# zhouxian/FluidLab

Hardware: AMD Instinct MI355X
Metric: MPM substeps/sec (fwd+bwd), 128^3 grid / 200k particles (higher is better)
Workload: dtype f32; 1 GPU; water block 128^3 grid, 200k particles (BASELINE configs[1] inputs), fwd+bwd, evolving (rolling window); nc_start=34727, nc_end=99039, parallelism=1 env, 1 GPU

## Files before the change

### __graft_entry__.py

```python
import os
import subprocess
import sys

ROOT = os.path.dirname(os.path.abspath(__file__))
CSRC = os.path.join(ROOT, 'fluidlab_amd', 'csrc')
HIP_LIB = os.path.join(CSRC, 'libfluidengine_hip.so')
HIPCC_FLAGS = ['--offload-arch=gfx950', '-O3', '-std=c++17', '-shared', '-fPIC', '-munsafe-fp-atomics', '-fno-slp-vectorize']


def _hipcc():
    for c in ('/opt/rocm/bin/hipcc', 'hipcc'):
        if c == 'hipcc' or os.path.exists(c):
            return c


def _source_hash(sources):
    import hashlib
    h = hashlib.sha256(' '.join(HIPCC_FLAGS).encode())
    for s in sources:
        h.update(os.path.basename(s).encode())
        with open(s, 'rb') as f:
            h.update(f.read())
    return h.hexdigest()


def build(force=False):
    srcs = [os.path.join(CSRC, f) for f in ('fe_engine.hip', 'fe_math.h', 'fe_grid_launch.h', 'fe_smoke.h', 'fe_smoke_reads.h', 'fe_mesh.h', 'fe_param_grad.h', 'fe_summary.h', 'fe_task_loss.h', 'fe_density.h', 'fe_render.h')] + \
           [os.path.join(ROOT, 'include', f) for f in ('fluidengine.h', 'fluidengine_ext.h')]
    stamp, want = HIP_LIB + '.srchash', _source_hash(srcs)
    have = open(stamp).read().strip() if os.path.exists(stamp) else ''
    if force or os.environ.get('FE_FORCE_BUILD') == '1' or not os.path.exists(HIP_LIB) or have != want:
        subprocess.check_call([_hipcc()] + HIPCC_FLAGS + ['-o', HIP_LIB, os.path.join(CSRC, 'fe_engine.hip')])
        with open(stamp, 'w') as f:
            f.write(want + '\n')
        print('build: compiled', os.path.relpath(HIP_LIB, ROOT), 'from sources', want[:16])
    else:
        print('build: up to date', os.path.relpath(HIP_LIB, ROOT), 'sources', want[:16])
    subprocess.check_call(['make', '-s', '-C', os.path.join(ROOT, 'oracle')])
    if ROOT not in sys.path:
        sys.path.insert(0, ROOT)
    import fluidlab_amd
    from fluidlab_amd import _capi
    lib = _capi.load_hip()
    missing = lib.missing_symbols()
    assert not missing, f'libfluidengine_hip.so is missing ABI symbols: {missing}'
    assert lib.has_ext, f'libfluidengine_hip.so is missing extension symbols: {lib.missing_ext_symbols()}'


def smoke():
    if ROOT not in sys.path:
        sys.path.insert(0, ROOT)
    sys.path.insert(0, os.path.join(ROOT, 'tests'))
    import numpy as np
    import scenarios as S
    from fluidlab_amd import _capi
    hip = _capi.load_hip()
    oracle = _capi.EngineLib(os.path.join(ROOT, 'oracle', '_build', 'libfe_oracle_f64.so'))
    sc = S.latte_mini()
    a = S.run_latte(hip, sc, device=0)
    b = S.run_latte(oracle, sc)
    assert (a['final']['used'] == b['final']['used']).all()
    assert S.rel_l2(a['final']['x'], b['final']['x']) <= 1e-5, S.rel_l2(a['final']['x'], b['final']['x'])
    assert S.rel_l2(a['step_loss'], b['step_loss']) <= 1e-4
    assert S.cosine(a['action_grad'], b['action_grad']) >= 0.999999
    assert S.rel_l2(a['action_grad'], b['action_grad']) <= 1e-4
    print('smoke ok: backend', hip.backend, 'loss', float(np.sum(a['step_loss'])),
          'action-grad rel L2 vs oracle', S.rel_l2(a['action_grad'], b['action_grad']))


if __name__ == '__main__':
    build(force='--force' in sys.argv)
    if len(sys.argv) > 1 and sys.argv[1] == 'smoke':
        smoke()
```

### fluidlab_amd/csrc/fe_engine.hip

```cpp
#include <hip/hip_runtime.h>

#include <algorithm>
#include <cstdio>
#include <cstdlib>
#include <cstring>
#include <string>
#include <vector>

#include "../../include/fluidengine.h"
#include "../../include/fluidengine_ext.h"
#include "fe_math.h"
#include "fe_grid_launch.h"

static_assert(sizeof(fe_real) == 4, "the HIP engine is fp32 (macros.py:207-211)");

#define FR_WORDS 25
#define GR_WORDS 24

template <typename T>
struct Plane {
    char* base; unsigned off;
    __host__ __device__ __forceinline__ T& operator[](int s) const { return *(T*)(base + (size_t)(off + (unsigned)s * (unsigned)sizeof(T))); }
    __host__ __device__ __forceinline__ T* ptr() const { return (T*)(base + (size_t)off); }
};
// ... 278 lines not shown
struct TileO { int ox, oy, oz; };
#define BLK_PACK(bi, bj, bk) (((bi) << 20) | ((bj) << 10) | (bk))
#define BLK_I(pk) ((pk) >> 20)
#define BLK_J(pk) (((pk) >> 10) & 1023)
#define BLK_K(pk) ((pk) & 1023)
__device__ __forceinline__ TileO tile_origin(int pk) {
    TileO t; t.ox = BLK_I(pk) * 4 - 1; t.oy = BLK_J(pk) * 4 - 1; t.oz = BLK_K(pk) * 4 - 1; return t;
}
__device__ __forceinline__ int tile_base(const TileO& t, const Stencil& st) {
    int lx = st.base[0] - t.ox, ly = st.base[1] - t.oy, lz = st.base[2] - t.oz;
    bool in = (unsigned)lx <= TILE_T - 3 && (unsigned)ly <= TILE_T - 3 && (unsigned)lz <= TILE_T - 3;
    return in ? (lx * TILE_T + ly) * TILE_T + lz : -1;
}
__device__ __forceinline__ bool tile_node(const TileO& t, int l, int n, int& i, int& j, int& k) {
    i = t.ox + (l >> 6); j = t.oy + ((l >> 3) & 7); k = t.oz + (l & 7);
    return (unsigned)i < (unsigned)n && (unsigned)j < (unsigned)n && (unsigned)k < (unsigned)n;
}

struct PairCtx {
    int4 it;
    int  ti;
    int  slab;
    int  nth, t0;
    int  i;
    bool live;
    bool quad;
};
#define QUAD_BIT (1 << 29)
#define QUAD_MAX 64
#ifndef QH
#define QH 2
#endif
struct UnitRec { int4 a, b, c, d; };
struct Unit { int4 a, b, q; };
__device__ __forceinline__ PairCtx pair_ctx(const Unit& u) {
    const int tid = threadIdx.x, half = __builtin_amdgcn_readfirstlane(tid >> 7);
    const bool same = (u.a.w >> 30) & 1;
    const int ia = u.a.w & 0x1fffffff, ib = u.b.w;
    const int ih = half ? ib : ia;
    PairCtx c;
    c.live = same || ih >= 0;
    c.it = (half && ib >= 0) ? u.b : u.a;
    c.it.w = 0;
    if (ih < 0) c.it.z = 0;
    c.ti = (half && !same) ? 1 : 0;
    c.slab = same ? ia : (ih >= 0 ? ih : ia);
    c.nth = same ? WG : HALF;
    c.t0 = same ? tid : (tid & (HALF - 1));
    c.i = tid & (HALF - 1);
    c.quad = false;
    return c;
}
__device__ __forceinline__ PairCtx unit_ctx(const Unit& u) {
    const int tid = threadIdx.x;
    const bool quad = (u.a.w & QUAD_BIT) != 0;
    const int wave = __builtin_amdgcn_readfirstlane(tid >> 6), half = wave >> 1;
    const bool same = (u.a.w >> 30) & 1;
    const int ia = u.a.w & 0x1fffffff;
    const int ax = u.a.x, ay = u.a.y, az = u.a.z, bx = u.b.x, by = u.b.y, bz = u.b.z, bw = u.b.w, qx = u.q.x, qy = u.q.y, qz = u.q.z, qw = u.q.w;
    const bool second = half && bw >= 0;
    const int mx = quad ? qx : (second ? bx : ax);
    const int my = quad ? qy : (second ? by : ay);
    const int mz = quad ? qz : (second ? bz : az);
    const int ih = quad ? (wave == 0 ? ia : qw) : (half ? bw : ia);
    PairCtx c;
    c.quad = quad;
    c.live = (same && !quad) || ih >= 0;
    c.it = make_int4(mx, my, ih >= 0 ? mz : 0, 0);
    c.ti = quad ? wave : ((half && !same) ? 1 : 0);
    c.slab = quad ? (ih >= 0 ? ih : 0) : (same ? ia : (ih >= 0 ? ih : ia));
    c.nth = quad ? 64 : (same ? WG : HALF);
    c.t0 = quad ? (tid & 63) : (same ? tid : (tid & (HALF - 1)));
    c.i = quad ? (tid & 63) : (tid & (HALF - 1));
    return c;
}
__device__ __forceinline__ void unit_sync(bool quad) {
    if (quad) asm volatile("" ::: "memory");
    else __syncthreads();
}
__device__ __forceinline__ void unit_enter(bool quad, bool& prev_quad) {
    if (prev_quad && !quad) __syncthreads();
    prev_quad = quad;
}
template <bool GATHER = false>
__device__ __forceinline__ Unit unit_load(const TableP& T, int w) {
    const int4* p = (const int4*)((GATHER ? T.units_p : T.units) + (w < T.units_cap ? w : T.units_cap - 1));
    int4 a = p[0], b = p[1], q = p[__builtin_amdgcn_readfirstlane(threadIdx.x >> 6)];
    if (w >= T.units_cap) a.z = -2;
#define UNIT_SCALAR(q) make_int4(__builtin_amdgcn_readfirstlane(q.x), __builtin_amdgcn_readfirstlane(q.y), __builtin_amdgcn_readfirstlane(q.z), __builtin_amdgcn_readfirstlane(q.w))
    Unit u;
    u.a = UNIT_SCALAR(a); u.b = UNIT_SCALAR(b); u.q = UNIT_SCALAR(q);
#undef UNIT_SCALAR
    return u;
}

#define FE_MAX_BATCH 8
#ifndef FE_KALIGN_BYTES
#define FE_KALIGN_BYTES 16384
#endif
#define FE_KALIGN __attribute__((aligned(FE_KALIGN_BYTES)))
template <typename A> struct Batch { A a[FE_MAX_BATCH]; };


__device__ void effector_move(const EffP& e, int f) {
    float xin[3] = {e.pos[f * 3] + e.v[f * 3], e.pos[f * 3 + 1] + e.v[f * 3 + 1], e.pos[f * 3 + 2] + e.v[f * 3 + 2]};
    float xn[3], J[3][3];
    boundary_x(e.bnd, xin, xn, J);
    e.pos[(f + 1) * 3] = xn[0]; e.pos[(f + 1) * 3 + 1] = xn[1]; e.pos[(f + 1) * 3 + 2] = xn[2];
    float w3[3] = {e.w[f * 3], e.w[f * 3 + 1], e.w[f * 3 + 2]};
    float q[4] = {e.quat[f * 4], e.quat[f * 4 + 1], e.quat[f * 4 + 2], e.quat[f * 4 + 3]};
    float qw[4], qo[4];
    quat_from_w(w3, qw);
    quat_mul(qw, q, qo);
    e.quat[(f + 1) * 4] = qo[0]; e.quat[(f + 1) * 4 + 1] = qo[1]; e.quat[(f + 1) * 4 + 2] = qo[2]; e.quat[(f + 1) * 4 + 3] = qo[3];
}

#define GS_BLK 112
struct GridStore { float4* data; int* flag; int cap;
    unsigned char* touched; unsigned char* dirty; unsigned char* live; unsigned char* cur; unsigned char stamp; };
__device__ __forceinline__ int stencil_regions(int lb) {
    const int lut = 0x26c93;
    const int ax = (lut >> (3 * (lb >> 6))) & 7, ay = (lut >> (3 * ((lb >> 3) & 7))) & 7, az = (lut >> (3 * (lb & 7))) & 7;
    const int myz = ((ay & 1) ? az : 0) | ((ay & 2) ? az << 3 : 0) | ((ay & 4) ? az << 6 : 0);
    return ((ax & 1) ? myz : 0) | ((ax & 2) ? myz << 9 : 0) | ((ax & 4) ? myz << 18 : 0);
}
__device__ __forceinline__ int neighbour_entry(const int* __restrict__ blk_slot, int nb, int pk) {
    int lane = threadIdx.x & 63;
    asm volatile("" : "+v"(lane));
    int e = -1;
    if (lane < 27) {
        const int i2 = BLK_I(pk) + lane / 9 - 1, j2 = BLK_J(pk) + (lane / 3) % 3 - 1, k2 = BLK_K(pk) + lane % 3 - 1;
        if ((unsigned)i2 < (unsigned)nb && (unsigned)j2 < (unsigned)nb && (unsigned)k2 < (unsigned)nb) e = blk_slot[(i2 * nb + j2) * nb + k2];
    }
    return e;
}
template <int CTRL, int ROW_MASK>
__device__ __forceinline__ int dpp_or(int x) { return x | __builtin_amdgcn_update_dpp(0, x, CTRL, ROW_MASK, 0xf, true); }
template <bool FG = false>
__device__ __forceinline__ int touch_regions(int mask, int entry, const GridStore& GS) {
    mask = dpp_or<0x111, 0xf>(mask); mask = dpp_or<0x112, 0xf>(mask); mask = dpp_or<0x114, 0xf>(mask); mask = dpp_or<0x118, 0xf>(mask);
    mask = dpp_or<0x142, 0xa>(mask); mask = dpp_or<0x143, 0xc>(mask);
    mask = __builtin_amdgcn_readlane(mask, 63);
    if (!FG && entry >= 0 && ((mask >> (threadIdx.x & 63)) & 1)) GS.touched[entry] = GS.stamp;
    return mask;
}
__device__ __forceinline__ void mark_dirty(const GridStore& GS, const int* __restrict__ blk_slot, int b) {
    const int e = blk_slot[b];
    if (e >= 0) GS.dirty[e] = GS.stamp;
}

#define FG_SH 32
#define FG_LINE 32
enum { FGC_STARTED = 0 , FGC_DONE = 8 , FGC_FIN = FGC_DONE + FG_SH , FGC_TOP = FGC_FIN + FG_SH, FGC_LATE, FGC_SKIP, FGC_ERR, FGC_N };
struct FgDev {
    float* late;
    int* late_flag; int* late_list;
    unsigned char* skipm;
    int* ctr;
};
struct FgArgs {
    const FgDev* F; const float4* slab; float* acc; float4* out; int* blk_list; int* blk_count; int* blk_flag; int f;
};
#define FG_CNT(a) ((int)((a) & 0x1fffffull))
#define FG_TCH(a) ((int)(((a) >> 21) & 0x1fffffull))
#define FG_DRT(a) ((int)((a) >> 42))
__shared__ int s_fg[10];
template <bool BWD> __device__ __forceinline__ void fg_owner_phase(const SimP& S, const TableP& T, const GridStore& GS, const FgArgs& A);
__device__ __forceinline__ void fg_rare(const FgDev* F) { (void)__hip_atomic_fetch_or(F->ctr + FGC_TOP * FG_LINE, 1 << 16, __ATOMIC_RELAXED, __HIP_MEMORY_SCOPE_AGENT); }
__device__ __forceinline__ void fg_mark_late(const FgDev* F, int e) {
    int* fl = F->late_flag + e;
    const int v = __hip_atomic_load(fl, __ATOMIC_RELAXED, __HIP_MEMORY_SCOPE_AGENT);
    if (v != 1 && atomicCAS(fl, v, 1) == v) {
        const int i = atomicAdd(F->ctr + FGC_LATE * FG_LINE, 1);
        __hip_atomic_store(F->late_list + i, e, __ATOMIC_RELAXED, __HIP_MEMORY_SCOPE_AGENT);
        fg_rare(F);
    }
}
__device__ __forceinline__ void fg_begin(const FgDev* F) {
    if (threadIdx.x == 0) (void)__hip_atomic_fetch_add(F->ctr + (FGC_STARTED + (blockIdx.x & 7)) * FG_LINE, 1, __ATOMIC_RELAXED, __HIP_MEMORY_SCOPE_AGENT);
    if (threadIdx.x < 10) s_fg[threadIdx.x] = 0;
    __syncthreads();
}
__device__ __forceinline__ int wave_or(int mask) {
    mask = dpp_or<0x111, 0xf>(mask); mask = dpp_or<0x112, 0xf>(mask); mask = dpp_or<0x114, 0xf>(mask); mask = dpp_or<0x118, 0xf>(mask);
// ... 409 lines not shown
#pragma unroll
    for (int a = 0; a < 3; a++)
#pragma unroll
        for (int b = 0; b < 3; b++) nC.a[a][b] = c4 * __builtin_fmaf(-st.fx[b], nv[a], M.a[a][b]);
}
template <bool TILE, bool ALIAS, bool ROLLED = false>
__device__ __forceinline__ void g2p_gather(const SimP& S, int lb, const Stencil& st, const float4* __restrict__ g_out, int tofs, float nv[3], m3& nC) {
    if (!TILE) { g2p_gather_global<true, ALIAS ? FE_SLOW_UNR : 1>(S, st, g_out, nv, nC); return; }
    const float* gt = ALIAS ? (const float*)s_acc : s_gtile;
    nv[0] = nv[1] = nv[2] = 0.f;
    const float c4 = 4.f * S.inv_dx;
    m3 M = m3_zero();
#pragma unroll ROLLED ? 1 : 9
    for (int ij = 0; ij < 9; ij++) {
        const int i = ij / 3, j = ij - 3 * i;
        const float wij = STW(st, i, 0) * STW(st, j, 1);
        float T[3] = {0.f, 0.f, 0.f}, Tz[3] = {0.f, 0.f, 0.f};
#pragma unroll
        for (int kk = 0; kk < 3; kk++) {
            const float weight = wij * st.w[kk][2];
            float g0, g1, g2;
            if (TILE) {
                const int l = tofs + lb + (i * TILE_T + j) * TILE_T + kk;
                g0 = gt[l]; g1 = gt[TILE_N + l]; g2 = gt[2 * TILE_N + l];
            } else {
                float4 gv = g_out[cell_addr(st.base[0] + i, st.base[1] + j, st.base[2] + kk, S.nb)];
                g0 = gv.x; g1 = gv.y; g2 = gv.z;
            }
            const float gw[3] = {weight * g0, weight * g1, weight * g2};
#pragma unroll
            for (int a = 0; a < 3; a++) { T[a] += gw[a]; if (kk > 0) Tz[a] += (float)kk * gw[a]; }
        }
#pragma unroll
        for (int a = 0; a < 3; a++) {
            nv[a] += T[a];
            M.a[a][0] += (float)i * T[a]; M.a[a][1] += (float)j * T[a]; M.a[a][2] += Tz[a];
        }
    }
#pragma unroll
    for (int a = 0; a < 3; a++)
#pragma unroll
        for (int b = 0; b < 3; b++) nC.a[a][b] = c4 * (M.a[a][b] - st.fx[b] * nv[a]);
}
template <int NIT, typename LD, typename ST>
__device__ __forceinline__ void tile_nodes_n(int t0, int nth, LD&& ld, ST&& st) {
    float4 v[NIT];
#pragma unroll
    for (int it = 0; it < NIT; it++) v[it] = ld(t0 + it * nth);
#pragma unroll
    for (int it = 0; it < NIT; it++) st(t0 + it * nth, v[it]);
}
template <bool QUADS = true, int MAXIT = 8, typename LD, typename ST>
__device__ __forceinline__ void tile_nodes(int t0, int nth, LD&& ld, ST&& st) {
    if (nth == WG) tile_nodes_n<2>(t0, nth, ld, st);
    else if (!QUADS || nth == HALF) {
        if constexpr (MAXIT >= 4) tile_nodes_n<4>(t0, nth, ld, st);
        else { tile_nodes_n<2>(t0, nth, ld, st); tile_nodes_n<2>(t0 + 2 * nth, nth, ld, st); }
    } else {
        if constexpr (MAXIT >= 8) tile_nodes_n<8>(t0, nth, ld, st);
        else if constexpr (MAXIT >= 4) { tile_nodes_n<4>(t0, nth, ld, st); tile_nodes_n<4>(t0 + 4 * nth, nth, ld, st); }
        else { for (int r = 0; r < 4; r++) tile_nodes_n<2>(t0 + 2 * r * nth, nth, ld, st); }
    }
}
__device__ __forceinline__ float4 tile_node_load(const TileO& to, const SimP& S, const float4* __restrict__ src, int l) {
    int i, j, k;
    const bool ok = tile_node(to, l, S.n, i, j, k);
    const float4 v = src[ok ? cell_addr(i, j, k, S.nb) : 0];
    return make_float4(ok ? v.x : 0.f, ok ? v.y : 0.f, ok ? v.z : 0.f, ok ? v.w : 0.f);
}
template <bool ALIAS = false>
__device__ __forceinline__ void load_tile3(const TileO& to, const SimP& S, const float4* __restrict__ src, const PairCtx& pc, int tofs_alias = 0) {
    if (!pc.live) return;
    float* gt = ALIAS ? (float*)s_acc : s_gtile;
    const int tofs = ALIAS ? tofs_alias : pc.ti * 3 * TILE_N;
    tile_nodes<ALIAS>(pc.t0, pc.nth, [&](int l) { return tile_node_load(to, S, src, l); },
                      [&](int l, const float4 v) { gt[tofs + l] = v.x; gt[tofs + TILE_N + l] = v.y; gt[tofs + 2 * TILE_N + l] = v.z; });
}

struct FuseP { float* fr_prev; const float4* g_out; int* slow; int* blk_count_prev; };
template <bool WRITE, bool GENERAL, bool FUSED = false, bool FG = false>
__device__ __forceinline__ void p2g_body(SimP S, float* fr_cur, float* fr_next, TableP T,
                                            const int* __restrict__ pool_idx, GridW G, AgentP agent, InjectP inj, int act, int f,
                                            GridStore GS, int fiso, FuseP FU = FuseP{nullptr, nullptr, nullptr, nullptr}) {
    if (!WRITE && GS.cap > 0 && GS.flag[f]) return;
    const int tid = threadIdx.x;
    if (WRITE && blockIdx.x == 0 && tid == 0 && act) {
        for (int i = 0; i < agent.n; i++) effector_move(agent.e[i], f);
    }
    if (FG) {
        if (blockIdx.x == 0 && tid == 0 && GS.cap > 0) __hip_atomic_store(GS.flag + f, 1, __ATOMIC_RELAXED, __HIP_MEMORY_SCOPE_AGENT);
        fg_begin(G.fg);
    }
    if (FUSED && blockIdx.x == 0 && tid == 0) *FU.blk_count_prev = 0;
    FrameV cur = frame_view(fr_cur, S.Np, 0, (!GENERAL && (fiso & 1)) ? 1 : 0);
    FrameV curw = frame_view(fr_cur, S.Np, 0);
    FrameV prev = frame_view(FUSED ? FU.fr_prev : fr_cur, S.Np);
    FrameV nxt = frame_view(fr_next, S.Np, S.wt & 1, (!GENERAL && (fiso & 2)) ? 1 : 0);
    const int slab_wt = FG ? 1 : (S.wt & 1);
    TL(S, 0);
    Unit un = unit_load(T, blockIdx.x);
    const int n_slots = T.meta[5];
    bool prev_quad = false;
    for (int wg = blockIdx.x; FG || wg < n_slots; wg += gridDim.x) {
        if (FG || wg != (int)blockIdx.x) un = unit_load(T, wg);
        if (FG && wg >= n_slots) break;
        if (un.a.z == -2) continue;
        if (un.a.z >= 0) {
            const PairCtx pc = unit_ctx(un);
            unit_enter(pc.quad, prev_quad);
            const int4 it = pc.it;
            const TileO to = tile_origin(it.x);
            const int aofs = pc.ti * 4 * TILE_N;
            int fg_t = 0, fg_d = 0;
            TL(S, 1);
            const int nbr_entry = neighbour_entry(T.blk_slot, S.nb, it.x);
            auto zero_tile = [&]() {
                if (pc.quad) { if (pc.live) for (int l = pc.t0; l < TILE_N; l += 64) ((int4*)((int*)s_acc + aofs))[l] = make_int4(0, 0, 0, 0); }
                else if (pc.live) for (int l = pc.t0; l < 4 * TILE_N; l += pc.nth) s_acc[aofs + l] = 0.0;
            };
            if (!FUSED) { zero_tile(); unit_sync(pc.quad); }
            FixScale fs_p = {1.f, 1.f}, fs_m = {1.f, 1.f};
            bool wshell = false;
            {
                const int wbase = pc.quad ? 0 : (pc.i & 64);
                const int cnt = __builtin_amdgcn_readfirstlane(min(64, max(0, it.z - wbase)));
                const LaneSplit ls = lane_split(cnt, (S.lsplit & 1) != 0 && !(WRITE && !FUSED && act && agent.collector));
                const int i = wbase + ls.p, s = it.y + i;
                const bool has = ls.ok && i < it.z;
                const int s_ld = has ? s : it.y;
                const int uflag = cur.used[s_ld];
                P2GRaw raw;
                if (FUSED) {
                    const int gofs_w = pc.quad ? aofs : 2 * aofs;
                    const int uprev = prev.used[s_ld];
                    const float4 a0 = prev.A0[s_ld];
                    load_F(cur, s_ld, raw.p.F);
                    raw.info = load_info(S, T.info, s_ld);
                    load_tile3<true>(to, S, FU.g_out, pc, gofs_w);
                    unit_sync(pc.quad);
                    const float xp[3] = {a0.x, a0.y, a0.z};
                    Stencil stp;
                    stencil_make(xp, S.inv_dx, stp);
                    if (has && uprev != 0 && stencil_inside(stp, S.n)) {
                        const int lbp = tile_base(to, stp);
                        if (lbp >= 0) g2p_gather<true, true>(S, lbp, stp, FU.g_out, gofs_w, raw.p.v, raw.p.C);
                        else { if (ls.primary) atomicAdd(FU.slow, 1); g2p_gather<false, true, true>(S, 0, stp, FU.g_out, 0, raw.p.v, raw.p.C); }
#pragma unroll
                        for (int a = 0; a < 3; a++) raw.p.x[a] = xp[a] + S.dt * raw.p.v[a];
                        if (ls.primary) store_xvC(curw, s, raw.p.x, raw.p.v, raw.p.C);
                    } else load_xvC(cur, s_ld, raw.p);
                    unit_sync(pc.quad);
                    zero_tile();
                    unit_sync(pc.quad);
                } else p2g_load(S, cur, s_ld, T.info, raw);
                bool used = has && uflag != 0;
                bool taken = false;
                if (WRITE && !FUSED && used && act && agent.collector) { taken = collector_takes(S, cur, nxt, s, T.info, agent); used = !taken; }
                P2GPrep q;
                q.inside = false;
                int lb = -1;
                if (used) {
                    p2g_compute<WRITE, GENERAL>(S, nxt, s, raw, G, q, ls.primary);
                    if (q.inside) lb = tile_base(to, q.st);
                } else {
                    q.m = 0.f; q.affine = m3_zero(); q.mv[0] = q.mv[1] = q.mv[2] = 0.f;
                    float zero[3] = {0.f, 0.f, 0.f};
                    stencil_make(zero, S.inv_dx, q.st);
                }
                TL(S, 2);
#ifdef FE_DUMMY_VALU
                {
                    float dmy = q.m;
#pragma unroll
                    for (int i_ = 0; i_ < FE_DUMMY_VALU; i_++) asm volatile("v_fma_f32 %0, %0, %0, %0" : "+v"(dmy));
                    asm volatile("" :: "v"(dmy));
                }
#endif
                const bool in_tile = lb >= 0;
                if (used && q.inside && !in_tile && ls.primary) { atomicAdd(G.slow, 1); p2g_scatter_global<FG>(S, q, G, GS, T.blk_slot, it.x, fg_d); }
                if (__any(in_tile)) {
                    fg_t = touch_regions<FG>(in_tile ? stencil_regions(lb) : 0, nbr_entry, GS);
                    if (pc.quad) {
                        wshell = __any(in_tile && stencil_on_shell(lb));
                        float bp = 0.f;
#pragma unroll
                        for (int a = 0; a < 3; a++) bp = fmaxf(bp, fabsf(q.mv[a]) + 2.f * S.dx * (fabsf(q.affine.a[a][0]) + fabsf(q.affine.a[a][1]) + fabsf(q.affine.a[a][2])));
                        fs_p = fix_scale(wave_max(in_tile ? bp : 0.f));
                        fs_m = fix_scale(wave_max(in_tile ? q.m : 0.f));
                        if (__any(in_tile && !(bp <= 3.4e38f))) fs_p.inv = __int_as_float(0x7fc00000);
                        const float sp = in_tile ? fs_p.s : 1.f;
                        q.m *= in_tile ? fs_m.s : 1.f;
#pragma unroll
                        for (int a = 0; a < 3; a++) { q.mv[a] *= sp; q.affine.a[a][0] *= sp; q.affine.a[a][1] *= sp; q.affine.a[a][2] *= sp; }
                        p2g_scatter_tile_split<true>(S, q, in_tile, in_tile ? lb : 0, aofs, ls);
                    } else p2g_scatter_tile_split<false>(S, q, in_tile, in_tile ? lb : 0, aofs, ls);
                }
                if (has && !used && !taken && WRITE && ls.primary) unused_particle_fwd(S, cur, nxt, s, T.pid_of_slot[s], pool_idx, agent, inj, f);
            }
            TL(S, 4);
            unit_sync(pc.quad);
            TL(S, 5);
            if (pc.quad) {
                if (pc.live) quad_handover<4, FG>(S, (const int*)s_acc + aofs, fs_p.inv, fs_m.inv, G.slab, pc.slab, G.g_in, GS, to, nbr_entry, wshell, slab_wt, fg_d);
            } else if (pc.live) for (int l = pc.t0; l < TILE_N; l += pc.nth)
                tile_handover<4, false, FG>(S, G.slab, pc.slab, G.g_in, GS, to, nbr_entry, l,
                                 make_float4((float)s_acc[aofs + l], (float)s_acc[aofs + TILE_N + l], (float)s_acc[aofs + 2 * TILE_N + l], (float)s_acc[aofs + 3 * TILE_N + l]), slab_wt, fg_d);
            if (FG) fg_unit_end(T, pc, nbr_entry, fg_t, fg_d);
            else unit_sync(pc.quad);
            TL(S, 6);
        } else {
            const int s = un.a.y + tid;
            if (s < S.N) {
                P2GRaw raw;
                bool have = false;
                if (FUSED && prev.used[s]) {
                    const float4 a0 = prev.A0[s];
                    const float xp[3] = {a0.x, a0.y, a0.z};
                    Stencil stp;
                    stencil_make(xp, S.inv_dx, stp);
                    if (stencil_inside(stp, S.n)) {
                        g2p_gather<false, true, true>(S, 0, stp, FU.g_out, 0, raw.p.v, raw.p.C);
#pragma unroll
                        for (int a = 0; a < 3; a++) raw.p.x[a] = xp[a] + S.dt * raw.p.v[a];
                        store_xvC(curw, s, raw.p.x, raw.p.v, raw.p.C);
                        have = true;
                    }
                }
                if (cur.used[s]) {
                    if (WRITE && !FUSED && act && agent.collector && collector_takes(S, cur, nxt, s, T.info, agent)) continue;
                    P2GPrep q;
                    if (FUSED && have) { load_F(cur, s, raw.p.F); raw.info = load_info(S, T.info, s); p2g_compute<WRITE, GENERAL>(S, nxt, s, raw, G, q); }
                    else p2g_prepare<WRITE, GENERAL>(S, cur, nxt, s, T.info, G, q);
                    int none = 0;
                    if (q.inside) p2g_scatter_global<FG>(S, q, G, GS, T.blk_slot, -1, none);
                } else if (WRITE) unused_particle_fwd(S, cur, nxt, s, T.pid_of_slot[s], pool_idx, agent, inj, f);
            }
        }
    }
}
struct P2GArgs { SimP S; float* fr_cur; float* fr_next; TableP T; const int* pool_idx; GridW G; AgentP agent; InjectP inj; int act; int f; GridStore GS; int fiso; FuseP FU; };
template <bool WRITE, bool GENERAL>
__global__ FE_KALIGN __launch_bounds__(WG, GENERAL ? 3 : 4) void k_p2g(SimP S, float* fr_cur, float* fr_next, TableP T, const int* pool_idx, GridW G, AgentP agent, InjectP inj, int act, int f, GridStore GS, int fiso) { p2g_body<WRITE, GENERAL>(S, fr_cur, fr_next, T, pool_idx, G, agent, inj, act, f, GS, fiso); }
template <bool GENERAL>
__global__ FE_KALIGN __launch_bounds__(WG, GENERAL ? 3 : 4) void k_g2p_p2g(SimP S, float* fr_cur, float* fr_next, TableP T, const int* pool_idx, GridW G, AgentP agent, InjectP inj, int act, int f, GridStore GS, int fiso, FuseP FU) { p2g_body<true, GENERAL, true>(S, fr_cur, fr_next, T, pool_idx, G, agent, inj, act, f, GS, fiso, FU); }
template <typename ARGS>
__device__ __forceinline__ const ARGS* fg_args_again() {
    const ARGS* p = (const ARGS*)__builtin_amdgcn_kernarg_segment_ptr();
    asm volatile("" : "+s"(p));
    return p;
}
template <bool GENERAL>
__global__ FE_KALIGN __launch_bounds__(WG, GENERAL ? 3 : 4) void k_p2g_fg(P2GArgs A) {
    p2g_body<true, GENERAL, false, true>(A.S, A.fr_cur, A.fr_next, A.T, A.pool_idx, A.G, A.agent, A.inj, A.act, A.f, A.GS, A.fiso);
    const P2GArgs* B = fg_args_again<P2GArgs>();
    TL(B->S, 3);
    fg_owner_phase<false>(B->S, B->T, B->GS, FgArgs{B->G.fg, B->G.slab, B->G.g_in, B->G.g_out, B->G.blk_list, B->G.blk_count, B->G.blk_flag, B->f});
}
template <bool GENERAL>
__global__ FE_KALIGN __launch_bounds__(WG, GENERAL ? 3 : 4) void k_g2p_p2g_fg(P2GArgs A) {
    p2g_body<true, GENERAL, true, true>(A.S, A.fr_cur, A.fr_next, A.T, A.pool_idx, A.G, A.agent, A.inj, A.act, A.f, A.GS, A.fiso, A.FU);
    const P2GArgs* B = fg_args_again<P2GArgs>();
    TL(B->S, 3);
    fg_owner_phase<false>(B->S, B->T, B->GS, FgArgs{B->G.fg, B->G.slab, B->G.g_in, B->G.g_out, B->G.blk_list, B->G.blk_count, B->G.blk_flag, B->f});
}
template <bool GENERAL>
__global__ FE_KALIGN __launch_bounds__(WG, GENERAL ? 3 : 4) void k_g2p_p2g_b(Batch<P2GArgs> B) { const P2GArgs& A = B.a[blockIdx.y]; p2g_body<true, GENERAL, true>(A.S, A.fr_cur, A.fr_next, A.T, A.pool_idx, A.G, A.agent, A.inj, A.act, A.f, A.GS, A.fiso, A.FU); }
template <bool WRITE, bool GENERAL>
__global__ FE_KALIGN __launch_bounds__(WG, GENERAL ? 3 : 4) void k_p2g_b(Batch<P2GArgs> B) { const P2GArgs& A = B.a[blockIdx.y]; p2g_body<WRITE, GENERAL>(A.S, A.fr_cur, A.fr_next, A.T, A.pool_idx, A.G, A.agent, A.inj, A.act, A.f, A.GS, A.fiso); }


template <bool NODE>
__device__ __forceinline__ bool agent_collide_particle(const SimP& S, const AgentP& agent, int f, const float x[3], float nv[3]) {
    const float sdt = NODE ? 0.f : S.dt;
    bool any = false;
    for (int ei = 0; ei < agent.n; ei++) {
        const EffP& e = agent.e[ei];
        if (!e.has_mesh) continue;
        const float pos[3] = {x[0] + sdt * nv[0], x[1] + sdt * nv[1], x[2] + sdt * nv[2]};
        if (!(pos[1] > agent.collide_min_y)) continue;
        float out[3];
        any |= t_dynamic_collide<float>(e.mesh, e.pos + f * 3, e.quat + f * 4, e.pos + (f + 1) * 3, e.quat + (f + 1) * 4, pos, nv, S.dt, out);
        nv[0] = out[0]; nv[1] = out[1]; nv[2] = out[2];
    }
    return any;
}
#define FE_MAX_STATICS 4
struct NodeWork { int c, ni, nj, nk; float4 gi; float go[3]; float pad; };
struct StaticsP { int n; const SdfP* s; };

template <bool STATICS, bool DYN = false>
__device__ __forceinline__ void node_velocity(const SimP& S, const StaticsP& ST, const float4 gi, int i, int j, int k, float vo[3], float kmul[3],
                                              float (*trace)[3] = nullptr, const AgentP* agent = nullptr, int f = 0, float* vdyn = nullptr,
                                              bool* dyn_hit = nullptr) {
    float inv = 1.f / gi.w;
    vo[0] = fmaf(S.dt, S.g[0], inv * gi.x);
    vo[1] = fmaf(S.dt, S.g[1], inv * gi.y);
    vo[2] = fmaf(S.dt, S.g[2], inv * gi.z);
    float xn[3] = {(float)i * S.dx, (float)j * S.dx, (float)k * S.dx};
    if (STATICS) {
#pragma unroll
        for (int si = 0; si < FE_MAX_STATICS; si++) {
            if (si < ST.n) {
                if (trace) { trace[si][0] = vo[0]; trace[si][1] = vo[1]; trace[si][2] = vo[2]; }
                static_collide(ST.s[si], xn, vo, nullptr);
            }
        }
    }
    if (DYN) {
        if (vdyn) { vdyn[0] = vo[0]; vdyn[1] = vo[1]; vdyn[2] = vo[2]; }
        const bool hit = agent_collide_particle<true>(S, *agent, f, xn, vo);
        if (dyn_hit) *dyn_hit = hit;
    }
    boundary_v(S.bnd, xn, vo, kmul);
}
__device__ __forceinline__ void node_statics_grad(const SimP& S, const StaticsP& ST, int i, int j, int k, const float (*trace)[3], float g[3]) {
    float xn[3] = {(float)i * S.dx, (float)j * S.dx, (float)k * S.dx};
#pragma unroll
    for (int si = FE_MAX_STATICS - 1; si >= 0; si--) {
        if (si < ST.n) {
            float vin[3] = {trace[si][0], trace[si][1], trace[si][2]};
            static_collide(ST.s[si], xn, vin, g);
        }
    }
}

__device__ __forceinline__ int2 nbr_record(const TableP& T, int e, int lane) {
    return lane < 27 ? T.nbr[e * 27 + lane] : make_int2(0, 0);
}
template <int NPL>
__device__ __forceinline__ float4 gather_slabs(const float4* __restrict__ slab, const int2 mine, int lane) {
    const int o[3] = {lane >> 4, (lane >> 2) & 3, lane & 3};
    int a0[8], n[8];
    float4 v0[8], v1[8];
#pragma unroll
    for (int c = 0; c < 8; c++) {
        int nbr = 0, si = 0;
        bool valid = true;
#pragma unroll
        for (int d = 0; d < 3; d++) {
            const bool other = (c >> d) & 1;
            valid = valid && (!other || o[d] <= 1);
            nbr = nbr * 3 + (other ? 0 : 1);
            si = si * SLAB_T + o[d] + (other ? 4 : 0);
        }
        const int f = __shfl(mine.x, nbr, 64), k = __shfl(mine.y, nbr, 64);
        n[c] = valid ? k : 0;
        a0[c] = valid ? (NPL == 4 ? f * SLAB_N + si : f * (SLAB_N * 16) + si * 12) : 0;
    }
    const __amdgpu_buffer_rsrc_t rs = wt_rsrc((void*)slab);
    auto ld = [&](int at) -> float4 {
        if (NPL == 4) return slab[at];
        const u32x3 u = __builtin_amdgcn_raw_buffer_load_b96(rs, at, 0, 0);
        return make_float4(__uint_as_float(u.x), __uint_as_float(u.y), __uint_as_float(u.z), 0.f);
    };
    constexpr int STRIDE = NPL == 4 ? SLAB_N : SLAB_N * 16;
#pragma unroll
    for (int c = 0; c < 8; c++) {
        const bool h0 = n[c] > 0, h1 = n[c] > 2;
        const float4 a = ld(h0 ? a0[c] : 0);
        const float4 b = ld(h1 ? a0[c] + 2 * STRIDE : 0);
        v0[c] = make_float4(h0 ? a.x : 0.f, h0 ? a.y : 0.f, h0 ? a.z : 0.f, h0 ? a.w : 0.f);
        v1[c] = make_float4(h1 ? b.x : 0.f, h1 ? b.y : 0.f, h1 ? b.z : 0.f, h1 ? b.w : 0.f);
    }
    float4 acc = make_float4(0.f, 0.f, 0.f, 0.f);
#pragma unroll
    for (int c = 0; c < 8; c++) {
        acc.x += v0[c].x; acc.y += v0[c].y; acc.z += v0[c].z; acc.w += v0[c].w;
        acc.x += v1[c].x; acc.y += v1[c].y; acc.z += v1[c].z; acc.w += v1[c].w;
        for (int k = 4; k < n[c]; k += 2) {
            const float4 v = ld(a0[c] + k * STRIDE);
            acc.x += v.x; acc.y += v.y; acc.z += v.z; acc.w += v.w;
        }
    }
    return acc;
}

__device__ __forceinline__ int static_entry(int wave) {
    const int G = gridDim.x;
    if ((G & 127) != 0) return blockIdx.x * 4 + wave;
    const int j = blockIdx.x >> 3;
    return ((j >> 4) * 8 + (blockIdx.x & 7)) * 64 + (j & 15) * 4 + wave;
}
template <bool KEEP, bool STATICS, bool DYN>
__device__ __forceinline__ void grid_body(SimP S, TableP T, const float4* __restrict__ slab, float* g_in, float4* g_out,
                                              const int* __restrict__ blk_list, const int* __restrict__ blk_count, int* blk_flag,
                                              GridStore GS, int f, int* frame_slow, StaticsP ST, AgentP agent) {
    if (KEEP && GS.cap > 0 && GS.flag[f]) return;
    const int lane = threadIdx.x & 63, wave = __builtin_amdgcn_readfirstlane(threadIdx.x >> 6);
    TL(S, 0);
    const int es = static_entry(wave);
    const bool es_ok = es < S.nb * S.nb * S.nb;
    const int blk_s = es_ok ? T.active[es] : 0;
    const unsigned char tch_s = es_ok ? GS.touched[es] : (unsigned char)0, drt_s = es_ok ? GS.dirty[es] : (unsigned char)0;
    const int2 nbr_s = es_ok ? nbr_record(T, es, lane) : make_int2(0, 0);
    const int n_static = T.meta[2], n_dyn = *blk_count;
    if (!KEEP && blockIdx.x == 0 && threadIdx.x == 0) {
        if (GS.cap > 0) GS.flag[f] = (n_static <= GS.cap && *frame_slow == 0) ? 1 : 0;
        *frame_slow = 0;
    }
    auto one_block = [&](int e, int b, bool is_static, bool touched, bool dirty, const int2 nbr) {
        const int c = (b << 6) | lane;
        const int bi = b / (S.nb * S.nb), bj = (b / S.nb) % S.nb, bk = b % S.nb;
        TL(S, 1);
        float4 gi = make_float4(0.f, 0.f, 0.f, 0.f);
        if (dirty) gi = make_float4(g_in[c], g_in[S.ncell + c], g_in[2 * S.ncell + c], g_in[3 * S.ncell + c]);
        if (touched) { const float4 t = gather_slabs<4>(slab, nbr, lane); gi.x += t.x; gi.y += t.y; gi.z += t.z; gi.w += t.w; }
        float4 out = make_float4(0.f, 0.f, 0.f, 0.f);
        if (gi.w > FE_EPS) TL(S, 2);
        if (gi.w > FE_EPS) {
            float vo[3], kmul[3];
            node_velocity<STATICS, DYN>(S, ST, gi, bi * 4 + (lane >> 4), bj * 4 + ((lane >> 2) & 3), bk * 4 + (lane & 3), vo, kmul, nullptr, &agent, f);
            out = make_float4(vo[0], vo[1], vo[2], 0.f);
        }
        g_out[c] = out;
        if (!KEEP) {
            if (is_static && e < GS.cap) {
                float4* dst = GS.data + ((size_t)f * GS.cap + e) * GS_BLK;
                dst[lane] = gi;
                const u32x3 u = {__float_as_uint(out.x), __float_as_uint(out.y), __float_as_uint(out.z)};
                __builtin_amdgcn_raw_buffer_store_b96(u, wt_rsrc(dst), 1024 + lane * 12, 0, 0);
            }
            if (dirty) { g_in[c] = 0.f; g_in[S.ncell + c] = 0.f; g_in[2 * S.ncell + c] = 0.f; g_in[3 * S.ncell + c] = 0.f; }
            if (lane == 0 && !is_static) blk_flag[b] = 0;
        } else {
            g_in[c] = gi.x; g_in[S.ncell + c] = gi.y; g_in[2 * S.ncell + c] = gi.z; g_in[3 * S.ncell + c] = gi.w;
        }
        TL(S, 3);
    };
    if (n_static <= 4 * (int)gridDim.x) {
        if (es < n_static) {
            const bool tm = tch_s == GS.stamp, dm = drt_s == GS.stamp;
            if (lane == 0) {
                if (KEEP) GS.cur[es] = (tm || dm) ? 1 : 0;
                else if (es < GS.cap) GS.live[(size_t)f * GS.cap + es] = (tm || dm) ? 1 : 0;
            }
            if (tm || dm) one_block(es, blk_s, true, tm, dm, nbr_s);
        }
    } else {
        const int W = 4 * (int)gridDim.x;
        for (int e0 = es; e0 < n_static; e0 += 8 * W) {
            unsigned tm = 0, dm = 0;
            int blk8[8]; int2 nbr8[8];
#pragma unroll
            for (int k = 0; k < 8; k++) {
                const int e = e0 + k * W;
                const bool ok = e < n_static;
                const int ec = ok ? e : e0;
                const unsigned char t = GS.touched[ec], d = GS.dirty[ec];
                blk8[k] = T.active[ec]; nbr8[k] = nbr_record(T, ec, lane);
                tm |= ((ok && t == GS.stamp) ? 1u : 0u) << k; dm |= ((ok && d == GS.stamp) ? 1u : 0u) << k;
            }
            tm = __builtin_amdgcn_readfirstlane(tm); dm = __builtin_amdgcn_readfirstlane(dm);
            if (lane < 8 && e0 + lane * W < n_static) {
                const int e = e0 + lane * W;
                if (KEEP) GS.cur[e] = ((tm | dm) >> lane) & 1;
                else if (e < GS.cap) GS.live[(size_t)f * GS.cap + e] = ((tm | dm) >> lane) & 1;
            }
            unsigned todo = tm | dm;
            while (todo) {
                const int k = __builtin_ctz(todo);
                todo &= todo - 1;
                int blk = blk8[0]; int2 nbr = nbr8[0];
#pragma unroll
                for (int j = 1; j < 8; j++) if (k == j) { blk = blk8[j]; nbr = nbr8[j]; }
                one_block(e0 + k * W, __builtin_amdgcn_readfirstlane(blk), true, (tm >> k) & 1, (dm >> k) & 1, nbr);
            }
        }
    }
    for (int d = blockIdx.x * 4 + wave; d < n_dyn; d += gridDim.x * 4) one_block(-1, blk_list[d], false, false, true, make_int2(0, 0));
}
struct GridArgs { SimP S; TableP T; const float4* slab; float* g_in; float4* g_out; const int* blk_list; const int* blk_count; int* blk_flag; GridStore GS; int f; int* frame_slow; StaticsP ST; AgentP agent; };
template <bool KEEP, bool STATICS, bool DYN>
__global__ FE_KALIGN __launch_bounds__(256, (STATICS || DYN) ? 2 : 4) void k_grid(SimP S, TableP T, const float4* slab, float* g_in, float4* g_out, const int* blk_list, const int* blk_count, int* blk_flag, GridStore GS, int f, int* frame_slow, StaticsP ST, AgentP agent) { grid_body<KEEP, STATICS, DYN>(S, T, slab, g_in, g_out, blk_list, blk_count, blk_flag, GS, f, frame_slow, ST, agent); }
template <bool KEEP, bool STATICS, bool DYN>
__global__ FE_KALIGN __launch_bounds__(256, (STATICS || DYN) ? 2 : 4) void k_grid_b(Batch<GridArgs> B) { const GridArgs& A = B.a[blockIdx.y]; grid_body<KEEP, STATICS, DYN>(A.S, A.T, A.slab, A.g_in, A.g_out, A.blk_list, A.blk_count, A.blk_flag, A.GS, A.f, A.frame_slow, A.ST, A.agent); }

__device__ __forceinline__ float4 fg_load16(const void* base, unsigned byte_off) {
    const u32x4 u = __builtin_amdgcn_raw_buffer_load_b128(wt_rsrc((void*)base), (int)byte_off, 0, 16);
    return make_float4(__uint_as_float(u.x), __uint_as_float(u.y), __uint_as_float(u.z), __uint_as_float(u.w));
}
__device__ __forceinline__ float4 fg_node_out(const SimP& S, const float4 gi, int b, int lane, float kmul[3]) {
    float4 out = make_float4(0.f, 0.f, 0.f, 0.f);
    kmul[0] = kmul[1] = kmul[2] = 0.f;
    if (gi.w > FE_EPS) {
        const int bi = b / (S.nb * S.nb), bj = (b / S.nb) % S.nb, bk = b % S.nb;
        float vo[3];
        node_velocity<false, false>(S, StaticsP{0, nullptr}, gi, bi * 4 + (lane >> 4), bj * 4 + ((lane >> 2) & 3), bk * 4 + (lane & 3), vo, kmul);
        out = make_float4(vo[0], vo[1], vo[2], 0.f);
    }
    return out;
}
__device__ __forceinline__ void fg_fwd_store(const GridStore& GS, const FgArgs& A, int e, int c, int lane, const float4 gi, const float4 out) {
    wt_store16(A.out, (unsigned)c * 16u, out);
    if (e >= 0 && e < GS.cap) {
        float4* dst = GS.data + ((size_t)A.f * GS.cap + e) * GS_BLK;
        wt_store16(dst, (unsigned)lane * 16u, gi);
        const u32x3 u = {__float_as_uint(out.x), __float_as_uint(out.y), __float_as_uint(out.z)};
        __builtin_amdgcn_raw_buffer_store_b96(u, wt_rsrc(dst), 1024 + lane * 12, 0, 16);
    }
}
__device__ __forceinline__ void fg_fwd_block(const SimP& S, const GridStore& GS, const FgArgs& A, int e, int b, const int2 nbr, bool touched, bool dirty) {
    const int lane = threadIdx.x & 63;
    const int c = (b << 6) | lane;
    float4 gi = make_float4(0.f, 0.f, 0.f, 0.f);
    if (dirty) gi = make_float4(atomicExch(A.acc + c, 0.f), atomicExch(A.acc + S.ncell + c, 0.f), atomicExch(A.acc + 2 * S.ncell + c, 0.f), atomicExch(A.acc + 3 * S.ncell + c, 0.f));
    if (touched) { const float4 t = gather_slabs<4>(A.slab, nbr, lane); gi.x += t.x; gi.y += t.y; gi.z += t.z; gi.w += t.w; }
    float kmul[3];
    const float4 out = fg_node_out(S, gi, b, lane, kmul);
    fg_fwd_store(GS, A, e, c, lane, gi, out);
}
__device__ __forceinline__ float4 fg_grad_out(const float4 gi, const float4 go, const float kmul[3]) {
    float4 out = make_float4(0.f, 0.f, 0.f, 0.f);
    if (gi.w > FE_EPS) {
        const float inv = 1.f / gi.w;
        const float g0 = go.x * kmul[0], g1 = go.y * kmul[1], g2 = go.z * kmul[2];
        out.x = g0 * inv; out.y = g1 * inv; out.z = g2 * inv;
        out.w = -(gi.x * g0 + gi.y * g1 + gi.z * g2) * inv * inv;
    }
    return out;
}
__device__ __forceinline__ void fg_bwd_block(const SimP& S, const GridStore& GS, const FgArgs& A, int e, int b, const int2 nbr, bool dirty) {
    const int lane = threadIdx.x & 63;
    const int c = (b << 6) | lane;
    const float4 gi = GS.data[((size_t)A.f * GS.cap + e) * GS_BLK + lane];
    float4 go = make_float4(0.f, 0.f, 0.f, 0.f);
    if (dirty) go = make_float4(atomicExch(A.acc + c, 0.f), atomicExch(A.acc + S.ncell + c, 0.f), atomicExch(A.acc + 2 * S.ncell + c, 0.f), 0.f);
    { const float4 t = gather_slabs<3>(A.slab, nbr, lane); go.x += t.x; go.y += t.y; go.z += t.z; }
    float kmul[3];
    (void)fg_node_out(S, gi, b, lane, kmul);
    wt_store16(A.out, (unsigned)c * 16u, fg_grad_out(gi, go, kmul));
}
__device__ __forceinline__ unsigned long long fg_word(const unsigned long long* p) {
    const unsigned long long a = __hip_atomic_load(p, __ATOMIC_RELAXED, __HIP_MEMORY_SCOPE_AGENT);
    return (unsigned long long)(unsigned)__builtin_amdgcn_readfirstlane((int)(unsigned)a) | ((unsigned long long)(unsigned)__builtin_amdgcn_readfirstlane((int)(unsigned)(a >> 32)) << 32);
}
__device__ __forceinline__ int fg_int(const int* p) { return __hip_atomic_load(p, __ATOMIC_RELAXED, __HIP_MEMORY_SCOPE_AGENT); }
__device__ __forceinline__ int fg_int_u(const int* p) { return __builtin_amdgcn_readfirstlane(fg_int(p)); }
#define FG_SPIN_MAX (1 << 22)
__device__ __forceinline__ void fg_give_up(const FgDev* F) { if ((threadIdx.x & 63) == 0) atomicAdd(F->ctr + FGC_ERR * FG_LINE, 1); }
template <bool BWD>
__device__ __forceinline__ void fg_entry(const SimP& S, const TableP& T, const GridStore& GS, const FgArgs& A, int e, unsigned long long a) {
    const int lane = threadIdx.x & 63;
    const bool touched = FG_TCH(a) != 0, dirty = FG_DRT(a) != 0;
    if (lane == 0) __hip_atomic_store(T.arrive + e, 0ull, __ATOMIC_RELAXED, __HIP_MEMORY_SCOPE_AGENT);
    const int b = T.active[e];
    const int2 nbr = nbr_record(T, e, lane);
    if (!BWD) {
        if (lane == 0 && e < GS.cap) __hip_atomic_store(GS.live + (size_t)A.f * GS.cap + e, (unsigned char)((touched || dirty) ? 1 : 0), __ATOMIC_RELAXED, __HIP_MEMORY_SCOPE_AGENT);
        if (touched || dirty) fg_fwd_block(S, GS, A, e, b, nbr, touched, dirty);
    } else {
        if (GS.live[(size_t)A.f * GS.cap + e] != 0) fg_bwd_block(S, GS, A, e, b, nbr, dirty);
    }
}
template <bool BWD>
__device__ __forceinline__ void fg_final(const SimP& S, const TableP& T, const GridStore& GS, const FgArgs& A) {
    const int lane = threadIdx.x & 63;
    const FgDev* F = A.F;
    int* const ctr = F->ctr;
    const int n_static = T.meta[2];
    const int* __restrict__ expected = (const int*)(T.arrive + S.nb * S.nb * S.nb);
    const int n_dyn = BWD ? 0 : fg_int_u(A.blk_count), n_skip = fg_int_u(ctr + FGC_SKIP * FG_LINE), n_late = fg_int_u(ctr + FGC_LATE * FG_LINE);
    if (!BWD && n_dyn > 0) {
        for (int d = 0; d < n_dyn; d++) {
            const int b = fg_int_u(A.blk_list + d), c = (b << 6) | lane;
            const float4 gi = make_float4(atomicExch(F->late + c, 0.f), atomicExch(F->late + S.ncell + c, 0.f), atomicExch(F->late + 2 * S.ncell + c, 0.f), atomicExch(F->late + 3 * S.ncell + c, 0.f));
            float kmul[3];
            fg_fwd_store(GS, A, -1, c, lane, gi, fg_node_out(S, gi, b, lane, kmul));
            if (lane == 0) __hip_atomic_store(A.blk_flag + b, 0, __ATOMIC_RELAXED, __HIP_MEMORY_SCOPE_AGENT);
        }
        if (lane == 0) {
            __hip_atomic_store(A.blk_count, 0, __ATOMIC_RELAXED, __HIP_MEMORY_SCOPE_AGENT);
            if (GS.cap > 0) __hip_atomic_store(GS.flag + A.f, 0, __ATOMIC_RELAXED, __HIP_MEMORY_SCOPE_AGENT);
        }
    }
    if (n_skip > 0) {
        for (int e0 = 0; e0 < n_static; e0 += 64) {
            const int e = e0 + lane;
            unsigned long long todo = __ballot(e < n_static && __hip_atomic_load(F->skipm + e, __ATOMIC_RELAXED, __HIP_MEMORY_SCOPE_AGENT) == GS.stamp);
            while (todo) {
                const int k = __builtin_ctzll(todo);
                todo &= todo - 1;
                const int ek = e0 + k;
                if (lane == 0) __hip_atomic_store(F->skipm + ek, (unsigned char)0, __ATOMIC_RELAXED, __HIP_MEMORY_SCOPE_AGENT);
                const unsigned long long a = fg_word(T.arrive + ek);
                if (FG_CNT(a) != expected[ek]) fg_give_up(F);
                fg_entry<BWD>(S, T, GS, A, ek, a);
            }
        }
        if (lane == 0) __hip_atomic_store(ctr + FGC_SKIP * FG_LINE, 0, __ATOMIC_RELAXED, __HIP_MEMORY_SCOPE_AGENT);
    }
    if (n_late > 0) {
        for (int it = 0; ; it++) {
            int v = lane < FG_SH ? fg_int(ctr + (FGC_FIN + lane) * FG_LINE) : 0;
#pragma unroll
            for (int o = 16; o >= 1; o >>= 1) v += __shfl_xor(v, o, 64);
            if ((unsigned)__builtin_amdgcn_readfirstlane(v) - S.fg_base == gridDim.x) break;
            if (it > FG_SPIN_MAX) { fg_give_up(F); break; }
            __builtin_amdgcn_s_sleep(8);
        }
        for (int i = 0; i < n_late; i++) {
            const int e = fg_int_u(F->late_list + i);
            const int b = T.active[e], c = (b << 6) | lane;
            if (lane == 0) __hip_atomic_store(F->late_flag + e, 0, __ATOMIC_RELAXED, __HIP_MEMORY_SCOPE_AGENT);
            float4 lt = make_float4(atomicExch(F->late + c, 0.f), atomicExch(F->late + S.ncell + c, 0.f), atomicExch(F->late + 2 * S.ncell + c, 0.f), 0.f);
            float kmul[3];
            if (!BWD) {
                lt.w = atomicExch(F->late + 3 * S.ncell + c, 0.f);
                const bool live = e < GS.cap && __hip_atomic_load(GS.live + (size_t)A.f * GS.cap + e, __ATOMIC_RELAXED, __HIP_MEMORY_SCOPE_AGENT) != 0;
                float4 gi = make_float4(0.f, 0.f, 0.f, 0.f);
                if (live) gi = fg_load16(GS.data + ((size_t)A.f * GS.cap + e) * GS_BLK, (unsigned)lane * 16u);
                gi.x += lt.x; gi.y += lt.y; gi.z += lt.z; gi.w += lt.w;
                fg_fwd_store(GS, A, e, c, lane, gi, fg_node_out(S, gi, b, lane, kmul));
                if (lane == 0 && e < GS.cap) __hip_atomic_store(GS.live + (size_t)A.f * GS.cap + e, (unsigned char)1, __ATOMIC_RELAXED, __HIP_MEMORY_SCOPE_AGENT);
            } else if (GS.live[(size_t)A.f * GS.cap + e] != 0) {
                const float4 gi = GS.data[((size_t)A.f * GS.cap + e) * GS_BLK + lane];
                (void)fg_node_out(S, gi, b, lane, kmul);
                const float4 d = fg_grad_out(gi, lt, kmul), o = fg_load16(A.out, (unsigned)c * 16u);
                wt_store16(A.out, (unsigned)c * 16u, make_float4(o.x + d.x, o.y + d.y, o.z + d.z, o.w + d.w));
            }
        }
        if (lane == 0) __hip_atomic_store(ctr + FGC_LATE * FG_LINE, 0, __ATOMIC_RELAXED, __HIP_MEMORY_SCOPE_AGENT);
    }
}
#define FG_NPF 2
template <bool BWD>
__device__ __forceinline__ void fg_owner_phase(const SimP& S, const TableP& T, const GridStore& GS, const FgArgs& A) {
    int lane = threadIdx.x & 63;
    asm volatile("" : "+v"(lane));
    const int wave = __builtin_amdgcn_readfirstlane(threadIdx.x >> 6);
    const FgDev* F = A.F;
    int* const ctr = F->ctr;
    const int G_ = gridDim.x, W = 4 * G_;
    const int es = static_entry(wave);
    const int n_static = T.meta[2];
    const int* __restrict__ expected = (const int*)(T.arrive + S.nb * S.nb * S.nb);
    const int e_l = es + lane * W;
    const bool have = e_l < n_static;
    const int exp_l = have ? expected[e_l] : 0, b_l = have ? T.active[e_l] : 0;
    const unsigned char live_l = (BWD && have) ? GS.live[(size_t)A.f * GS.cap + e_l] : (unsigned char)0;
    int2 pf[FG_NPF];
#pragma unroll
    for (int j = 0; j < FG_NPF; j++) pf[j] = (es + j * W < n_static) ? nbr_record(T, es + j * W, lane) : make_int2(0, 0);
    int st = lane < 8 ? fg_int(ctr + (FGC_STARTED + lane) * FG_LINE) : 0;
    st += __shfl_xor(st, 1, 64); st += __shfl_xor(st, 2, 64); st += __shfl_xor(st, 4, 64);
    const bool wait = (unsigned)__builtin_amdgcn_readfirstlane(st) - S.fg_base == (unsigned)G_ && !S.fg_nowait;
    unsigned long long a_l = have ? __hip_atomic_load(T.arrive + e_l, __ATOMIC_RELAXED, __HIP_MEMORY_SCOPE_AGENT) : 0ull;
    unsigned long long pending = __ballot(have);
    if (!wait) {
        const bool skip = have && FG_CNT(a_l) != exp_l;
        if (skip) __hip_atomic_store(F->skipm + e_l, GS.stamp, __ATOMIC_RELAXED, __HIP_MEMORY_SCOPE_AGENT);
        int nskip = __popcll(__ballot(skip));
        for (int e = es + 64 * W; e < n_static; e += W) { if (lane == 0) __hip_atomic_store(F->skipm + e, GS.stamp, __ATOMIC_RELAXED, __HIP_MEMORY_SCOPE_AGENT); nskip++; }
        if (nskip && lane == 0) { atomicAdd(ctr + FGC_SKIP * FG_LINE, nskip); fg_rare(F); }
        pending &= ~__ballot(skip);
    }
    asm volatile("s_waitcnt vmcnt(0)" ::: "memory");
    int r1 = -1;
    bool signs = false;
    if (lane == 0 && atomicAdd(&s_fg[8], 1) == 3) { signs = true; r1 = atomicAdd(ctr + (FGC_DONE + (int)(blockIdx.x % FG_SH)) * FG_LINE, 1); }
    signs = __builtin_amdgcn_readfirstlane(signs ? 1 : 0) != 0;
    for (int it = 0; pending; it++) {
        const bool mine_pending = (pending >> lane) & 1ull;
        const bool done = mine_pending && FG_CNT(a_l) == exp_l;
        const unsigned long long done_now = __ballot(done);
        if (!done_now) {
            if (it > FG_SPIN_MAX) { fg_give_up(F); break; }
            __builtin_amdgcn_s_sleep(2);
            if (mine_pending) a_l = __hip_atomic_load(T.arrive + e_l, __ATOMIC_RELAXED, __HIP_MEMORY_SCOPE_AGENT);
            continue;
        }
        TL(S, 5);
        const bool touched = FG_TCH(a_l) != 0, dirty = FG_DRT(a_l) != 0;
        bool heavy = false;
        if (done) {
            __hip_atomic_store(T.arrive + e_l, 0ull, __ATOMIC_RELAXED, __HIP_MEMORY_SCOPE_AGENT);
            if (!BWD) {
                heavy = touched || dirty;
                if (e_l < GS.cap) __hip_atomic_store(GS.live + (size_t)A.f * GS.cap + e_l, (unsigned char)(heavy ? 1 : 0), __ATOMIC_RELAXED, __HIP_MEMORY_SCOPE_AGENT);
            } else heavy = live_l != 0;
        }
        unsigned long long todo = __ballot(heavy);
        const unsigned long long dirty_set = __ballot(dirty), touched_set = __ballot(touched);
        pending &= ~done_now;
        if ((pending >> lane) & 1ull) a_l = __hip_atomic_load(T.arrive + e_l, __ATOMIC_RELAXED, __HIP_MEMORY_SCOPE_AGENT);
        auto record = [&](int kk) -> int2 {
            if (kk < FG_NPF) {
                int2 r = pf[0];
#pragma unroll
                for (int j = 1; j < FG_NPF; j++) if (kk == j) r = pf[j];
                return r;
            }
            return nbr_record(T, es + kk * W, lane);
        };
        int k = todo ? __builtin_ctzll(todo) : -1;
        int2 nbr = k >= 0 ? record(k) : make_int2(0, 0);
        while (k >= 0) {
            todo &= todo - 1;
            const int k_next = todo ? __builtin_ctzll(todo) : -1;
            const int2 nbr_next = k_next >= 0 ? record(k_next) : make_int2(0, 0);
            const int e = es + k * W, b = __builtin_amdgcn_readlane(b_l, k);
            if (!BWD) fg_fwd_block(S, GS, A, e, b, nbr, (touched_set >> k) & 1ull, (dirty_set >> k) & 1ull);
            else fg_bwd_block(S, GS, A, e, b, nbr, (dirty_set >> k) & 1ull);
            k = k_next; nbr = nbr_next;
        }
    }
    if (wait) for (int e = es + 64 * W; e < n_static; e += W) {
        const int exp_e = expected[e];
        unsigned long long a = fg_word(T.arrive + e);
        for (int it = 0; FG_CNT(a) != exp_e; it++) {
            if (it > FG_SPIN_MAX) { fg_give_up(F); break; }
            __builtin_amdgcn_s_sleep(2);
            a = fg_word(T.arrive + e);
        }
        fg_entry<BWD>(S, T, GS, A, e, a);
    }
    TL(S, 4);
// ... 29 lines not shown
}

__device__ __forceinline__ void load_tile4(const TileO& to, const SimP& S, const float4* __restrict__ src, const PairCtx& pc) {
    if (!pc.live) return;
    const int tofs = pc.ti * 4 * TILE_N;
    tile_nodes<false>(pc.t0, pc.nth, [&](int l) { return tile_node_load(to, S, src, l); },
                      [&](int l, const float4 v) { s_tile[tofs + l] = v.x; s_tile[tofs + TILE_N + l] = v.y; s_tile[tofs + 2 * TILE_N + l] = v.z; s_tile[tofs + 3 * TILE_N + l] = v.w; });
}

template <bool COLLIDE>
__device__ __forceinline__ bool slot_g2p(const SimP& S, const FrameV& cur, const FrameV& nxt, int s, bool use_tile,
                                         const TileO& to, const float4* __restrict__ g_out, int* slow, const AgentP& agent, int f,
                                         int u, const float4 a0, int tofs, float xn[3]) {
    if (!u) return false;
    float x[3] = {a0.x, a0.y, a0.z};
    Stencil st;
    stencil_make(x, S.inv_dx, st);
    if (!stencil_inside(st, S.n)) return false;
    const int lb = use_tile ? tile_base(to, st) : -1;
    if (lb >= 0) used_particle_g2p<true, COLLIDE>(S, cur, nxt, s, lb, st, x, g_out, agent, f, tofs, xn);
    else { if (use_tile) atomicAdd(slow, 1); used_particle_g2p<false, COLLIDE>(S, cur, nxt, s, 0, st, x, g_out, agent, f, 0, xn); }
    return true;
}

#define SORT_CLR_WGS 32
struct SortKeyP { int* key; int* rank; int* cnt; int* bcnt; int* nact; };
__shared__ int s_sk[8];
__device__ __forceinline__ int sort_key_of(const SimP& S, const float x[3]) {
    Stencil st;
    stencil_make(x, S.inv_dx, st);
    return stencil_inside(st, S.n) ? cell_addr(st.base[0], st.base[1], st.base[2], S.nb) : S.ncell;
}
template <bool WG_TAIL>
__device__ __forceinline__ void sort_key_rank(const SimP& S, const SortKeyP& K, bool has, int s, int kk) {
    int lane = threadIdx.x & 63;
    asm volatile("" : "+v"(lane));
    const unsigned long long below = (1ull << lane) - 1ull;
    int r_tail = -1;
    if (WG_TAIL) {
        const int wave = __builtin_amdgcn_readfirstlane(threadIdx.x >> 6);
        const unsigned long long mt = __ballot(has && kk == S.ncell);
        if (lane == 0) s_sk[wave] = __popcll(mt);
        __syncthreads();
        if (threadIdx.x == 0) {
            const int tot = s_sk[0] + s_sk[1] + s_sk[2] + s_sk[3];
            int base = 0;
            if (tot > 0) { base = atomicAdd(K.cnt + S.ncell, tot); atomicAdd(K.bcnt + (S.ncell >> 6), tot); }
            s_sk[4] = base;
        }
        __syncthreads();
        int before = 0;
        for (int w = 0; w < wave; w++) before += s_sk[w];
        if (has && kk == S.ncell) r_tail = s_sk[4] + before + __popcll(mt & below);
        __syncthreads();
        has = has && kk != S.ncell;
    }
    unsigned long long rem = __ballot(has);
    int leader = lane, idx = 0, size = 0;
    while (rem) {
        const int L = __builtin_ctzll(rem);
        const int k = __builtin_amdgcn_readlane(kk, L);
        const unsigned long long m = __ballot(has && kk == k);
        if ((m >> lane) & 1ull) { leader = L; idx = __popcll(m & below); size = __popcll(m); }
        rem &= ~m;
    }
    int base = 0;
    if (has && lane == leader) base = atomicAdd(K.cnt + kk, size);
    rem = __ballot(has);
    while (rem) {
        const int L = __builtin_ctzll(rem);
        const int b = __builtin_amdgcn_readlane(kk >> 6, L);
        const unsigned long long m = __ballot(has && (kk >> 6) == b);
        if (lane == L) atomicAdd(K.bcnt + b, __popcll(m));
        rem &= ~m;
    }
    const int r = __shfl(base, leader, 64) + idx;
    if (has) { K.key[s] = kk; K.rank[s] = r; }
    else if (WG_TAIL && r_tail >= 0) { K.key[s] = S.ncell; K.rank[s] = r_tail; }
}

template <bool COLLIDE, bool SORTKEY = false>
__device__ __forceinline__ void g2p_body(SimP S, float* fr_cur, float* fr_next, TableP T, const float4* __restrict__ g_out,
                                            int* blk_count, int* slow, AgentP agent, int f, SortKeyP K = SortKeyP{nullptr, nullptr, nullptr, nullptr, nullptr}) {
    const int tid = threadIdx.x;
    if (blockIdx.x == 0 && tid == 0) { *blk_count = 0; if (SORTKEY) *K.nact = 0; }
    const int n_wg = gridDim.x;
    FrameV cur = frame_view(fr_cur, S.Np);
    FrameV nxt = frame_view(fr_next, S.Np, S.wt & 2);
    TL(S, 0);
    Unit un = unit_load<true>(T, blockIdx.x);
    const int n_slots = T.meta[9];
    for (int wg = blockIdx.x; wg < n_slots; wg += n_wg) {
        if (wg != (int)blockIdx.x) un = unit_load<true>(T, wg);
        if (un.a.z == -2) continue;
        if (un.a.z >= 0) {
            const PairCtx pc = pair_ctx(un);
            const int4 it = pc.it;
            const TileO to = tile_origin(it.x);
            const int i = pc.i;
            const int s0 = it.y + (i < it.z ? i : 0);
            TL(S, 1);
            const int u = cur.used[s0];
            const float4 a0 = cur.A0[s0];
            load_tile3(to, S, g_out, pc);
            __syncthreads();
            TL(S, 2);
            float xn[3] = {0.f, 0.f, 0.f};
            bool moved = false;
            if (i < it.z) moved = slot_g2p<COLLIDE>(S, cur, nxt, s0, true, to, g_out, slow, agent, f, u, a0, pc.ti * 3 * TILE_N, xn);
            if (SORTKEY) {
                int kk = S.ncell;
                if (moved) kk = sort_key_of(S, xn);
                else if (i < it.z && !u && nxt.used[s0]) { const float4 n0 = nxt.A0[s0]; const float xi[3] = {n0.x, n0.y, n0.z}; kk = sort_key_of(S, xi); }
                sort_key_rank<false>(S, K, i < it.z, s0, kk);
            }
            TL(S, 3);
            __syncthreads();
            TL(S, 4);
        } else {
            const int s = un.a.y + tid;
            TileO none = {0, 0, 0};
            float xn[3] = {0.f, 0.f, 0.f};
            bool moved = false;
            int u = 0;
            if (s < S.N) { u = cur.used[s]; moved = slot_g2p<COLLIDE>(S, cur, nxt, s, false, none, g_out, slow, agent, f, u, cur.A0[s], 0, xn); }
            if (SORTKEY) {
                int kk = S.ncell;
                if (moved) kk = sort_key_of(S, xn);
                else if (s < S.N && !u && nxt.used[s]) { const float4 n0 = nxt.A0[s]; const float xi[3] = {n0.x, n0.y, n0.z}; kk = sort_key_of(S, xi); }
                sort_key_rank<true>(S, K, s < S.N, s, kk);
            }
        }
    }
}
struct G2PArgs { SimP S; float* fr_cur; float* fr_next; TableP T; const float4* g_out; int* blk_count; int* slow; AgentP agent; int f; };
template <bool COLLIDE>
__global__ FE_KALIGN __launch_bounds__(WG) void k_g2p(SimP S, float* fr_cur, float* fr_next, TableP T, const float4* g_out, int* blk_count, int* slow, AgentP agent, int f) { g2p_body<COLLIDE>(S, fr_cur, fr_next, T, g_out, blk_count, slow, agent, f); }
template <bool COLLIDE>
__global__ FE_KALIGN __launch_bounds__(WG) void k_g2p_sortkey(SimP S, float* fr_cur, float* fr_next, TableP T, const float4* g_out, int* blk_count, int* slow, AgentP agent, int f, SortKeyP K) { g2p_body<COLLIDE, true>(S, fr_cur, fr_next, T, g_out, blk_count, slow, agent, f, K); }
template <bool COLLIDE>
__global__ FE_KALIGN __launch_bounds__(WG) void k_g2p_b(Batch<G2PArgs> B) { const G2PArgs& A = B.a[blockIdx.y]; g2p_body<COLLIDE>(A.S, A.fr_cur, A.fr_next, A.T, A.g_out, A.blk_count, A.slow, A.agent, A.f); }



struct VoutSrc { const float4* g_out; const float4* store; const int* blk_slot; };
__device__ __forceinline__ float4 store_vout(const float4* __restrict__ st, int slot, int node) {
    const u32x3 u = __builtin_amdgcn_raw_buffer_load_b96(wt_rsrc((void*)st), slot * (GS_BLK * 16) + 1024 + node * 12, 0, 0);
    return make_float4(__uint_as_float(u.x), __uint_as_float(u.y), __uint_as_float(u.z), 0.f);
}
__device__ __forceinline__ float4 vout_at(const SimP& S, const VoutSrc& V, int i, int j, int k) {
    if (!V.store) return V.g_out[cell_addr(i, j, k, S.nb)];
    const int slot = V.blk_slot[(((i >> 2) * S.nb) + (j >> 2)) * S.nb + (k >> 2)];
    return slot >= 0 ? store_vout(V.store, slot, ((i & 3) << 4) | ((j & 3) << 2) | (k & 3)) : make_float4(0.f, 0.f, 0.f, 0.f);
}

template <bool GPRE = false>
__device__ __forceinline__ void used_particle_g2p_grad(const SimP& S, const FrameV& Gn, const FrameV& Gc, int s, const Stencil& st, const VoutSrc& V, float* gg_out,
                                                       const PState* gpre = nullptr) {
    PState g;
    if (GPRE) copy_xvC(g, *gpre);
    else load_xvC(Gn, s, g);
    float gv[3] = {g.v[0] + S.dt * g.x[0], g.v[1] + S.dt * g.x[1], g.v[2] + S.dt * g.x[2]};
    const float c4 = 4.f * S.inv_dx;
    float gfx[3] = {0.f, 0.f, 0.f};
    float qb[3], qz[3], nvw[3] = {0.f, 0.f, 0.f};
#pragma unroll
    for (int a = 0; a < 3; a++) {
        qb[a] = gv[a] - c4 * (g.C.a[a][0] * st.fx[0] + g.C.a[a][1] * st.fx[1] + g.C.a[a][2] * st.fx[2]);
        qz[a] = c4 * g.C.a[a][2];
    }
#pragma unroll 1
    for (int ij = 0; ij < 9; ij++) {
        const int i = ij / 3, j = ij - 3 * i;
        const float wi = STW(st, i, 0), wj = STW(st, j, 1);
        const float wiwj = wi * wj, dwiwj = stencil_dw(st, i, 0) * wj, widwj = wi * stencil_dw(st, j, 1);
        float qij[3];
#pragma unroll
        for (int a = 0; a < 3; a++) qij[a] = qb[a] + c4 * (g.C.a[a][0] * (float)i + g.C.a[a][1] * (float)j);
#pragma unroll
        for (int kk = 0; kk < 3; kk++) {
            const float wk = st.w[kk][2];
            const float weight = wiwj * wk;
            float q[3];
#pragma unroll
            for (int a = 0; a < 3; a++) q[a] = kk == 0 ? qij[a] : qij[a] + (float)kk * qz[a];
            const int c = cell_addr(st.base[0] + i, st.base[1] + j, st.base[2] + kk, S.nb);
            const float4 vo = vout_at(S, V, st.base[0] + i, st.base[1] + j, st.base[2] + kk);
            const float v0 = vo.x, v1 = vo.y, v2 = vo.z;
            float* dst = gg_out + c;
            unsafeAtomicAdd(dst, weight * q[0]);
            unsafeAtomicAdd(dst + S.ncell, weight * q[1]);
            unsafeAtomicAdd(dst + 2 * S.ncell, weight * q[2]);
            const float sdot = v0 * q[0] + v1 * q[1] + v2 * q[2];
            const float w3 = wiwj * wk;
            nvw[0] += w3 * v0; nvw[1] += w3 * v1; nvw[2] += w3 * v2;
            const float t = wk * sdot;
            gfx[0] += dwiwj * t;
            gfx[1] += widwj * t;
            gfx[2] += wiwj * (stencil_dw(st, kk, 2) * sdot);
        }
    }
#pragma unroll
    for (int b = 0; b < 3; b++) gfx[b] -= c4 * (nvw[0] * g.C.a[0][b] + nvw[1] * g.C.a[1][b] + nvw[2] * g.C.a[2][b]);
    pstore(Gc, Gc.A0, s, make_float4(g.x[0] + S.inv_dx * gfx[0], g.x[1] + S.inv_dx * gfx[1], g.x[2] + S.inv_dx * gfx[2], 0.f));
}

template <bool GPRE = false>
__device__ __forceinline__ void g2p_grad_slot_global(const SimP& S, const FrameV& cur, const FrameV& Gn, const FrameV& Gc, int s,
                                                     const VoutSrc& V, float* gg_out, const AgentP& agent, int f, const GridStore& GS, const PState* gpre = nullptr) {
    if (!cur.used[s]) return;
    float4 a0 = cur.A0[s];
    float x[3] = {a0.x, a0.y, a0.z};
    Stencil st;
    stencil_make(x, S.inv_dx, st);
    if (!stencil_inside(st, S.n)) {
        if (GPRE) Gc.A0[s] = make_float4(gpre->x[0], gpre->x[1], gpre->x[2], 0.f);
        else { float4 gx = Gn.A0[s]; Gc.A0[s] = make_float4(gx.x, gx.y, gx.z, 0.f); }
        return;
    }
    used_particle_g2p_grad<GPRE>(S, Gn, Gc, s, st, V, gg_out, gpre);
    for (int bx = st.base[0] >> 2; bx <= (st.base[0] + 2) >> 2; bx++)
        for (int by = st.base[1] >> 2; by <= (st.base[1] + 2) >> 2; by++)
// ... 202 lines not shown
        gfx[1] -= nvw[0] * qy[0] + nvw[1] * qy[1] + nvw[2] * qy[2];
        gfx[2] -= nvw[0] * qz[0] + nvw[1] * qz[1] + nvw[2] * qz[2];
        if (live && primary) pstore(Gc, Gc.A0, s, make_float4(g.x[0] + S.inv_dx * gfx[0], g.x[1] + S.inv_dx * gfx[1], g.x[2] + S.inv_dx * gfx[2], 0.f));
    }
    NODE_FENCE();
    float inv = 1.f;
    if (QUAD) {
        asm volatile("s_waitcnt lgkmcnt(0)" ::: "memory");
        int* acc = (int*)acc3 + tofs;
        for (int l = threadIdx.x & 63; l < 3 * TILE_N / 4; l += 64) ((int4*)acc)[l] = make_int4(0, 0, 0, 0);
        asm volatile("" ::: "memory");
        float b = 0.f;
#pragma unroll
        for (int a = 0; a < 3; a++) b = fmaxf(b, fabsf(qb[a]) + 2.f * (fabsf(qx[a]) + fabsf(qy[a]) + fabsf(qz[a])));
        const FixScale fs = fix_scale(wave_max(live ? b : 0.f));
        inv = __any(live && !(b <= 3.4e38f)) ? __int_as_float(0x7fc00000) : fs.inv;
#pragma unroll
        for (int a = 0; a < 3; a++) { qb[a] *= fs.s; qx[a] *= fs.s; qy[a] *= fs.s; qz[a] *= fs.s; }
    }
    Stencil sw = st;
    int l0s = l0;
    if (G == 1 && S.wsort) {
        int key = live ? lb : 0x3ff;
        if (wave_needs_sort(key)) {
            const int dest = wave_sort_dest(key);
            wave_send(dest, key);
#pragma unroll
            for (int a = 0; a < 3; a++) {
                wave_send(dest, qb[a]); wave_send(dest, qx[a]); wave_send(dest, qy[a]); wave_send(dest, qz[a]);
#pragma unroll
                for (int b = 0; b < 3; b++) wave_send(dest, sw.w[a][b]);
            }
            live = key != 0x3ff; lb = live ? key : 0; l0s = tofs + lb;
        }
    }
    const SegScan sc = seg_setup(live ? lb + (G > 1 ? gofs << 10 : 0) : (0x40000000 | (int)threadIdx.x));
    const bool issue = sc.tail && live;
    const float livef = live ? 1.f : 0.f;
#pragma unroll UNR_X
    for (int ii = 0; ii < NI; ii++) {
        const int i = G > 1 ? gi : ii;
        const float lwi = livef * ((G > 1 || MINW >= 4) ? STW(sw, i, 0) : sw.w[ii][0]);
#pragma unroll
        for (int jj = 0; jj < NJ; jj++) {
            const int j = G == 9 ? gj : jj;
            const float lw = lwi * (G == 9 ? STW(sw, j, 1) : sw.w[jj][1]);
            float qij[3];
#pragma unroll
            for (int a = 0; a < 3; a++) qij[a] = qb[a] + (float)i * qx[a] + (float)j * qy[a];
#pragma unroll
            for (int kk = 0; kk < 3; kk++) {
                const float weight = lw * sw.w[kk][2];
                float c0 = weight * (qij[0] + (float)kk * qz[0]), c1 = weight * (qij[1] + (float)kk * qz[1]), c2 = weight * (qij[2] + (float)kk * qz[2]);
                seg_scan3(sc, c0, c1, c2);
                if (issue) {
                    const int l = l0s + ((G > 1 ? 0 : ii) * TILE_T + (G == 9 ? 0 : jj)) * TILE_T + kk;
                    if (QUAD) {
                        int* acc = (int*)acc3;
                        atomicAdd(acc + l, fix_round(c0));
                        atomicAdd(acc + TILE_N + l, fix_round(c1));
                        atomicAdd(acc + 2 * TILE_N + l, fix_round(c2));
                    } else {
                        atomicAdd(&acc3[l], (double)c0);
                        atomicAdd(&acc3[TILE_N + l], (double)c1);
                        atomicAdd(&acc3[2 * TILE_N + l], (double)c2);
                    }
                }
            }
        }
    }
    return inv;
}
template <int MINW, bool QUAD, int AR = 0>
__device__ __forceinline__ float g2p_grad_particle2_split(const SimP& S, const FrameV& Gn, const FrameV& Gc, int s, int lb, const Stencil& st,
                                                          bool live, int tofs, const float* gt, const LaneSplit& ls, const PState* gpre = nullptr) {
    if (ls.G == 1) return g2p_grad_particle2<MINW, QUAD, 1, AR>(S, Gn, Gc, s, lb, st, live, tofs, gt, 0, true, gpre);
    if (ls.G == 3) return g2p_grad_particle2<MINW, QUAD, 3, AR>(S, Gn, Gc, s, lb, st, live, tofs, gt, ls.gofs, ls.primary, gpre);
    return g2p_grad_particle2<MINW, QUAD, 9, AR>(S, Gn, Gc, s, lb, st, live, tofs, gt, ls.gofs, ls.primary, gpre);
}
template <int MINW>
__device__ __forceinline__ void g2p_grad2_body(SimP S, float* fr_cur, float* Gn_, float* Gc_, TableP T,
                                                  const float4* __restrict__ g_out, float* gg_out, float4* slab, int* slow,
                                                  GridStore GS, int f, AgentP agent) {
    const int tid = threadIdx.x;
    const bool stored = GS.cap > 0 && GS.flag[f];
    VoutSrc V; V.g_out = g_out; V.store = stored ? GS.data + (size_t)f * GS.cap * GS_BLK : nullptr; V.blk_slot = T.blk_slot;
    FrameV cur = frame_view(fr_cur, S.Np);
    FrameV Gn = frame_view(Gn_, S.Np), Gc = frame_view(Gc_, S.Np, S.wt & 4);
    TL(S, 0);
    Unit un = unit_load(T, blockIdx.x);
    const int n_slots = T.meta[5];
    bool prev_quad = false;
    for (int wg = blockIdx.x; wg < n_slots; wg += gridDim.x) {
        if (wg != (int)blockIdx.x) un = unit_load(T, wg);
        if (un.a.z == -2) continue;
        if (un.a.z >= 0) {
            const PairCtx pc = unit_ctx(un);
            unit_enter(pc.quad, prev_quad);
            const int4 it = pc.it;
            const TileO to = tile_origin(it.x);
            const int tofs = pc.ti * 3 * TILE_N;
            const int wbase = pc.quad ? 0 : (pc.i & 64);
            const int cnt = __builtin_amdgcn_readfirstlane(min(64, max(0, it.z - wbase)));
            const LaneSplit ls = lane_split(cnt, (S.lsplit & 2) != 0);
            const int i = wbase + ls.p;
            const bool has = ls.ok && i < it.z;
            const int s = it.y + (has ? i : 0);
            const int nbr_entry = neighbour_entry(T.blk_slot, S.nb, it.x);
            const int u0 = cur.used[s];
            const float4 a00 = cur.A0[s];
            float* gt = pc.quad ? (float*)s_acc3 + tofs : s_tile3 + tofs;
            float inv = 1.f;
            bool wshell = false;
            if (FE_LEAN_QUADS && pc.quad && V.store) {
                const bool u_ = has && u0 != 0;
                const int l0_ = (int)(a00.x * S.inv_dx - 0.5f) - to.ox, l1_ = (int)(a00.y * S.inv_dx - 0.5f) - to.oy, l2_ = (int)(a00.z * S.inv_dx - 0.5f) - to.oz;
                const bool in_ = u_ && (unsigned)l0_ <= TILE_T - 3 && (unsigned)l1_ <= TILE_T - 3 && (unsigned)l2_ <= TILE_T - 3;
                wshell = __any(in_ && ((l0_ == 0) | (l0_ == 5) | (l1_ == 0) | (l1_ == 5) | (l2_ == 0) | (l2_ == 5)));
                if (pc.live) { if (wshell) g2p_grad_load_tile2(to, S, g_out, V.store, nbr_entry, pc, gt); else quad_load_vout_inner(V.store, nbr_entry, gt); }
            } else {
                g2p_grad_load_tile2(to, S, g_out, V.store, nbr_entry, pc, gt);
                if (!pc.quad && pc.live) for (int l = pc.t0; l < 3 * TILE_N; l += pc.nth) s_acc3[tofs + l] = 0.0;
            }
            unit_sync(pc.quad);
            TL(S, 2);
            {
                const bool used = has && u0 != 0;
                float x[3] = {0.f, 0.f, 0.f};
                if (used) { x[0] = a00.x; x[1] = a00.y; x[2] = a00.z; }
                Stencil st;
                stencil_make(x, S.inv_dx, st);
                const bool inside = used && stencil_inside(st, S.n);
                const int lb = inside ? tile_base(to, st) : -1;
                const bool live = lb >= 0;
                if (pc.quad && !(FE_LEAN_QUADS && V.store)) wshell = __any(live && stencil_on_shell(lb));
                if (__any(live)) {
                    if (pc.quad) inv = g2p_grad_particle2_split<MINW, true>(S, Gn, Gc, s, live ? lb : 0, st, live, tofs, gt, ls);
                    else g2p_grad_particle2_split<MINW, false>(S, Gn, Gc, s, live ? lb : 0, st, live, tofs, gt, ls);
                } else if (pc.quad && pc.live) {
                    asm volatile("s_waitcnt lgkmcnt(0)" ::: "memory");
                    for (int l = pc.t0; l < 3 * TILE_N; l += pc.nth) ((int*)s_acc3)[tofs + l] = 0;
                }
                g2p_grad_wave_slow(S, Gn, Gc, s, a00, inside && !live && ls.primary, used && !inside && ls.primary, V, gg_out, slow, GS, nullptr, it.x, nbr_entry);
            }
            TL(S, 5);
            unit_sync(pc.quad);
            TL(S, 6);
            if (pc.quad) {
                if (pc.live) quad_handover<3>(S, (const int*)s_acc3 + tofs, inv, inv, slab, pc.slab, gg_out, GS, to, nbr_entry, wshell, S.wt & 4);
            } else if (pc.live) for (int l = pc.t0; l < TILE_N; l += pc.nth)
                tile_handover<3>(S, slab, pc.slab, gg_out, GS, to, nbr_entry, l,
                                 make_float4((float)s_acc3[tofs + l], (float)s_acc3[tofs + TILE_N + l], (float)s_acc3[tofs + 2 * TILE_N + l], 0.f), S.wt & 4);
            unit_sync(pc.quad);
            TL(S, 7);
        } else {
            const int s = un.a.y + tid;
            if (s < S.N) g2p_grad_slot_global(S, cur, Gn, Gc, s, V, gg_out, agent, f, GS);
        }
    }
}
template <int MINW>
__global__ FE_KALIGN __launch_bounds__(WG, MINW) void k_g2p_grad2(SimP S, float* fr_cur, float* Gn_, float* Gc_, TableP T, const float4* g_out, float* gg_out, float4* slab, int* slow, GridStore GS, int f, AgentP agent) { g2p_grad2_body<MINW>(S, fr_cur, Gn_, Gc_, T, g_out, gg_out, slab, slow, GS, f, agent); }
template <int MINW>
__global__ FE_KALIGN __launch_bounds__(WG, MINW) void k_g2p_grad2_b(Batch<G2PGradArgs> B) { const G2PGradArgs& A = B.a[blockIdx.y]; g2p_grad2_body<MINW>(A.S, A.fr_cur, A.Gn_, A.Gc_, A.T, A.g_out, A.gg_out, A.slab, A.slow, A.GS, A.f, A.agent); }


__device__ __forceinline__ float row_sum(float v) {
    v += __shfl_xor(v, 8, 64); v += __shfl_xor(v, 4, 64); v += __shfl_xor(v, 2, 64); v += __shfl_xor(v, 1, 64);
    return v;
}
template <bool NODE>
__device__ __forceinline__ void collide_chain_grad_row(const SimP& S, const AgentP& agent, int f, const float x[3], const float nv0[3],
                                                       float g[3], float gx[3], int sub) {
    const int row0 = (threadIdx.x & 63) & ~15;
    const float sdt = NODE ? 0.f : S.dt;
    float nv[3] = {nv0[0], nv0[1], nv0[2]};
    float vin[FE_MAX_EFF][3];
#pragma unroll
    for (int ei = 0; ei < FE_MAX_EFF; ei++) {
        if (ei < agent.n && agent.e[ei].has_mesh) {
            const EffP& e = agent.e[ei];
            vin[ei][0] = nv[0]; vin[ei][1] = nv[1]; vin[ei][2] = nv[2];
            const float pos[3] = {x[0] + sdt * nv[0], x[1] + sdt * nv[1], x[2] + sdt * nv[2]};
            if (pos[1] > agent.collide_min_y) {
                float out[3];
                t_dynamic_collide<float>(e.mesh, e.pos + f * 3, e.quat + f * 4, e.pos + (f + 1) * 3, e.quat + (f + 1) * 4, pos, nv, S.dt, out);
                nv[0] = out[0]; nv[1] = out[1]; nv[2] = out[2];
            }
        }
    }
#pragma unroll
    for (int ei = FE_MAX_EFF - 1; ei >= 0; ei--) {
        if (!(ei < agent.n && agent.e[ei].has_mesh)) continue;
        const EffP& e = agent.e[ei];
        const float v[3] = {vin[ei][0], vin[ei][1], vin[ei][2]};
        if (!(x[1] + sdt * v[1] > agent.collide_min_y)) continue;
        const int dir = sub;
        Dual p0[3], q0[4], p1[3], q1[4], pos[3], mv[3], out[3];
#pragma unroll
        for (int d = 0; d < 3; d++) {
            p0[d] = Dual(e.pos[f * 3 + d], dir == 3 + d ? 1.f : 0.f);
            p1[d] = Dual(e.pos[(f + 1) * 3 + d]);
            mv[d] = Dual(v[d], dir == d ? 1.f : 0.f);
            pos[d] = Dual(x[d] + sdt * v[d]);
        }
#pragma unroll
        for (int d = 0; d < 4; d++) {
            q0[d] = Dual(e.quat[f * 4 + d], dir == 6 + d ? 1.f : 0.f);
            q1[d] = Dual(e.quat[(f + 1) * 4 + d]);
        }
        const bool hit = t_dynamic_collide<Dual>(e.mesh, p0, q0, p1, q1, pos, mv, S.dt, out);
        if (!hit) continue;
        const float r = dir < 10 ? g[0] * out[0].d + g[1] * out[1].d + g[2] * out[2].d : 0.f;
        float c[3], a[3], gq0[4];
#pragma unroll
        for (int d = 0; d < 3; d++) { c[d] = __shfl(r, row0 + d, 64); a[d] = __shfl(r, row0 + 3 + d, 64); }
#pragma unroll
        for (int d = 0; d < 4; d++) gq0[d] = __shfl(r, row0 + 6 + d, 64);
        const float idt = 1.f / S.dt;
        const float w[3] = {(g[0] - c[0]) * idt, (g[1] - c[1]) * idt, (g[2] - c[2]) * idt};
        float pm[3];
        {
            const float qn = 1.f / sqrtf(e.quat[f * 4] * e.quat[f * 4] + e.quat[f * 4 + 1] * e.quat[f * 4 + 1] + e.quat[f * 4 + 2] * e.quat[f * 4 + 2] + e.quat[f * 4 + 3] * e.quat[f * 4 + 3]);
            const float qi[4] = {e.quat[f * 4] * qn, -e.quat[f * 4 + 1] * qn, -e.quat[f * 4 + 2] * qn, -e.quat[f * 4 + 3] * qn};
            const float rel0[3] = {x[0] + sdt * v[0] - e.pos[f * 3], x[1] + sdt * v[1] - e.pos[f * 3 + 1], x[2] + sdt * v[2] - e.pos[f * 3 + 2]};
            t_quat_rotate(rel0, qi, pm);
        }
        float gq1[4];
#pragma unroll
        for (int k = 0; k < 4; k++) {
            Dual qd[4], pmd[3], rot[3];
            for (int d = 0; d < 4; d++) qd[d] = Dual(e.quat[(f + 1) * 4 + d], d == k ? 1.f : 0.f);
            for (int d = 0; d < 3; d++) pmd[d] = Dual(pm[d]);
            t_quat_rotate(pmd, qd, rot);
            gq1[k] = w[0] * rot[0].d + w[1] * rot[1].d + w[2] * rot[2].d;
        }
#pragma unroll
        for (int d = 0; d < 3; d++) {
            const float gpos = -a[d] - w[d];
            if (!NODE) gx[d] += gpos;
            g[d] = c[d] + sdt * gpos;
            if (sub == 0) { atomicAdd(&s_pose[ei * 14 + d], a[d]); atomicAdd(&s_pose[ei * 14 + 7 + d], w[d]); }
        }
        if (sub == 0) {
#pragma unroll
            for (int d = 0; d < 4; d++) { atomicAdd(&s_pose[ei * 14 + 3 + d], gq0[d]); atomicAdd(&s_pose[ei * 14 + 10 + d], gq1[d]); }
        }
    }
}

__device__ void collide_grad_row(const SimP& S, const AgentP& agent, int f, const FrameV& cur, const FrameV& Gn, const VoutSrc& V, int s, int sub) {
    const float4 a0 = cur.A0[s];
    const float x[3] = {a0.x, a0.y, a0.z};
    Stencil st;
    stencil_make(x, S.inv_dx, st);
    const float4 g0 = Gn.A0[s], g1 = Gn.A1[s];
    float g[3] = {g0.w + S.dt * g0.x, g1.x + S.dt * g0.y, g1.y + S.dt * g0.z};
    float gx[3] = {0.f, 0.f, 0.f};
    if (stencil_inside(st, S.n)) {
        float nv[3] = {0.f, 0.f, 0.f};
        for (int n = sub; n < 27; n += 16) {
            const int i = n / 9, j = (n / 3) % 3, k = n % 3;
            const float weight = STW(st, i, 0) * STW(st, j, 1) * STW(st, k, 2);
            const float4 gv = vout_at(S, V, st.base[0] + i, st.base[1] + j, st.base[2] + k);
            nv[0] += weight * gv.x; nv[1] += weight * gv.y; nv[2] += weight * gv.z;
        }
        nv[0] = row_sum(nv[0]); nv[1] = row_sum(nv[1]); nv[2] = row_sum(nv[2]);
        collide_chain_grad_row<false>(S, agent, f, x, nv, g, gx, sub);
    }
    if (sub == 0) {
        const float nx[3] = {g0.x + gx[0], g0.y + gx[1], g0.z + gx[2]};
        Gn.A0[s] = make_float4(nx[0], nx[1], nx[2], g[0] - S.dt * nx[0]);
        Gn.A1[s] = make_float4(g[1] - S.dt * nx[1], g[2] - S.dt * nx[2], g1.z, g1.w);
    }
}

__global__ __launch_bounds__(256) void k_collide_list(SimP S, float* fr_cur, int f, AgentP agent, int* list, int* count) {
    const int s = blockIdx.x * 256 + threadIdx.x;
    if (s < S.N && frame_view(fr_cur, S.Np).used[s] != 0 && agent.hit[(size_t)f * S.Np + s] != 0) list[atomicAdd(count, 1)] = s;
}
__global__ __launch_bounds__(256) void k_collide_grad(SimP S, float* fr_cur, float* Gn_, const float4* __restrict__ g_out, TableP T,
                                                      GridStore GS, int f, AgentP agent, const int* __restrict__ list, const int* __restrict__ count) {
    const int n = *count;
    if ((int)blockIdx.x * 16 >= n) return;
    const int tid = threadIdx.x;
    if (tid < FE_MAX_EFF * 14) s_pose[tid] = 0.f;
    __syncthreads();
    FrameV cur = frame_view(fr_cur, S.Np), Gn = frame_view(Gn_, S.Np);
    const bool stored = GS.cap > 0 && GS.flag[f];
    VoutSrc V; V.g_out = g_out; V.store = stored ? GS.data + (size_t)f * GS.cap * GS_BLK : nullptr; V.blk_slot = T.blk_slot;
    for (int base = blockIdx.x * 16; base < n; base += gridDim.x * 16) {
        const int idx = base + (tid >> 4);
        if (idx < n) collide_grad_row(S, agent, f, cur, Gn, V, list[idx], tid & 15);
    }
    pose_flush(agent, f);
}

template <bool STATICS, bool DYN>
__device__ __forceinline__ void grid_grad_body(SimP S, TableP T, const float4* __restrict__ slab, float* g_in, float* gg_out, float4* gg_in,
                                                   const int* __restrict__ blk_list, const int* __restrict__ blk_count, int* blk_flag,
                                                   GridStore GS, int f, StaticsP ST, AgentP agent, NodeWork* work, int* work_count) {
    const int lane = threadIdx.x & 63, wave = __builtin_amdgcn_readfirstlane(threadIdx.x >> 6);
    const int es = static_entry(wave);
    const bool es_ok = es < S.nb * S.nb * S.nb;
    const int blk_s = es_ok ? T.active[es] : 0;
    const unsigned char lv_st = (es_ok && es < GS.cap) ? GS.live[(size_t)f * GS.cap + es] : (unsigned char)0, lv_cur = es_ok ? GS.cur[es] : (unsigned char)0;
    const unsigned char drt_s = es_ok ? GS.dirty[es] : (unsigned char)0;
    const int2 nbr_s = es_ok ? nbr_record(T, es, lane) : make_int2(0, 0);
    const bool stored = GS.cap > 0 && GS.flag[f];
    const int n_static = T.meta[2], n_dyn = *blk_count;
    auto one_block = [&](int e, int b, bool is_static, bool dirty, const int2 nbr) {
        const int c = (b << 6) | lane;
        const int bi = b / (S.nb * S.nb), bj = (b / S.nb) % S.nb, bk = b % S.nb;
        const float4 gi = stored ? GS.data[((size_t)f * GS.cap + e) * GS_BLK + lane]
                                 : make_float4(g_in[c], g_in[S.ncell + c], g_in[2 * S.ncell + c], g_in[3 * S.ncell + c]);
        float4 go = make_float4(0.f, 0.f, 0.f, 0.f);
        if (dirty) go = make_float4(gg_out[c], gg_out[S.ncell + c], gg_out[2 * S.ncell + c], 0.f);
        if (is_static) { const float4 t = gather_slabs<3>(slab, nbr, lane); go.x += t.x; go.y += t.y; go.z += t.z; }
        float4 out = make_float4(0.f, 0.f, 0.f, 0.f);
        if (gi.w > FE_EPS) {
            float vo[3], kmul[3];
            float trace[FE_MAX_STATICS][3];
            const int ni = bi * 4 + (lane >> 4), nj = bj * 4 + ((lane >> 2) & 3), nk = bk * 4 + (lane & 3);
            bool dyn_hit = false;
            node_velocity<STATICS, DYN>(S, ST, gi, ni, nj, nk, vo, kmul, trace, &agent, f, nullptr, &dyn_hit);
            float inv = 1.f / gi.w;
            float gcol[3] = {go.x * kmul[0], go.y * kmul[1], go.z * kmul[2]};
            if (DYN && dyn_hit && (gcol[0] != 0.f || gcol[1] != 0.f || gcol[2] != 0.f)) {
                NodeWork w; w.c = c; w.ni = ni; w.nj = nj; w.nk = nk; w.gi = gi; w.go[0] = go.x; w.go[1] = go.y; w.go[2] = go.z; w.pad = 0.f;
                work[atomicAdd(work_count, 1)] = w;
                gcol[0] = gcol[1] = gcol[2] = 0.f;
            }
            if (STATICS) node_statics_grad(S, ST, ni, nj, nk, trace, gcol);
            float g0 = gcol[0], g1 = gcol[1], g2 = gcol[2];
            out.x = g0 * inv; out.y = g1 * inv; out.z = g2 * inv;
            out.w = -(gi.x * g0 + gi.y * g1 + gi.z * g2) * inv * inv;
        }
        gg_in[c] = out;
        if (!stored) { g_in[c] = 0.f; g_in[S.ncell + c] = 0.f; g_in[2 * S.ncell + c] = 0.f; g_in[3 * S.ncell + c] = 0.f; }
        if (dirty) { gg_out[c] = 0.f; gg_out[S.ncell + c] = 0.f; gg_out[2 * S.ncell + c] = 0.f; }
        if (lane == 0 && !is_static) blk_flag[b] = 0;
    };
    const unsigned char* __restrict__ live = stored ? GS.live + (size_t)f * GS.cap : GS.cur;
    if (n_static <= 4 * (int)gridDim.x) {
        if (es < n_static && (stored ? lv_st : lv_cur) != 0) one_block(es, blk_s, true, drt_s == GS.stamp, nbr_s);
    } else {
        const int W = 4 * (int)gridDim.x;
        for (int e0 = es; e0 < n_static; e0 += 8 * W) {
            unsigned lm = 0, dm = 0;
#pragma unroll
            for (int k = 0; k < 8; k++) {
                const int e = e0 + k * W;
                const bool ok = e < n_static;
                const unsigned char l = ok ? live[e] : (unsigned char)0, d = ok ? GS.dirty[e] : (unsigned char)0;
                lm |= (l != 0 ? 1u : 0u) << k; dm |= (d == GS.stamp ? 1u : 0u) << k;
            }
            lm = __builtin_amdgcn_readfirstlane(lm); dm = __builtin_amdgcn_readfirstlane(dm);
            unsigned todo = lm;
            int k = todo ? __builtin_ctz(todo) : -1;
            int blk = k >= 0 ? T.active[e0 + k * W] : 0;
            int2 nbr = k >= 0 ? nbr_record(T, e0 + k * W, lane) : make_int2(0, 0);
            while (k >= 0) {
                todo &= todo - 1;
                const int k_next = todo ? __builtin_ctz(todo) : -1;
                const int blk_next = k_next >= 0 ? T.active[e0 + k_next * W] : 0;
                const int2 nbr_next = k_next >= 0 ? nbr_record(T, e0 + k_next * W, lane) : make_int2(0, 0);
                one_block(e0 + k * W, blk, true, (dm >> k) & 1, nbr);
                k = k_next; blk = blk_next; nbr = nbr_next;
            }
        }
    }
    for (int d = blockIdx.x * 4 + wave; d < n_dyn; d += gridDim.x * 4) one_block(0, blk_list[d], false, true, make_int2(0, 0));
}
struct GridGradArgs { SimP S; TableP T; const float4* slab; float* g_in; float* gg_out; float4* gg_in; const int* blk_list; const int* blk_count; int* blk_flag; GridStore GS; int f; StaticsP ST; AgentP agent; NodeWork* work; int* work_count; };
template <bool STATICS, bool DYN>
__global__ FE_KALIGN __launch_bounds__(256, (STATICS || DYN) ? 2 : 4) void k_grid_grad(SimP S, TableP T, const float4* slab, float* g_in, float* gg_out, float4* gg_in, const int* blk_list, const int* blk_count, int* blk_flag, GridStore GS, int f, StaticsP ST, AgentP agent, NodeWork* work, int* work_count) { grid_grad_body<STATICS, DYN>(S, T, slab, g_in, gg_out, gg_in, blk_list, blk_count, blk_flag, GS, f, ST, agent, work, work_count); }
template <bool STATICS, bool DYN>
__global__ FE_KALIGN __launch_bounds__(256, (STATICS || DYN) ? 2 : 4) void k_grid_grad_b(Batch<GridGradArgs> B) { const GridGradArgs& A = B.a[blockIdx.y]; grid_grad_body<STATICS, DYN>(A.S, A.T, A.slab, A.g_in, A.gg_out, A.gg_in, A.blk_list, A.blk_count, A.blk_flag, A.GS, A.f, A.ST, A.agent, A.work, A.work_count); }


template <bool STATICS>
__global__ __launch_bounds__(256) void k_grid_collide_grad(SimP S, float4* gg_in, int f, StaticsP ST, AgentP agent, const NodeWork* __restrict__ work,
                                                           const int* __restrict__ work_count) {
    const int n = *work_count;
    if ((int)blockIdx.x * 16 >= n) return;
    const int tid = threadIdx.x;
    if (tid < FE_MAX_EFF * 14) s_pose[tid] = 0.f;
    __syncthreads();
    const int sub = tid & 15;
    for (int base = blockIdx.x * 16; base < n; base += gridDim.x * 16) {
    const int idx = base + (tid >> 4);
    if (idx < n) {
        const NodeWork w = work[idx];
        float vo[3], kmul[3], vdyn[3];
        float trace[FE_MAX_STATICS][3];
        node_velocity<STATICS, true>(S, ST, w.gi, w.ni, w.nj, w.nk, vo, kmul, trace, &agent, f, vdyn);
        float gcol[3] = {w.go[0] * kmul[0], w.go[1] * kmul[1], w.go[2] * kmul[2]};
        const float xn[3] = {(float)w.ni * S.dx, (float)w.nj * S.dx, (float)w.nk * S.dx};
        collide_chain_grad_row<true>(S, agent, f, xn, vdyn, gcol, nullptr, sub);
        if (STATICS) node_statics_grad(S, ST, w.ni, w.nj, w.nk, trace, gcol);
        const float inv = 1.f / w.gi.w;
        if (sub == 0)
            gg_in[w.c] = make_float4(gcol[0] * inv, gcol[1] * inv, gcol[2] * inv, -(w.gi.x * gcol[0] + w.gi.y * gcol[1] + w.gi.z * gcol[2]) * inv * inv);
    }
    }
    pose_flush(agent, f);
}

__device__ void effector_move_grad(const EffP& e, int f) {
    float xin[3] = {e.pos[f * 3] + e.v[f * 3], e.pos[f * 3 + 1] + e.v[f * 3 + 1], e.pos[f * 3 + 2] + e.v[f * 3 + 2]};
    float xn[3], J[3][3];
    boundary_x(e.bnd, xin, xn, J);
    for (int d = 0; d < 3; d++) {
        float g = J[0][d] * e.gpos[(f + 1) * 3] + J[1][d] * e.gpos[(f + 1) * 3 + 1] + J[2][d] * e.gpos[(f + 1) * 3 + 2];
        atomicAdd(&e.gpos[f * 3 + d], g);
        e.gv[f * 3 + d] += g;
    }
    const float gq[4] = {e.gquat[(f + 1) * 4], e.gquat[(f + 1) * 4 + 1], e.gquat[(f + 1) * 4 + 2], e.gquat[(f + 1) * 4 + 3]};
    if (gq[0] != 0.f || gq[1] != 0.f || gq[2] != 0.f || gq[3] != 0.f) {
#pragma unroll 1
        for (int dir = 0; dir < 7; dir++) {
            Dual w[3], q[4], out[4];
            for (int d = 0; d < 3; d++) w[d] = Dual(e.w[f * 3 + d], dir == d ? 1.f : 0.f);
            for (int d = 0; d < 4; d++) q[d] = Dual(e.quat[f * 4 + d], dir == 3 + d ? 1.f : 0.f);
            t_move_quat<Dual>(w, q, out);
            const float c = gq[0] * out[0].d + gq[1] * out[1].d + gq[2] * out[2].d + gq[3] * out[3].d;
            if (dir < 3) e.gw[f * 3 + dir] += c; else atomicAdd(&e.gquat[f * 4 + dir - 3], c);
        }
    }
}

struct GradDst {
    FrameV G; const int* __restrict__ to_slot; const int* __restrict__ pid_of_slot;
    __device__ __forceinline__ int slot(int s) const { return to_slot ? to_slot[pid_of_slot[s]] : s; }
};
template <bool TILE, bool GENERAL, bool PRE = false, bool NOSTASH = false, int G = 1, int AR = 0, bool KEEP = false>
__device__ __forceinline__ void used_particle_p2g_grad(const SimP& S, const FrameV& cur, const FrameV& Gn, const FrameV& Gc, int s,
                                                       const float4* __restrict__ info_, const TileO& to,
                                                       const float4* __restrict__ gg_in, int* slow, int tofs, const P2GRaw& pre, const GradDst& D, const float* tl = nullptr,
                                                       int gofs = 0, bool primary = true, PState* keep = nullptr) {
    PState p;
    PInfo info;
    if (PRE) { p = pre.p; info = pre.info; }
    else { load_xvC(cur, s, p); load_F(cur, s, p.F); info = load_info(S, info_, s); }
    Constitutive k;
    constitutive_eval_t<GENERAL>(p.C, p.F, S.dt, info.mu, info.lam, info.mass, info.cls, S.stress_scale, k);
    Stencil st;
    stencil_make(p.x, S.inv_dx, st);
    const bool inside = stencil_inside(st, S.n);
    const int lb = (TILE && inside) ? tile_base(to, st) : -1;
    if (TILE && inside && lb < 0) {
        if (!primary && !KEEP) return;
        if (primary) atomicAdd(slow, 1);
        used_particle_p2g_grad<false, GENERAL, false, NOSTASH, 1, AR, KEEP>(S, cur, Gn, Gc, s, info_, to, gg_in, slow, 0, pre, D, nullptr, 0, primary, keep);
        return;
    }
    float* stash = Stash<GENERAL, AR>::at();
    int col = threadIdx.x;
    if (!NOSTASH) {
#pragma unroll
        for (int a = 0; a < 3; a++)
// ... 86 lines not shown
    asm volatile("" : "+v"(s));
    const int sd = D.slot(s);
    {
        asm volatile("" : "+v"(col));
        if (NOSTASH) { PState q2; load_xvC(cur, s, q2); p.C = q2.C; load_F(cur, s, p.F); }
        else {
#pragma unroll
        for (int a = 0; a < 3; a++)
#pragma unroll
            for (int b = 0; b < 3; b++) {
                p.C.a[a][b] = stash[(a * 3 + b) * WG + col]; p.F.a[a][b] = stash[(9 + a * 3 + b) * WG + col];
                if (GENERAL) { k.U.a[a][b] = stash[(18 + a * 3 + b) * WG + col]; k.V.a[a][b] = stash[(27 + a * 3 + b) * WG + col]; }
            }
        }
        m3 IdtC = m3_scale(p.C, S.dt);
        IdtC.a[0][0] += 1.f; IdtC.a[1][1] += 1.f; IdtC.a[2][2] += 1.f;
        k.Ft = m3_mul(IdtC, p.F);
        if (!GENERAL) k.J = m3_det(k.Ft);
    }
    m3 Fg2; load_F(Gn, s, Fg2);
    const float4 gc0 = Gc.A0[s];
    float gx[3] = {gc0.x + gxs[0], gc0.y + gxs[1], gc0.z + gxs[2]};
    float gvv[3] = {info.mass * Gv[0], info.mass * Gv[1], info.mass * Gv[2]};
    m3 gC, gF;
    constitutive_grad_t<GENERAL>(p.C, p.F, S.dt, info.mu, info.lam, info.mass, info.cls, S.stress_scale, k, GA, Fg2, gC, gF);
    if (KEEP) {
#pragma unroll
        for (int a = 0; a < 3; a++) {
            keep->x[a] = gx[a]; keep->v[a] = gvv[a];
#pragma unroll
            for (int b = 0; b < 3; b++) keep->C.a[a][b] = gC.a[a][b];
        }
        if (primary) store_F(D.G, sd, gF);
        return;
    }
    if (G > 1 && !primary) return;
    store_xvC(D.G, sd, gx, gvv, gC);
    store_F(D.G, sd, gF);
}

template <bool TILE, bool GENERAL, bool PRE = false, bool NOSTASH = false, int G = 1, int AR = 0, bool KEEP = false>
__device__ __forceinline__ bool slot_p2g_grad(const SimP& S, const FrameV& cur, const FrameV& Gn, const FrameV& Gc, int s, const TableP& T,
                                              const int* __restrict__ pool_idx,
                                              const TileO& to, const float4* __restrict__ gg_in, int* slow, const AgentP& agent,
                                              const InjectP& inj, int f, int tofs, int used, const P2GRaw& pre, const GradDst& D, const float* tl = nullptr,
                                              int gofs = 0, bool primary = true, PState* keep = nullptr) {
    if (!PRE) used = cur.used[s];
    if (used) { used_particle_p2g_grad<TILE, GENERAL, PRE, NOSTASH, G, AR, KEEP>(S, cur, Gn, Gc, s, T.info, to, gg_in, slow, tofs, pre, D, tl, gofs, primary, keep); return true; }
    if ((G > 1 || KEEP) && !primary) return false;
    bool injected = false;
    if (!(KEEP && TILE) && inj.on) { const int j = pool_idx[T.pid_of_slot[s]] - inj.act_id; injected = j >= 0 && j < inj.flux; }
    FrameV Gn_f = Gn, Dg_f = D.G;
    if (!injected) Gn_f.iso = 0;
    Dg_f.iso = 0;
    PState g; load_xvC(Gn, s, g); load_F(Gn_f, s, g.F);
    if (Gn_f.iso == 2) { const float t = g.F.a[2][2] * (1.f / 3.f); g.F.a[0][0] = g.F.a[1][1] = g.F.a[2][2] = t; }
    const int sd = D.slot(s);
    store_xvC(D.G, sd, g.x, g.v, g.C); store_F(Dg_f, sd, g.F);
    if (!(KEEP && TILE) && inj.on) {
        int j = pool_idx[T.pid_of_slot[s]] - inj.act_id;
        if (j >= 0 && j < inj.flux) {
            const EffP& e = agent.e[agent.inj];
            float* gp = e.gpos + f * 3;
            atomicAdd(gp + 0, g.x[0]); atomicAdd(gp + 1, g.x[1]); atomicAdd(gp + 2, g.x[2]);
#pragma unroll 1
            for (int k = 0; k < 4; k++) {
                Dual q[4], ip[3], iv[3], rp[3], rv[3];
                for (int d = 0; d < 4; d++) q[d] = Dual(e.quat[f * 4 + d], d == k ? 1.f : 0.f);
                for (int d = 0; d < 3; d++) { ip[d] = Dual(e.inject_p[d]); iv[d] = Dual(e.inject_v[d]); }
                t_quat_rotate(ip, q, rp); t_quat_rotate(iv, q, rv);
                const float c = g.x[0] * rp[0].d + g.x[1] * rp[1].d + g.x[2] * rp[2].d + g.v[0] * rv[0].d + g.v[1] * rv[1].d + g.v[2] * rv[2].d;
                if (c != 0.f) atomicAdd(&e.gquat[f * 4 + k], c);
            }
        }
    }
    return false;
}

template <bool GENERAL, int MINW>
__device__ __forceinline__ void p2g_grad_body(SimP S, float* fr_cur, float* Gn_, float* Gc_, TableP T,
                                                 const int* __restrict__ pool_idx,
                                                 const float4* __restrict__ gg_in, int* blk_count, int* slow, AgentP agent,
                                                 InjectP inj, int act, int f, float* Gd_, const int* __restrict__ to_slot, int fiso) {
    const int tid = threadIdx.x;
    if (blockIdx.x == 0 && tid == 0) {
        *blk_count = 0;
        if (act) for (int i = agent.n - 1; i >= 0; i--) effector_move_grad(agent.e[i], f);
    }
    FrameV cur = frame_view(fr_cur, S.Np, 0, (!GENERAL && (fiso & 1)) ? 1 : 0);
    FrameV Gn = frame_view(Gn_, S.Np, 0, (!GENERAL && (fiso & 2)) ? 2 : 0), Gc = frame_view(Gc_, S.Np, S.wt & 8);
    const GradDst D = {frame_view(Gd_, S.Np, S.wt & 8, (!GENERAL && (fiso & 4)) ? 2 : 0), to_slot, T.pid_of_slot};
    TL(S, 0);
    constexpr bool QLIST = !GENERAL;
    Unit un = unit_load<!QLIST>(T, blockIdx.x);
    bool useq = QLIST;
    if (QLIST) {
        const Unit un_p = unit_load<true>(T, blockIdx.x);
        useq = T.meta[16] != 0;
        if (!useq) un = un_p;
    }
    const int n_slots = T.meta[useq ? 5 : 9];
    bool prev_quad = false;
    for (int wg = blockIdx.x; wg < n_slots; wg += gridDim.x) {
        if (wg != (int)blockIdx.x) { if (useq) un = unit_load<false>(T, wg); else un = unit_load<true>(T, wg); }
        if (un.a.z == -2) continue;
        if (QLIST && un.a.z >= 0 && (un.a.w & QUAD_BIT)) {
            const PairCtx pc = unit_ctx(un);
            unit_enter(true, prev_quad);
            const int4 it = pc.it;
            const TileO to = tile_origin(it.x);
            float* tl = pc.ti < 2 ? s_tile + pc.ti * 4 * TILE_N : s_stash_l + (pc.ti - 2) * 4 * TILE_N;
            if (pc.live) tile_nodes_n<8>(pc.t0, 64, [&](int l) { return tile_node_load(to, S, gg_in, l); },
                                         [&](int l, const float4 v) { tl[l] = v.x; tl[TILE_N + l] = v.y; tl[2 * TILE_N + l] = v.z; tl[3 * TILE_N + l] = v.w; });
            unit_sync(true);
            P2GRaw no_pre;
            {
                const LaneSplit ls = lane_split(__builtin_amdgcn_readfirstlane(min(64, it.z)), FE_SPLIT_PGG && (S.lsplit & 4) != 0);
                const int i = ls.p;
                if (ls.ok && i < it.z) {
                    if (ls.G == 1) slot_p2g_grad<true, GENERAL, false, true, 1>(S, cur, Gn, Gc, it.y + i, T, pool_idx, to, gg_in, slow, agent, inj, f, 0, 0, no_pre, D, tl);
                    else if (ls.G == 3) slot_p2g_grad<true, GENERAL, false, true, 3>(S, cur, Gn, Gc, it.y + i, T, pool_idx, to, gg_in, slow, agent, inj, f, 0, 0, no_pre, D, tl, ls.gofs, ls.primary);
                    else slot_p2g_grad<true, GENERAL, false, true, 9>(S, cur, Gn, Gc, it.y + i, T, pool_idx, to, gg_in, slow, agent, inj, f, 0, 0, no_pre, D, tl, ls.gofs, ls.primary);
                }
            }
            unit_sync(true);
            continue;
        }
        if (un.a.z >= 0) {
            const PairCtx pc = QLIST ? unit_ctx(un) : pair_ctx(un);
            if (QLIST) unit_enter(false, prev_quad);
            const int4 it = pc.it;
            const TileO to = tile_origin(it.x);
            TL(S, 1);
            load_tile4(to, S, gg_in, pc);
            __syncthreads();
            TL(S, 2);
            P2GRaw no_pre;
            {
                const int wbase = pc.i & 64;
                const LaneSplit ls = lane_split(__builtin_amdgcn_readfirstlane(min(64, max(0, it.z - wbase))), FE_SPLIT_PGG && !GENERAL && (S.lsplit & 4) != 0);
                const int i = wbase + ls.p, tofs = pc.ti * 4 * TILE_N;
                if (ls.ok && i < it.z) {
                    if (GENERAL || ls.G == 1) slot_p2g_grad<true, GENERAL, false, false, 1>(S, cur, Gn, Gc, it.y + i, T, pool_idx, to, gg_in, slow, agent, inj, f, tofs, 0, no_pre, D);
                    else if (ls.G == 3) slot_p2g_grad<true, GENERAL, false, false, 3>(S, cur, Gn, Gc, it.y + i, T, pool_idx, to, gg_in, slow, agent, inj, f, tofs, 0, no_pre, D, nullptr, ls.gofs, ls.primary);
                    else slot_p2g_grad<true, GENERAL, false, false, 9>(S, cur, Gn, Gc, it.y + i, T, pool_idx, to, gg_in, slow, agent, inj, f, tofs, 0, no_pre, D, nullptr, ls.gofs, ls.primary);
                }
            }
            TL(S, 3);
            __syncthreads();
            TL(S, 4);
        } else {
            if (QLIST) unit_enter(false, prev_quad);
            const int s = un.a.y + tid;
            TileO none = {0, 0, 0};
            P2GRaw none_pre;
            if (s < S.N) slot_p2g_grad<false, GENERAL, false>(S, cur, Gn, Gc, s, T, pool_idx, none, gg_in, slow, agent, inj, f, 0, 0, none_pre, D);
        }
    }
}
struct P2GGradArgs { SimP S; float* fr_cur; float* Gn_; float* Gc_; TableP T; const int* pool_idx; const float4* gg_in; int* blk_count; int* slow; AgentP agent; InjectP inj; int act; int f; float* Gd_; const int* to_slot; int fiso; };
template <bool GENERAL, int MINW>
__global__ FE_KALIGN __launch_bounds__(WG, MINW) void k_p2g_grad(SimP S, float* fr_cur, float* Gn_, float* Gc_, TableP T, const int* pool_idx, const float4* gg_in, int* blk_count, int* slow, AgentP agent, InjectP inj, int act, int f, float* Gd_, const int* to_slot, int fiso) { p2g_grad_body<GENERAL, MINW>(S, fr_cur, Gn_, Gc_, T, pool_idx, gg_in, blk_count, slow, agent, inj, act, f, Gd_, to_slot, fiso); }
template <bool GENERAL, int MINW>
__global__ FE_KALIGN __launch_bounds__(WG, MINW) void k_p2g_grad_b(Batch<P2GGradArgs> B) { const P2GGradArgs& A = B.a[blockIdx.y]; p2g_grad_body<GENERAL, MINW>(A.S, A.fr_cur, A.Gn_, A.Gc_, A.T, A.pool_idx, A.gg_in, A.blk_count, A.slow, A.agent, A.inj, A.act, A.f, A.Gd_, A.to_slot, A.fiso); }

struct BwdFuseP { float* fr_prev; float* Gp_; const float4* g_out; float* gg_out; float4* slab; };
template <int MINW, bool GENERAL = false>
__device__ __forceinline__ void p2g_grad_g2p_grad_body(SimP S, float* fr_cur, float* Gn_, float* Gc_, TableP T, const int* __restrict__ pool_idx,
                                                         const float4* __restrict__ gg_in, int* blk_count, int* slow, AgentP agent, InjectP inj, int act, int f,
                                                         int fiso, BwdFuseP B, GridStore GS) {
    const int tid = threadIdx.x;
    if (blockIdx.x == 0 && tid == 0) {
        *blk_count = 0;
        if (act) for (int i = agent.n - 1; i >= 0; i--) effector_move_grad(agent.e[i], f);
    }
    VoutSrc V; V.g_out = B.g_out; V.store = GS.data + (size_t)(f - 1) * GS.cap * GS_BLK; V.blk_slot = T.blk_slot;
    constexpr int AR = GENERAL ? 2 : 1;
    FrameV cur = frame_view(fr_cur, S.Np, 0, (!GENERAL && (fiso & 1)) ? 1 : 0), prev = frame_view(B.fr_prev, S.Np);
    FrameV Gn = frame_view(Gn_, S.Np, 0, (!GENERAL && (fiso & 2)) ? 2 : 0);
    FrameV Gc = frame_view(Gc_, S.Np, S.wt & 8, (!GENERAL && (fiso & 4)) ? 2 : 0);
    FrameV Gp = frame_view(B.Gp_, S.Np, S.wt & 4);
    const GradDst D = {Gc, nullptr, T.pid_of_slot};
    float* const t4 = lds_tile4<AR>();
    double* const acc3 = lds_acc3<AR>();
    const int n_slots = T.meta[GENERAL ? 9 : 5];
    bool prev_quad = false, any_tail = false;
    for (int wg = blockIdx.x; ; wg += gridDim.x) {
        const Unit un = unit_load<GENERAL>(T, wg);
        if (wg >= n_slots) break;
        if (un.a.z == -2) continue;
        if (un.a.z >= 0) {
            const PairCtx pc = GENERAL ? pair_ctx(un) : unit_ctx(un);
            unit_enter(pc.quad, prev_quad);
            const int4 it = pc.it;
            const TileO to = tile_origin(it.x);
            const int wbase = pc.quad ? 0 : (pc.i & 64);
            const int cnt = __builtin_amdgcn_readfirstlane(min(64, max(0, it.z - wbase)));
            const LaneSplit ls = lane_split(cnt, false);
            const int i = wbase + ls.p;
            const bool has = ls.ok && i < it.z;
            const int s = it.y + (has ? i : 0);
            const int nbr_entry = neighbour_entry(T.blk_slot, S.nb, it.x);
            float* tl = t4 + pc.ti * 4 * TILE_N;
            if (pc.live) tile_nodes<!GENERAL>(pc.t0, pc.nth, [&](int l) { return tile_node_load(to, S, gg_in, l); },
                                              [&](int l, const float4 v) { tl[l] = v.x; tl[TILE_N + l] = v.y; tl[2 * TILE_N + l] = v.z; tl[3 * TILE_N + l] = v.w; });
            unit_sync(pc.quad);
            PState g;
            bool kept = false;
            P2GRaw no_pre;
            if (has) {
                if (pc.quad) kept = slot_p2g_grad<true, GENERAL, false, true, 1, AR, true>(S, cur, Gn, Gc, s, T, pool_idx, to, gg_in, slow, agent, inj, f, 0, 0, no_pre, D, tl, 0, ls.primary, &g);
                else kept = slot_p2g_grad<true, GENERAL, false, false, 1, AR, true>(S, cur, Gn, Gc, s, T, pool_idx, to, gg_in, slow, agent, inj, f, pc.ti * 4 * TILE_N, 0, no_pre, D, nullptr, 0, ls.primary, &g);
            }
            if (!kept) {
#pragma unroll
                for (int a = 0; a < 3; a++) { g.x[a] = 0.f; g.v[a] = 0.f; }
                g.C = m3_zero();
            }
            asm volatile("" : "+v"(g.x[0]), "+v"(g.x[1]), "+v"(g.x[2]), "+v"(g.v[0]), "+v"(g.v[1]), "+v"(g.v[2]));
            asm volatile("" : "+v"(g.C.a[0][0]), "+v"(g.C.a[0][1]), "+v"(g.C.a[0][2]), "+v"(g.C.a[1][0]), "+v"(g.C.a[1][1]), "+v"(g.C.a[1][2]), "+v"(g.C.a[2][0]), "+v"(g.C.a[2][1]), "+v"(g.C.a[2][2]));
            unit_sync(pc.quad);
            const int tofs = pc.quad ? pc.ti * 4 * TILE_N - 6 * TILE_N : pc.ti * 3 * TILE_N;
            const int u0 = prev.used[s];
            const float4 a00 = prev.A0[s];
            float* gt = pc.quad ? (float*)acc3 + tofs : lds_tile3<AR>() + tofs;
            g2p_grad_load_tile2<!GENERAL, GENERAL ? 2 : 4>(to, S, B.g_out, V.store, nbr_entry, pc, gt);
            if (!pc.quad && pc.live) for (int l = pc.t0; l < 3 * TILE_N; l += pc.nth) acc3[tofs + l] = 0.0;
            unit_sync(pc.quad);
            float inv = 1.f;
            bool wshell = false;
            {
                const bool used = has && u0 != 0;
                float x[3] = {0.f, 0.f, 0.f};
                if (used) { x[0] = a00.x; x[1] = a00.y; x[2] = a00.z; }
                Stencil st;
                stencil_make(x, S.inv_dx, st);
                const bool inside = used && stencil_inside(st, S.n);
                const int lb = inside ? tile_base(to, st) : -1;
                const bool live = lb >= 0;
                if (has && kept && ls.primary && !inside) store_xvC(Gc, s, g.x, g.v, g.C);
                if (pc.quad) wshell = __any(live && stencil_on_shell(lb));
                if (__any(live)) {
                    if (pc.quad) inv = g2p_grad_particle2<4, true, 1, AR>(S, Gc, Gp, s, live ? lb : 0, st, live, tofs, gt, 0, true, &g);
                    else g2p_grad_particle2<4, false, 1, AR>(S, Gc, Gp, s, live ? lb : 0, st, live, tofs, gt, 0, true, &g);
                } else if (pc.quad && pc.live) {
                    asm volatile("s_waitcnt lgkmcnt(0)" ::: "memory");
                    for (int l = pc.t0; l < 3 * TILE_N; l += pc.nth) ((int*)acc3)[tofs + l] = 0;
                }
                g2p_grad_wave_slow<true>(S, Gc, Gp, s, a00, inside && !live && ls.primary, used && !inside && ls.primary, V, B.gg_out, slow, GS, &g, it.x, nbr_entry);
            }
            unit_sync(pc.quad);
            if (pc.quad) {
                if (pc.live) quad_handover<3>(S, (const int*)acc3 + tofs, inv, inv, B.slab, pc.slab, B.gg_out, GS, to, nbr_entry, wshell, S.wt & 4);
            } else if (pc.live) for (int l = pc.t0; l < TILE_N; l += pc.nth)
                tile_handover<3>(S, B.slab, pc.slab, B.gg_out, GS, to, nbr_entry, l,
                                 make_float4((float)acc3[tofs + l], (float)acc3[tofs + TILE_N + l], (float)acc3[tofs + 2 * TILE_N + l], 0.f), S.wt & 4);
            unit_sync(pc.quad);
        } else any_tail = true;
    }
    if (!any_tail) return;
    __syncthreads();
    for (int wg = blockIdx.x; wg < n_slots; wg += gridDim.x) {
        const Unit un = unit_load<GENERAL>(T, wg);
        if (un.a.z != -1) continue;
        {
            int t_ = tid;
            asm volatile("" : "+v"(t_));
            const int s = un.a.y + t_;
            TileO none = {0, 0, 0};
            P2GRaw none_pre;
            if (s < S.N) {
                PState g;
                const bool kept = slot_p2g_grad<false, GENERAL, false, false, 1, AR, true>(S, cur, Gn, Gc, s, T, pool_idx, none, gg_in, slow, agent, inj, f, 0, 0, none_pre, D, nullptr, 0, true, &g);
                if (kept) {
                    if (!prev.used[s]) store_xvC(Gc, s, g.x, g.v, g.C);
                    else g2p_grad_slot_global<true>(S, prev, Gc, Gp, s, V, B.gg_out, agent, f - 1, GS, &g);
                }
            }
        }
    }
}
struct PggArgs { SimP S; float* fr_cur; float* Gn_; float* Gc_; TableP T; const int* pool_idx; const float4* gg_in; int* blk_count; int* slow; AgentP agent; InjectP inj; int act; int f; int fiso; BwdFuseP B; GridStore GS; };
#ifndef FE_FB_WAVES_LESS
#define FE_FB_WAVES_LESS 0
#endif
template <int MINW, bool GENERAL = false>
__global__ FE_KALIGN __launch_bounds__(WG, MINW - FE_FB_WAVES_LESS) void k_pgg_g2pg(SimP S, float* fr_cur, float* Gn_, float* Gc_, TableP T, const int* pool_idx, const float4* gg_in, int* blk_count, int* slow, AgentP agent, InjectP inj, int act, int f, int fiso, BwdFuseP B, GridStore GS) { p2g_grad_g2p_grad_body<MINW, GENERAL>(S, fr_cur, Gn_, Gc_, T, pool_idx, gg_in, blk_count, slow, agent, inj, act, f, fiso, B, GS); }
template <int MINW>
__global__ FE_KALIGN __launch_bounds__(WG, MINW - FE_FB_WAVES_LESS) void k_pgg_g2pg_b(Batch<PggArgs> Bt) { const PggArgs& A = Bt.a[blockIdx.y]; p2g_grad_g2p_grad_body<MINW>(A.S, A.fr_cur, A.Gn_, A.Gc_, A.T, A.pool_idx, A.gg_in, A.blk_count, A.slow, A.agent, A.inj, A.act, A.f, A.fiso, A.B, A.GS); }


#ifndef SORT_YFAST
#define SORT_YFAST 0
#endif
#define SORT_HB 4096
__device__ __forceinline__ int row_iscan(int x) {
    x += __builtin_amdgcn_update_dpp(0, x, 0x111, 0xf, 0xf, false);
    x += __builtin_amdgcn_update_dpp(0, x, 0x112, 0xf, 0xf, false);
    x += __builtin_amdgcn_update_dpp(0, x, 0x114, 0xf, 0xf, false);
    x += __builtin_amdgcn_update_dpp(0, x, 0x118, 0xf, 0xf, false);
    return x;
}
__device__ __forceinline__ int wave_iscan(int x) {
    x = row_iscan(x);
    x += __builtin_amdgcn_update_dpp(0, x, 0x142, 0xa, 0xf, false);
    x += __builtin_amdgcn_update_dpp(0, x, 0x143, 0xc, 0xf, false);
    return x;
}
__global__ __launch_bounds__(256) void k_sort_count(SimP S, float* fr, int n_pwg, int* key, int* rank, int* cnt, int* bcnt,
                                                    const int* __restrict__ clr_active, const int* __restrict__ clr_meta, int* clr_slot, int* nact) {
    __shared__ int hist[SORT_HB + 1];
    __shared__ int kmin;
    const int tid = threadIdx.x;
    if (blockIdx.x == 0 && tid == 0) *nact = 0;
    if ((int)blockIdx.x >= n_pwg) {
        const int n = clr_meta[2];
        for (int i = (blockIdx.x - n_pwg) * 256 + tid; i < n; i += SORT_CLR_WGS * 256) clr_slot[clr_active[i]] = -1;
        return;
    }
    const int s = blockIdx.x * blockDim.x + tid;
    const bool valid = s < S.N;
    int kk = S.ncell;
    if (valid) {
        FrameV cur = frame_view(fr, S.Np);
        const float4 a0 = cur.A0[s];
        if (cur.used[s]) {
            float x[3] = {a0.x, a0.y, a0.z};
            Stencil st;
            stencil_make(x, S.inv_dx, st);
            if (stencil_inside(st, S.n)) {
                kk = cell_addr(st.base[0], st.base[1], st.base[2], S.nb);
#if SORT_YFAST
                kk = (kk & ~63) | ((st.base[0] & 3) << 4) | ((st.base[2] & 3) << 2) | (st.base[1] & 3);
#endif
            }
        }
    }
    const bool is_tail = kk == S.ncell;
    if (tid == 0) kmin = 0x7fffffff;
    for (int l = tid; l <= SORT_HB; l += 256) hist[l] = 0;
    __syncthreads();
    if (valid && !is_tail) atomicMin(&kmin, kk);
    __syncthreads();
    const int rel = is_tail ? SORT_HB : kk - kmin;
    const bool local = valid && rel <= SORT_HB && (is_tail || rel < SORT_HB);
    int r = 0;
    if (local) r = atomicAdd(&hist[rel], 1);
    else if (valid) r = atomicAdd(&cnt[kk], 1);
    {
        unsigned long long todo = __ballot(valid && !local);
        const int myb = kk >> 6;
        while (todo) {
            const int b = __builtin_amdgcn_readlane(myb, __builtin_ctzll(todo));
            const unsigned long long same = __ballot(valid && !local && myb == b);
            if ((tid & 63) == __builtin_ctzll(todo)) atomicAdd(&bcnt[b], __popcll(same));
            todo &= ~same;
        }
    }
    __syncthreads();
    if (kmin != 0x7fffffff) {
        const int k0 = kmin, base = k0 & ~63, lane = tid & 63;
        for (int j = tid >> 6; j <= SORT_HB / 64; j += 4) {
            const int l = base + j * 64 + lane - k0;
            const int n = wave_iscan((l >= 0 && l < SORT_HB) ? hist[l] : 0);
            if (lane == 63 && n > 0) atomicAdd(&bcnt[(base >> 6) + j], n);
        }
    }
    if (tid == 255 && hist[SORT_HB] > 0) atomicAdd(&bcnt[S.ncell >> 6], hist[SORT_HB]);
    __syncthreads();
    {
// ... 835 lines not shown
    double* tl_partial = nullptr; size_t tl_partial_cap = 0;
    int* tl_cnt = nullptr;
    FeDensitySpec dn_spec[FE_DENSITY_MAX_FIELDS] = {}; double* dn_target[FE_DENSITY_MAX_FIELDS] = {}; bool dn_has_target[FE_DENSITY_MAX_FIELDS] = {};
    unsigned long long* dn_words[FE_TASK_LOSS_MAX_DENSITY_TERMS + 1] = {}; double* dn_r[FE_TASK_LOSS_MAX_DENSITY_TERMS + 1] = {}; size_t dn_cap[FE_TASK_LOSS_MAX_DENSITY_TERMS + 1] = {};
    int tl_n_density = 0;
    int density_lds = -1;
    struct RenderState* render = nullptr;
    int render_lane_pixels = FE_RENDER_LANE_PIXELS;
    int task_pair_chunk = 0;
    bool has_mesh_effector = false; std::vector<float*> mesh_vox;
    bool has_rigid = false; int n_bodies = 0;
    RigidBody* bodies_dev = nullptr;
    int* body_start = nullptr; int* body_pids = nullptr;
    int *blk_flag = nullptr, *blk_list = nullptr, *blk_count = nullptr, *err_dev = nullptr;
    float* stage_r = nullptr; int* stage_i = nullptr;
    unsigned char* node_mark = nullptr; unsigned long long* counters = nullptr;
    std::vector<EffHost> effs;
    EffP* effs_dev = nullptr;
    int loss_steps = 0; float *tgt = nullptr, *chamfer = nullptr, *step_loss = nullptr;
    size_t bytes = 0;
    std::string err;
    hipEvent_t ev_t0 = nullptr, ev_t1 = nullptr, ev_batch = nullptr;
    hipStream_t own_stream = nullptr;
    bool prof_on = false;
    std::vector<hipEvent_t> prof_ev; std::vector<int> prof_kid; size_t prof_used = 0;
    double prof_ms[KID_COUNT] = {0}; long long prof_n[KID_COUNT] = {0};
#ifdef FE_TIMELINE
    unsigned long long* tl_dev = nullptr;
#endif

    float* frame(int f) { return frame_ptr[f]; }
    float*& spare_frame() { return frame_ptr[L + 1]; }
    float* grad(int f) { return grad_ptr[f & 1]; }
    size_t grad_words() const { return (size_t)GR_WORDS * Np + Np; }
    TableP tableP(int id) const { TableP t; t.pid_of_slot = tables[id].pid; t.info = tables[id].info; t.meta = tables[id].meta; t.active = tables[id].active; t.blk_slot = tables[id].blk_slot; t.units = tables[id].units; t.units_p = tables[id].units_p; t.units_cap = (int)units_cap; t.nbr = tables[id].nbr; t.arrive = tables[id].arrive; return t; }
    int* expected_of(int id) const { return (int*)(tables[id].arrive + (size_t)nb * nb * nb); }
    const int* pid_of(int f) const { return tables[tbl_of_frame[f]].pid; }
};

static std::string g_create_err;

static hipError_t hipMemcpyOnStream(FeEngine* h, void* dst, const void* src, size_t bytes, hipMemcpyKind kind);

#define FAIL(h, msg) do { (h)->err = (msg); return 1; } while (0)
#define FE_ENTRY(h) do { if ((h) != nullptr) (void)hipSetDevice((h)->device); } while (0)
#define HIPCK(h, call) do { hipError_t e_ = (call); if (e_ != hipSuccess) { (h)->err = std::string(#call) + ": " + hipGetErrorString(e_); return 1; } } while (0)
#define CHECK_FRAME(h, f) do { if ((f) < 0 || (f) > (h)->L) FAIL(h, "frame index out of range"); } while (0)
#define CHECK_EFF(h, e) do { if ((e) < 0 || (e) >= (int)(h)->effs.size()) FAIL(h, "effector index out of range"); } while (0)

static hipError_t hipMemcpyOnStream(FeEngine* h, void* dst, const void* src, size_t bytes, hipMemcpyKind kind) {
    hipError_t e = hipMemcpyAsync(dst, src, bytes, kind, h->stream);
    if (e != hipSuccess) return e;
    return hipStreamSynchronize(h->stream);
}

namespace {

template <typename T>
int dev_alloc(FeEngine* h, T** p, size_t count, bool zero = true) {
    size_t bytes = count * sizeof(T);
    if (bytes == 0) bytes = sizeof(T);
    HIPCK(h, hipMalloc((void**)p, bytes));
    if (zero) HIPCK(h, hipMemsetAsync(*p, 0, bytes, h->stream));
    h->bytes += bytes;
    return 0;
}

BoundaryP to_boundary(const FeBoundary& b) {
    BoundaryP r;
    r.type = b.type;
    for (int i = 0; i < 3; i++) { r.lower[i] = b.lower[i]; r.upper[i] = b.upper[i]; }
    r.cx = b.xz_center[0]; r.cz = b.xz_center[1]; r.radius = b.xz_radius; r.restitution = b.restitution; r.lock_dims = b.lock_dims;
    return r;
}

AgentP agent_params(FeEngine* h) {
    AgentP a; a.n = (int)h->effs.size(); a.inj = 0; a.e = h->effs_dev; a.collide_min_y = h->collide_min_y;
    a.collector = h->has_collector ? h->collector_dev : nullptr; a.collector_mat = h->collector_mat;
    a.hit = h->hit_dev;
    for (size_t i = 0; i < h->effs.size(); i++) if (h->effs[i].p.type == FE_EFF_INJECTOR) a.inj = (int)i;
    return a;
}

inline dim3 pgrid(FeEngine* h) { return dim3((h->N + 255) / 256); }
inline dim3 wgrid(FeEngine* h) { int g = (h->N + 63) / 64 + 8; if (g < 512) g = 512; return dim3(g < h->wgrid_cap ? g : h->wgrid_cap); }
inline dim3 wgrid_g2p(FeEngine* h) { int g = (h->N + 63) / 64 + 8; if (g < 512) g = 512; return dim3(g < h->wgrid_cap_g2p ? g : h->wgrid_cap_g2p); }
inline dim3 wgrid_pgg(FeEngine* h) { int g = (h->N + 63) / 64 + 8; if (g < 512) g = 512; return dim3(g < h->wgrid_cap_pgg ? g : h->wgrid_cap_pgg); }
inline dim3 ggrid(FeEngine* h) { return dim3(fe_grid_launch_fixed(h->nb * h->nb * h->nb, h->ggrid_cap)); }
inline dim3 ggrid_list(FeEngine* h, int t, int f, bool fwd) {
    const int blocks = h->nb * h->nb * h->nb;
    long long hint = -1; int kind = FE_GL_NONE;
    if (h->grid_list_launch) {
        if (h->grid_hint_force >= 0) { hint = h->grid_hint_force; kind = FE_GL_FORCED; }
        else if (h->len_host && t > 0 && (size_t)t < h->len_slots) {
            const unsigned mine = h->tbl_serial[t];
            const unsigned long long w = __atomic_load_n(h->len_host + t, __ATOMIC_RELAXED);
            if (mine != 0u && mine > h->hint_floor_serial && (unsigned)(w >> 32) == mine) { hint = (long long)(unsigned)w; kind = FE_GL_EXACT; }
            else if (fwd) {
                for (unsigned i = 0; i < 32u && i < h->sort_ring_n; i++) {
                    const FeEngine::SortRef& r = h->sort_ring[(h->sort_ring_n - 1u - i) % 32u];
                    if (r.serial <= h->hint_floor_serial) break;
                    const unsigned long long v = __atomic_load_n(h->len_host + r.t, __ATOMIC_RELAXED);
                    if ((unsigned)(v >> 32) == r.serial) { hint = (long long)(unsigned)v; kind = FE_GL_LAGGED; break; }
                }
            }
        }
    }
    const int g = fe_grid_launch_wgs(hint, h->grid_hint_margin, kind != FE_GL_LAGGED, blocks, h->ggrid_cap, h->grid_one_cap);
    FeEngine::GridLaunchRec& rec = (fwd ? h->gl_fwd : h->gl_bwd)[f];
    rec.wgs = g; rec.hint = (int)hint; rec.kind = kind;
    return dim3(g);
}

void prof_drain(FeEngine* h);
void prof_begin(FeEngine* h, int kid) {
#ifdef FE_TIMELINE
    if (!h->tl_dev) { (void)hipMalloc((void**)&h->tl_dev, sizeof(unsigned long long) * KID_COUNT * TL_WGS * 9); }
    h->S.tl = h->tl_dev + (size_t)kid * TL_WGS * 9;
    (void)hipMemsetAsync(h->S.tl, 0, sizeof(unsigned long long) * TL_WGS * 9, h->stream);
#endif
    if (!h->prof_on) return;
    if (h->prof_used >= 8192) prof_drain(h);
    if (h->prof_used + 2 > h->prof_ev.size()) {
        for (int i = 0; i < 256; i++) { hipEvent_t e; (void)hipEventCreate(&e); h->prof_ev.push_back(e); }
    }
    h->prof_kid.push_back(kid);
    (void)hipEventRecord(h->prof_ev[h->prof_used++], h->stream);
}
void prof_end(FeEngine* h) {
    if (!h->prof_on) return;
    (void)hipEventRecord(h->prof_ev[h->prof_used++], h->stream);
}
void prof_drain(FeEngine* h) {
    if (h->prof_used == 0) return;
    (void)hipStreamSynchronize(h->stream);
    for (size_t i = 0; i + 1 < h->prof_used; i += 2) {
        float ms = 0;
        (void)hipEventElapsedTime(&ms, h->prof_ev[i], h->prof_ev[i + 1]);
        int kid = h->prof_kid[i / 2];
        h->prof_ms[kid] += ms; h->prof_n[kid]++;
    }
    h->prof_used = 0; h->prof_kid.clear();
}

int find_injector(FeEngine* h) {
    for (size_t i = 0; i < h->effs.size(); i++) if (h->effs[i].p.type == FE_EFF_INJECTOR) return (int)i;
    return -1;
}

int make_inject(FeEngine* h, int f, int f_global, int act, bool forward, InjectP& inj) {
    inj.on = 0; inj.act_id = 0; inj.row = 0; inj.flux = 0;
    int ie = find_injector(h);
    if (ie < 0) return 0;
    EffHost& E = h->effs[ie];
    if (!act || (h->inject_till >= 0 && f_global >= h->inject_till)) {
        if (forward) E.act_id[f + 1] = E.act_id[f];
        return 0;
    }
    if (E.act_range.empty()) FAIL(h, "injector has no act_range");
    int row = E.p.locally_random ? f : f_global;
    if (row < 0 || row >= E.p.random_length) FAIL(h, "injector random_vector row out of range");
    if (forward) {
        if (E.act_id[f] + E.p.flux > (int)E.act_range.size()) FAIL(h, "too many particles added");
        E.act_id[f + 1] = E.act_id[f] + E.p.flux;
    }
    inj.on = 1; inj.act_id = E.act_id[f]; inj.row = row; inj.flux = E.p.flux;
// ... 44 lines not shown
int use_static_table(FeEngine*, int) { return 0; }

inline int quad_max(FeEngine* h) { return h->quad; }
int sort_frame(FeEngine* h, int f) {
    if (f <= h->last_sorted_f) h->tbl_bank ^= 1;
    h->last_sorted_f = f;
    const int id_new = 1 + f + h->tbl_bank * (h->L + 1), id_old = h->tbl_of_frame[f];
    if (ensure_table(h, id_new)) return 1;
    for (int slot = 0; slot < 2; slot++)
        if (h->gtbl[slot] == id_new && reorder_grad(h, slot, 0)) return 1;
    FeEngine::Table& tn = h->tables[id_new];
    const int ncell = h->S.ncell;
    const bool fine = h->prof_on && h->prof_fine;
    if (!fine) prof_begin(h, KID_SORT);
    const int n_pwg = (int)pgrid(h).x;
    const int nblk = h->nb * h->nb * h->nb;
    if (fine) prof_begin(h, KID_SORT_COUNT);
    const bool have_keys = h->keys_frame == f && h->sort_scratch_dirty;
    if (!have_keys && h->sort_scratch_dirty) {
        HIPCK(h, hipMemsetAsync(h->sort_cnt, 0, sizeof(int) * ((size_t)ncell + 1), h->stream));
        HIPCK(h, hipMemsetAsync(h->sort_bcnt, 0, sizeof(int) * (size_t)(((nblk + 1 + SORT_BLK_WG - 1) / SORT_BLK_WG) * SORT_BLK_WG), h->stream));
    }
    h->keys_frame = -1; h->sort_scratch_dirty = false;
    if (!have_keys)
    hipLaunchKernelGGL(k_sort_count, dim3(n_pwg + SORT_CLR_WGS), dim3(256), 0, h->stream, h->S, h->frame(f), n_pwg, h->sort_key, h->sort_rank, h->sort_cnt, h->sort_bcnt,
                       tn.active, tn.meta, tn.blk_slot, h->sort_nact);
    if (fine) { prof_end(h); prof_begin(h, KID_SORT_SCAN); }
    const int blk_wgs = (nblk + 1 + SORT_BLK_WG - 1) / SORT_BLK_WG, scan_wgs = (nblk + 63) / 64, act_wgs = (nblk + 255) / 256;
    ListLenOut LL = {nullptr, 0u};
    if ((size_t)id_new < h->len_slots) {
        if (++h->sort_serial == 0u) { h->sort_serial = 1u; h->hint_floor_serial = 0u; std::fill(h->tbl_serial.begin(), h->tbl_serial.end(), 0u); h->sort_ring_n = 0; }
        h->tbl_serial[id_new] = h->sort_serial;
        h->sort_ring[h->sort_ring_n++ % 32] = {id_new, h->sort_serial};
        LL = {h->len_dev + id_new, h->sort_serial};
    }
    if (h->sort_one_scan && blk_wgs <= 2 * h->n_cus) {
        h->scan_ready += blk_wgs; h->scan_act += act_wgs;
        const SortScanSync Y = {h->sort_nact + 1, h->scan_ready, h->sort_nact + 2, h->scan_act, LL};
        hipLaunchKernelGGL(k_sort_blk_scan, dim3(blk_wgs + scan_wgs + act_wgs), dim3(256), 0, h->stream, nblk, h->nb, ncell, h->item_max, h->loose_max, quad_max(h), h->sort_bcnt, h->sort_partial,
                           blk_wgs, scan_wgs, h->sort_cnt, h->sort_start, h->sort_nact, tn.active, tn.blk_slot, tn.items, tn.pairs, tn.singles, tn.singles + h->items_cap, tn.blk_first,
                           h->sort_base, tn.meta, Y);
    } else {
        hipLaunchKernelGGL(k_sort_blk_partial, dim3(blk_wgs + scan_wgs + act_wgs), dim3(256), 0, h->stream, nblk, h->nb, h->item_max, h->loose_max, quad_max(h), h->sort_bcnt, h->sort_partial,
                           blk_wgs, scan_wgs, h->sort_cnt, h->sort_start, h->sort_nact, tn.active, tn.blk_slot);
        hipLaunchKernelGGL(k_sort_blk_final, dim3(blk_wgs), dim3(256), 0, h->stream, nblk, h->nb, ncell, h->item_max, h->loose_max, quad_max(h), h->sort_bcnt, h->sort_cnt, h->sort_start, h->sort_partial,
                           tn.items, tn.pairs, tn.singles, tn.singles + h->items_cap, tn.blk_first, h->sort_base, h->sort_nact, tn.meta, LL);
    }
    if (fine) { prof_end(h); prof_begin(h, KID_SORT_PERM); }
    int* pid_dst = id_old == id_new ? h->sort_pid : tn.pid;
    const UnitsArgs U = {h->sort_bcnt, h->nb, h->S.xcd, h->quad_min_units, h->quad_fit, h->pack_units, h->pgg_quad_min_units, tn.items, tn.pairs, tn.singles, tn.singles + h->items_cap, tn.blk_first, tn.active, tn.meta, tn.units, tn.units_p, (int)h->units_cap, tn.nbr, (h->fuse_grid & 3) ? (int*)(tn.arrive + (size_t)nblk) : (int*)nullptr};
    tn.has_expected = (h->fuse_grid & 3) != 0;
    hipLaunchKernelGGL(k_sort_apply, dim3(n_pwg + SORT_UNIT_WGS), dim3(256), 0, h->stream, h->N, (size_t)h->Np, n_pwg, h->sort_key, h->sort_rank, h->sort_start, h->sort_base,
                       h->tables[id_old].pid, pid_dst, tn.slot_of_pid, h->pinfo, tn.info, h->spare_frame(), h->frame(f), U, h->S.uni, h->fiso[f] ? 1 : 0);
    if (id_old == id_new) HIPCK(h, hipMemcpyAsync(tn.pid, h->sort_pid, sizeof(int) * h->Np, hipMemcpyDeviceToDevice, h->stream));
    prof_end(h);
    std::swap(h->frame_ptr[f], h->spare_frame());
    h->tbl_of_frame[f] = id_new;
    return 0;
}

StaticsP statics_p(FeEngine* h) { StaticsP p; p.n = (int)h->statics_host.size(); p.s = h->statics_dev; return p; }

GridStore grid_store(FeEngine* h) {
    GridStore g; g.data = h->gstore; g.flag = h->gs_flag; g.cap = h->gs_cap;
    g.touched = h->ent_touched; g.dirty = h->ent_dirty; g.live = h->gs_live; g.cur = h->cur_live; g.stamp = (unsigned char)(1 + h->stamp % 255);
    return g;
}

inline int* bcount(FeEngine* h, int f) { return h->blk_count + (f & 1); }
inline float4* gout(FeEngine* h, int f) { return h->g_out + (size_t)(f & 1) * h->S.ncell; }
inline float4* ggin(FeEngine* h, int f) { return h->gg_in + (size_t)(f & 1) * h->S.ncell; }
GridW grid_w(FeEngine* h, int f) {
    GridW g; g.g_in = h->g_in; g.slab = h->slab; g.ncell = h->S.ncell; g.frame_slow = h->frame_slow_dev; g.blk_flag = h->blk_flag; g.blk_list = h->blk_list; g.blk_count = bcount(h, f); g.err = h->err_dev; g.slow = h->slow_dev;
    g.fg = h->fg_dev; g.g_out = gout(h, f);
    return g;
}

inline bool grid_collide(FeEngine* h) { return h->has_mesh_effector && (h->collide_type & 2); }
inline bool particle_collide(FeEngine* h) { return h->has_mesh_effector && (h->collide_type & 1); }

template <bool KEEP>
void launch_grid(FeEngine* h, const TableP& T, int f, const AgentP& ag) {
    const dim3 gg = ggrid_list(h, h->tbl_of_frame[f], f, !KEEP);
#define LAUNCH_GRID(ST_, DY_) hipLaunchKernelGGL(HIP_KERNEL_NAME(k_grid<KEEP, ST_, DY_>), gg, dim3(256), 0, h->stream, h->S, T, h->slab, h->g_in, gout(h, f), \
                           h->blk_list, bcount(h, f), h->blk_flag, grid_store(h), f, h->frame_slow_dev, statics_p(h), ag)
    if (grid_collide(h)) { if (h->statics_host.empty()) LAUNCH_GRID(false, true); else LAUNCH_GRID(true, true); }
    else { if (h->statics_host.empty()) LAUNCH_GRID(false, false); else LAUNCH_GRID(true, false); }
#undef LAUNCH_GRID
}

inline int fwd_iso(FeEngine* h, int f) { return (h->fiso[f] ? 1 : 0) | ((h->all_simple_liquid && h->compact_F) ? 2 : 0); }

inline bool fusable_fwd(FeEngine* h, int f) {
    return h->fuse_g2p && f > 0 && !(h->sort_interval > 0 && f % h->sort_interval == 0) && !particle_collide(h) && !h->has_rigid && !h->has_collector;
}
inline bool fuse_grid_possible(FeEngine* h, int t) {
    return (h->fuse_grid & 3) != 0 && h->sort_interval > 0 && t > 0 && h->loose_max == 0 && h->statics_host.empty() && !h->has_mesh_effector &&
           h->gs_cap == h->nb * h->nb * h->nb && h->tables[t].has_expected;
}
inline bool fuse_grid_ok(FeEngine* h, int f) { return fuse_grid_possible(h, h->tbl_of_frame[f]) && ((h->fuse_grid & 3) >= 2 || !h->tail_used); }
inline void fg_launch_begin(FeEngine* h) { h->S.fg_base = h->fg_started; h->S.fg_nowait = (h->fuse_grid & 4) ? 1 : 0; }
inline void fg_launch_end(FeEngine* h, dim3 grid) { h->fg_started += grid.x; }
int substep_fwd(FeEngine* h, int f, int f_global, int act, bool g2p_pending = false, bool defer_g2p = false) {
    h->gs_host_valid = false;
    h->stamp++;
    InjectP inj;
    if (make_inject(h, f, f_global, act, true, inj)) return 1;
    if (h->sort_interval > 0 && f % h->sort_interval == 0) { if (sort_frame(h, f)) return 1; h->tail_used = false; }
    h->tbl_of_frame[f + 1] = h->tbl_of_frame[f];
    use_static_table(h, h->tbl_of_frame[f]);
    const TableP T = h->tableP(h->tbl_of_frame[f]);
    AgentP ag = agent_params(h);
    const int fiso = fwd_iso(h, f);
    const bool fg = fuse_grid_ok(h, f);
    if (inj.on) h->tail_used = true;
    if (fg) fg_launch_begin(h);
    if (g2p_pending) {
        const FuseP FU = {h->frame(f - 1), gout(h, f - 1), h->slow_dev, bcount(h, f - 1)};
        prof_begin(h, KID_G2P_P2G);
        if (fg) {
            const P2GArgs A = {h->S, h->frame(f), h->frame(f + 1), T, h->pool_idx, grid_w(h, f), ag, inj, act, f, grid_store(h), h->all_simple_liquid ? fiso : 0, FU};
            if (h->all_simple_liquid) hipLaunchKernelGGL((k_g2p_p2g_fg<false>), wgrid(h), dim3(WG), 0, h->stream, A);
            else hipLaunchKernelGGL((k_g2p_p2g_fg<true>), wgrid(h), dim3(WG), 0, h->stream, A);
        } else if (h->all_simple_liquid)
            hipLaunchKernelGGL((k_g2p_p2g<false>), wgrid(h), dim3(WG), 0, h->stream, h->S, h->frame(f), h->frame(f + 1), T,
                               h->pool_idx, grid_w(h, f), ag, inj, act, f, grid_store(h), fiso, FU);
        else
            hipLaunchKernelGGL((k_g2p_p2g<true>), wgrid(h), dim3(WG), 0, h->stream, h->S, h->frame(f), h->frame(f + 1), T,
                               h->pool_idx, grid_w(h, f), ag, inj, act, f, grid_store(h), 0, FU);
        prof_end(h);
    } else {
    prof_begin(h, KID_P2G);
    if (fg) {
        const P2GArgs A = {h->S, h->frame(f), h->frame(f + 1), T, h->pool_idx, grid_w(h, f), ag, inj, act, f, grid_store(h), h->all_simple_liquid ? fiso : 0, FuseP{nullptr, nullptr, nullptr, nullptr}};
        if (h->all_simple_liquid) hipLaunchKernelGGL((k_p2g_fg<false>), wgrid(h), dim3(WG), 0, h->stream, A);
        else hipLaunchKernelGGL((k_p2g_fg<true>), wgrid(h), dim3(WG), 0, h->stream, A);
    } else if (h->all_simple_liquid)
        hipLaunchKernelGGL((k_p2g<true, false>), wgrid(h), dim3(WG), 0, h->stream, h->S, h->frame(f), h->frame(f + 1), T,
                           h->pool_idx, grid_w(h, f), ag, inj, act, f, grid_store(h), fiso);
    else
        hipLaunchKernelGGL((k_p2g<true, true>), wgrid(h), dim3(WG), 0, h->stream, h->S, h->frame(f), h->frame(f + 1), T,
                           h->pool_idx, grid_w(h, f), ag, inj, act, f, grid_store(h), 0);
    prof_end(h);
    }
    if (fg) fg_launch_end(h, wgrid(h));
    h->fiso[f + 1] = (fiso & 2) != 0;
    if (!fg) {
    prof_begin(h, KID_GRID);
    launch_grid<false>(h, T, f, ag);
    prof_end(h);
    }
    if (defer_g2p) return 0;
    prof_begin(h, KID_G2P);
    const bool sortkey = h->sort_keys_in_g2p && h->sort_interval > 0 && (f + 1) % h->sort_interval == 0 && !h->has_rigid;
    if (sortkey) {
        if (h->sort_scratch_dirty) {
            HIPCK(h, hipMemsetAsync(h->sort_cnt, 0, sizeof(int) * ((size_t)h->S.ncell + 1), h->stream));
            HIPCK(h, hipMemsetAsync(h->sort_bcnt, 0, sizeof(int) * (size_t)((((size_t)h->nb * h->nb * h->nb + 1 + SORT_BLK_WG - 1) / SORT_BLK_WG) * SORT_BLK_WG), h->stream));
        }
        const SortKeyP K = {h->sort_key, h->sort_rank, h->sort_cnt, h->sort_bcnt, h->sort_nact};
        if (particle_collide(h))
            hipLaunchKernelGGL(k_g2p_sortkey<true>, wgrid_g2p(h), dim3(WG), 0, h->stream, h->S, h->frame(f), h->frame(f + 1), T, gout(h, f), bcount(h, f), h->slow_dev, ag, f, K);
        else
            hipLaunchKernelGGL(k_g2p_sortkey<false>, wgrid_g2p(h), dim3(WG), 0, h->stream, h->S, h->frame(f), h->frame(f + 1), T, gout(h, f), bcount(h, f), h->slow_dev, ag, f, K);
        h->keys_frame = f + 1; h->sort_scratch_dirty = true;
    } else if (particle_collide(h))
        hipLaunchKernelGGL(k_g2p<true>, wgrid_g2p(h), dim3(WG), 0, h->stream, h->S, h->frame(f), h->frame(f + 1), T, gout(h, f), bcount(h, f), h->slow_dev, ag, f);
    else
        hipLaunchKernelGGL(k_g2p<false>, wgrid_g2p(h), dim3(WG), 0, h->stream, h->S, h->frame(f), h->frame(f + 1), T, gout(h, f), bcount(h, f), h->slow_dev, ag, f);
    prof_end(h);
    if (h->has_rigid) {
        hipLaunchKernelGGL(k_rigid_body<false>, dim3(h->n_bodies), dim3(256), 0, h->stream, h->S, h->frame(f), h->frame(f + 1), (float*)nullptr,
                           h->tables[h->tbl_of_frame[f]].slot_of_pid, h->body_start, h->body_pids, h->bodies_dev);
    }
    return 0;
}

int fetch_gs_flags(FeEngine* h) {
    if (h->gs_cap > 0 && !h->gs_host_valid) {
        h->gs_host.resize(h->L + 1);
        HIPCK(h, hipMemcpyAsync(h->gs_host.data(), h->gs_flag, sizeof(int) * (h->L + 1), hipMemcpyDeviceToHost, h->stream));
        HIPCK(h, hipStreamSynchronize(h->stream));
        h->gs_host_valid = true;
    }
    return 0;
}
inline bool fusable_bwd(FeEngine* h, int f) {
    if (!h->all_simple_liquid && h->fuse_bwd < 2 && h->Np / 256 > 2 * 3 * (size_t)h->n_cus) return false;
    return h->fuse_bwd && f > 0 && h->g2p_grad_v == 3 && (h->p2g_grad_waves >= 4 || !h->all_simple_liquid) && !particle_collide(h) && !h->has_rigid && !h->has_collector &&
           h->tbl_of_frame[f - 1] == h->tbl_of_frame[f] && h->tbl_of_frame[f] >= 0 && h->gs_cap > 0 && h->gs_host_valid && h->gs_host[f - 1] != 0;
}
int substep_bwd(FeEngine* h, int f, int f_global, int act, int next_f = -1, bool compact_out = false, bool g2p_done = false, bool fuse_next = false) {
    InjectP inj;
    if (make_inject(h, f, f_global, act, false, inj)) return 1;
    const int t = h->tbl_of_frame[f];
    if (!g2p_done && h->gpartial[(f + 1) & 1]) FAIL(h, "the adjoint of frame f + 1 is incomplete: a fused fe_step_grad passed it on in registers (only the adjoint of a call's first frame is defined afterwards; option fuse_bwd = 0 keeps every frame's)");
    if (reorder_grad(h, (f + 1) & 1, t)) return 1;
    use_static_table(h, t);
    const TableP T = h->tableP(t);
    AgentP ag = agent_params(h);
    InjectP noinj = {0, 0, 0, 0};
    if (fetch_gs_flags(h)) return 1;
    const bool stored = h->gs_cap > 0 && h->gs_host[f] != 0;
    if (!g2p_done) {
    if (!stored) {
    h->stamp++;
    prof_begin(h, KID_P2G_RE);
    if (h->all_simple_liquid)
        hipLaunchKernelGGL((k_p2g<false, false>), wgrid(h), dim3(WG), 0, h->stream, h->S, h->frame(f), h->frame(f + 1), T,
                           h->pool_idx, grid_w(h, f), ag, noinj, 0, f, grid_store(h), h->fiso[f] ? 1 : 0);
    else
        hipLaunchKernelGGL((k_p2g<false, true>), wgrid(h), dim3(WG), 0, h->stream, h->S, h->frame(f), h->frame(f + 1), T,
                           h->pool_idx, grid_w(h, f), ag, noinj, 0, f, grid_store(h), 0);
    prof_end(h);
    prof_begin(h, KID_GRID_KEEP);
    launch_grid<true>(h, T, f, ag);
    prof_end(h);
    }
    h->stamp++;
    if (h->has_rigid) {
        hipLaunchKernelGGL(k_rigid_body<true>, dim3(h->n_bodies), dim3(256), 0, h->stream, h->S, h->frame(f), h->frame(f + 1), h->grad(f + 1),
                           h->tables[t].slot_of_pid, h->body_start, h->body_pids, h->bodies_dev);
    }
    prof_begin(h, KID_G2P_GRAD);
    if (particle_collide(h)) {
        HIPCK(h, hipMemsetAsync(h->hit_count, 0, sizeof(int), h->stream));
        hipLaunchKernelGGL(k_collide_list, pgrid(h), dim3(256), 0, h->stream, h->S, h->frame(f), f, ag, h->hit_list, h->hit_count);
        hipLaunchKernelGGL(k_collide_grad, dim3(std::min((h->N + 15) / 16, 2048)), dim3(256), 0, h->stream, h->S, h->frame(f), h->grad(f + 1), gout(h, f), T, grid_store(h), f, ag,
                           h->hit_list, h->hit_count);
    }
    if (h->g2p_grad_v == 2) hipLaunchKernelGGL(k_g2p_grad2<3>, wgrid(h), dim3(WG), 0, h->stream, h->S, h->frame(f), h->grad(f + 1), h->grad(f), T, gout(h, f), h->gg_out, h->slab, h->slow_dev, grid_store(h), f, ag);
    else hipLaunchKernelGGL(k_g2p_grad2<4>, wgrid(h), dim3(WG), 0, h->stream, h->S, h->frame(f), h->grad(f + 1), h->grad(f), T, gout(h, f), h->gg_out, h->slab, h->slow_dev, grid_store(h), f, ag);
    prof_end(h);
    }
    prof_begin(h, KID_GRID_GRAD);
    const dim3 ggg = ggrid_list(h, t, f, false);
#define LAUNCH_GRID_GRAD(ST_, DY_) hipLaunchKernelGGL(HIP_KERNEL_NAME(k_grid_grad<ST_, DY_>), ggg, dim3(256), 0, h->stream, h->S, T, h->slab, h->g_in, h->gg_out, \
                           ggin(h, f), h->blk_list, bcount(h, f), h->blk_flag, grid_store(h), f, statics_p(h), ag, h->node_work, h->node_work_count)
    if (grid_collide(h)) {
        if (!h->node_work && (dev_alloc(h, &h->node_work, (size_t)h->S.ncell, false) || dev_alloc(h, &h->node_work_count, 1))) return 1;
        HIPCK(h, hipMemsetAsync(h->node_work_count, 0, sizeof(int), h->stream));
        if (h->statics_host.empty()) LAUNCH_GRID_GRAD(false, true); else LAUNCH_GRID_GRAD(true, true);
        const dim3 wg((unsigned)std::min((h->S.ncell + 15) / 16, 1024));
        if (h->statics_host.empty()) hipLaunchKernelGGL(k_grid_collide_grad<false>, wg, dim3(256), 0, h->stream, h->S, ggin(h, f), f, statics_p(h), ag, h->node_work, h->node_work_count);
        else hipLaunchKernelGGL(k_grid_collide_grad<true>, wg, dim3(256), 0, h->stream, h->S, ggin(h, f), f, statics_p(h), ag, h->node_work, h->node_work_count);
    } else { if (h->statics_host.empty()) LAUNCH_GRID_GRAD(false, false); else LAUNCH_GRID_GRAD(true, false); }
    prof_end(h);
    if (h->param_grad) {
        prof_begin(h, KID_PARAM_GRAD);
        if (h->all_simple_liquid) hipLaunchKernelGGL(k_param_grad<false>, pgrid(h), dim3(256), 0, h->stream, h->S, h->frame(f), T, ggin(h, f), h->fiso[f] ? 1 : 0, (float)h->cfg.p_vol, h->pg_acc);
        else hipLaunchKernelGGL(k_param_grad<true>, pgrid(h), dim3(256), 0, h->stream, h->S, h->frame(f), T, ggin(h, f), 0, (float)h->cfg.p_vol, h->pg_acc);
        prof_end(h);
    }
    const int t_next = (h->fold_reorder && next_f >= 0) ? h->tbl_of_frame[next_f] : t;
    const bool fold = t_next != t && t_next >= 0;
    float* g_dst = fold ? h->grad_ptr[2] : h->grad(f);
    const int* to_slot = fold ? h->tables[t_next].slot_of_pid : nullptr;
    const bool gc_out = compact_out && h->compact_F && h->all_simple_liquid && !h->has_collector;
    const int giso = (h->fiso[f] ? 1 : 0) | (h->gcompact[(f + 1) & 1] ? 2 : 0) | (gc_out ? 4 : 0);
#define LAUNCH_P2G_GRAD(G, W) hipLaunchKernelGGL((k_p2g_grad<G, W>), wgrid_pgg(h), dim3(WG), 0, h->stream, h->S, h->frame(f), h->grad(f + 1), \
                           h->grad(f), T, h->pool_idx, ggin(h, f), bcount(h, f), h->slow_dev, ag, inj, act, f, g_dst, to_slot, giso)
    if (!fuse_next) prof_begin(h, KID_P2G_GRAD);
    if (fuse_next) {
        h->stamp++;
        const BwdFuseP B = {h->frame(f - 1), h->grad(f - 1), gout(h, f - 1), h->gg_out, h->slab};
        prof_begin(h, KID_PGG_G2PG);
        if (h->all_simple_liquid)
            hipLaunchKernelGGL(k_pgg_g2pg<4>, wgrid(h), dim3(WG), 0, h->stream, h->S, h->frame(f), h->grad(f + 1), h->grad(f), T, h->pool_idx, ggin(h, f), bcount(h, f), h->slow_dev,
                               ag, inj, act, f, giso, B, grid_store(h));
        else
            hipLaunchKernelGGL((k_pgg_g2pg<3, true>), wgrid(h), dim3(WG), 0, h->stream, h->S, h->frame(f), h->grad(f + 1), h->grad(f), T, h->pool_idx, ggin(h, f), bcount(h, f), h->slow_dev,
                               ag, inj, act, f, 0, B, grid_store(h));
    } else if (h->all_simple_liquid) {
        if (h->p2g_grad_waves >= 4) LAUNCH_P2G_GRAD(false, 4);
        else if (h->p2g_grad_waves == 3) LAUNCH_P2G_GRAD(false, 3);
        else LAUNCH_P2G_GRAD(false, 2);
    } else LAUNCH_P2G_GRAD(true, 1);
    prof_end(h);
    if (fold) std::swap(h->grad_ptr[2], h->grad_ptr[f & 1]);
    h->gtbl[f & 1] = fold ? t_next : t;
    h->gcompact[f & 1] = gc_out;
    h->gpartial[f & 1] = fuse_next;
    return 0;
}

bool batchable(FeEngine** hs, int B) {
    if (B < 2 || B > FE_MAX_BATCH) return false;
    for (int i = 0; i < B; i++) if (!hs[i]) return false;
    for (int i = 0; i < B; i++) {
        FeEngine* h = hs[i];
        if (h->device != hs[0]->device || h->n != hs[0]->n || h->L != hs[0]->L || h->all_simple_liquid != hs[0]->all_simple_liquid ||
            h->sort_interval != hs[0]->sort_interval || h->p2g_grad_waves != hs[0]->p2g_grad_waves || h->g2p_grad_v != hs[0]->g2p_grad_v || h->S.wt != hs[0]->S.wt || !h->statics_host.empty() || h->has_mesh_effector || h->has_rigid || h->prof_fine ||
            (h->gs_cap > 0) != (hs[0]->gs_cap > 0)) return false;
        for (int j = 0; j < i; j++) if (hs[j] == h) return false;
    }
    return true;
}
inline dim3 wgrid_b(FeEngine** hs, int B) { unsigned g = 0; for (int i = 0; i < B; i++) g = std::max(g, wgrid(hs[i]).x); return dim3(g, B); }

void batch_fork(FeEngine** hs, int B) {
    (void)hipEventRecord(hs[0]->ev_batch, hs[0]->own_stream);
    for (int i = 1; i < B; i++) { (void)hipStreamWaitEvent(hs[i]->own_stream, hs[0]->ev_batch, 0); hs[i]->stream = hs[i]->own_stream; }
}
void batch_join(FeEngine** hs, int B) {
    for (int i = 1; i < B; i++) {
        (void)hipEventRecord(hs[i]->ev_batch, hs[i]->own_stream);
        (void)hipStreamWaitEvent(hs[0]->own_stream, hs[i]->ev_batch, 0);
        hs[i]->stream = hs[0]->own_stream;
    }
}

int substep_fwd_batch(FeEngine** hs, int B, int f, int f_global, int act, bool g2p_pending = false, bool defer_g2p = false) {
    FeEngine* h0 = hs[0];
    Batch<P2GArgs> bp; Batch<GridArgs> bg; Batch<G2PArgs> bq;
    const bool sorting = h0->sort_interval > 0 && f % h0->sort_interval == 0;
    if (sorting) batch_fork(hs, B);
    struct Join { FeEngine** hs; int B; bool on; ~Join() { if (on) batch_join(hs, B); } };
    {
    Join join{hs, B, sorting};
    for (int i = 0; i < B; i++) {
        FeEngine* h = hs[i];
        h->gs_host_valid = false;
        h->stamp++;
        InjectP inj;
        if (make_inject(h, f, f_global, act, true, inj)) return 1;
        if (h->sort_interval > 0 && f % h->sort_interval == 0 && sort_frame(h, f)) return 1;
        h->tbl_of_frame[f + 1] = h->tbl_of_frame[f];
        use_static_table(h, h->tbl_of_frame[f]);
        const TableP T = h->tableP(h->tbl_of_frame[f]);
        const AgentP ag = agent_params(h);
        const int fiso = fwd_iso(h, f);
        bp.a[i] = P2GArgs{h->S, h->frame(f), h->frame(f + 1), T, h->pool_idx, grid_w(h, f), ag, inj, act, f, grid_store(h), h->all_simple_liquid ? fiso : 0,
                           g2p_pending ? FuseP{h->frame(f - 1), gout(h, f - 1), h->slow_dev, bcount(h, f - 1)} : FuseP{nullptr, nullptr, nullptr, nullptr}};
        h->fiso[f + 1] = h->all_simple_liquid && (fiso & 2) != 0;
        bg.a[i] = GridArgs{h->S, T, h->slab, h->g_in, gout(h, f), h->blk_list, bcount(h, f), h->blk_flag, grid_store(h), f, h->frame_slow_dev, statics_p(h), ag};
        bq.a[i] = G2PArgs{h->S, h->frame(f), h->frame(f + 1), T, gout(h, f), bcount(h, f), h->slow_dev, ag, f};
    }
    }
    if (g2p_pending) {
        prof_begin(h0, KID_G2P_P2G);
        if (h0->all_simple_liquid) hipLaunchKernelGGL((k_g2p_p2g_b<false>), wgrid_b(hs, B), dim3(WG), 0, h0->stream, bp);
        else hipLaunchKernelGGL((k_g2p_p2g_b<true>), wgrid_b(hs, B), dim3(WG), 0, h0->stream, bp);
        prof_end(h0);
    } else {
    prof_begin(h0, KID_P2G);
    if (h0->all_simple_liquid) hipLaunchKernelGGL((k_p2g_b<true, false>), wgrid_b(hs, B), dim3(WG), 0, h0->stream, bp);
    else hipLaunchKernelGGL((k_p2g_b<true, true>), wgrid_b(hs, B), dim3(WG), 0, h0->stream, bp);
    prof_end(h0);
    }
    prof_begin(h0, KID_GRID);
    hipLaunchKernelGGL(HIP_KERNEL_NAME(k_grid_b<false, false, false>), dim3(ggrid(h0).x, B), dim3(256), 0, h0->stream, bg);
    prof_end(h0);
    if (defer_g2p) return 0;
    prof_begin(h0, KID_G2P);
// ... 1496 lines not shown
```

Measured before the change: 11770 substep_pairs/s.

## Preload hot kernel arguments and issue head loads before kernel prologue

Moves the pointers and scalars each kernel needs first (unit tables, meta, active/touched/dirty/nbr arrays, grid size) to the front of the argument list, and enables kernarg preloading so they arrive in SGPRs. Each hot kernel issues its first dependent global loads at entry, then places a scheduling barrier, so memory latency overlaps the rest of the prologue. The intent is to shorten per-kernel startup latency across many small launches. The risk is that the extra live registers and the changed signatures touch many launch sites, and that the compiler flag behaves differently across kernels.

Result: faster. 12090 substep_pairs/s, median of 6 (+2.7%).

```diff
diff --git a/__graft_entry__.py b/__graft_entry__.py
--- a/__graft_entry__.py
+++ b/__graft_entry__.py
@@ -5,7 +5,8 @@
 ROOT = os.path.dirname(os.path.abspath(__file__))
 CSRC = os.path.join(ROOT, 'fluidlab_amd', 'csrc')
 HIP_LIB = os.path.join(CSRC, 'libfluidengine_hip.so')
-HIPCC_FLAGS = ['--offload-arch=gfx950', '-O3', '-std=c++17', '-shared', '-fPIC', '-munsafe-fp-atomics', '-fno-slp-vectorize']
+HIPCC_FLAGS = ['--offload-arch=gfx950', '-O3', '-std=c++17', '-shared', '-fPIC', '-munsafe-fp-atomics', '-fno-slp-vectorize',
+               '-mllvm', '-amdgpu-kernarg-preload-count=16']
 
 
 def _hipcc():
diff --git a/fluidlab_amd/csrc/fe_engine.hip b/fluidlab_amd/csrc/fe_engine.hip
--- a/fluidlab_amd/csrc/fe_engine.hip
+++ b/fluidlab_amd/csrc/fe_engine.hip
@@ -384,17 +384,23 @@
     if (prev_quad && !quad) __syncthreads();
     prev_quad = quad;
 }
+struct UnitAsk { int4 a, b, q; };
 template <bool GATHER = false>
-__device__ __forceinline__ Unit unit_load(const TableP& T, int w) {
+__device__ __forceinline__ UnitAsk unit_ask(const TableP& T, int w) {
     const int4* p = (const int4*)((GATHER ? T.units_p : T.units) + (w < T.units_cap ? w : T.units_cap - 1));
-    int4 a = p[0], b = p[1], q = p[__builtin_amdgcn_readfirstlane(threadIdx.x >> 6)];
-    if (w >= T.units_cap) a.z = -2;
+    UnitAsk r = {p[0], p[1], p[__builtin_amdgcn_readfirstlane(threadIdx.x >> 6)]};
+    if (w >= T.units_cap) r.a.z = -2;
+    return r;
+}
+__device__ __forceinline__ Unit unit_take(const UnitAsk& r) {
 #define UNIT_SCALAR(q) make_int4(__builtin_amdgcn_readfirstlane(q.x), __builtin_amdgcn_readfirstlane(q.y), __builtin_amdgcn_readfirstlane(q.z), __builtin_amdgcn_readfirstlane(q.w))
     Unit u;
-    u.a = UNIT_SCALAR(a); u.b = UNIT_SCALAR(b); u.q = UNIT_SCALAR(q);
+    u.a = UNIT_SCALAR(r.a); u.b = UNIT_SCALAR(r.b); u.q = UNIT_SCALAR(r.q);
 #undef UNIT_SCALAR
     return u;
 }
+template <bool GATHER = false>
+__device__ __forceinline__ Unit unit_load(const TableP& T, int w) { return unit_take(unit_ask<GATHER>(T, w)); }
 
 #define FE_MAX_BATCH 8
 #ifndef FE_KALIGN_BYTES
@@ -402,6 +408,9 @@
 #endif
 #define FE_KALIGN __attribute__((aligned(FE_KALIGN_BYTES)))
 template <typename A> struct Batch { A a[FE_MAX_BATCH]; };
+#define HEAD_END(never_negative) do { __builtin_amdgcn_sched_barrier(0); if ((never_negative) < 0) return; } while (0)
+template <typename V>
+__device__ __forceinline__ V head_ask(const V* p, int i) { asm volatile("" : "+v"(i)); return p[i]; }
 
 
 __device__ void effector_move(const EffP& e, int f) {
@@ -977,6 +986,9 @@
 __device__ __forceinline__ void p2g_body(SimP S, float* fr_cur, float* fr_next, TableP T,
                                             const int* __restrict__ pool_idx, GridW G, AgentP agent, InjectP inj, int act, int f,
                                             GridStore GS, int fiso, FuseP FU = FuseP{nullptr, nullptr, nullptr, nullptr}) {
+    const UnitAsk ask0 = unit_ask(T, blockIdx.x);
+    const int n_slots = T.meta[5];
+    HEAD_END(T.units_cap);
     if (!WRITE && GS.cap > 0 && GS.flag[f]) return;
     const int tid = threadIdx.x;
     if (WRITE && blockIdx.x == 0 && tid == 0 && act) {
@@ -993,8 +1005,7 @@
     FrameV nxt = frame_view(fr_next, S.Np, S.wt & 1, (!GENERAL && (fiso & 2)) ? 1 : 0);
     const int slab_wt = FG ? 1 : (S.wt & 1);
     TL(S, 0);
-    Unit un = unit_load(T, blockIdx.x);
-    const int n_slots = T.meta[5];
+    Unit un = unit_take(ask0);
     bool prev_quad = false;
     for (int wg = blockIdx.x; FG || wg < n_slots; wg += gridDim.x) {
         if (FG || wg != (int)blockIdx.x) un = unit_load(T, wg);
@@ -1135,9 +1146,9 @@
 }
 struct P2GArgs { SimP S; float* fr_cur; float* fr_next; TableP T; const int* pool_idx; GridW G; AgentP agent; InjectP inj; int act; int f; GridStore GS; int fiso; FuseP FU; };
 template <bool WRITE, bool GENERAL>
-__global__ FE_KALIGN __launch_bounds__(WG, GENERAL ? 3 : 4) void k_p2g(SimP S, float* fr_cur, float* fr_next, TableP T, const int* pool_idx, GridW G, AgentP agent, InjectP inj, int act, int f, GridStore GS, int fiso) { p2g_body<WRITE, GENERAL>(S, fr_cur, fr_next, T, pool_idx, G, agent, inj, act, f, GS, fiso); }
+__global__ FE_KALIGN __launch_bounds__(WG, GENERAL ? 3 : 4) void k_p2g(const UnitRec* h_units, const int* h_meta, int h_cap, SimP S, float* fr_cur, float* fr_next, TableP T, const int* pool_idx, GridW G, AgentP agent, InjectP inj, int act, int f, GridStore GS, int fiso) { T.units = h_units; T.meta = h_meta; T.units_cap = h_cap; p2g_body<WRITE, GENERAL>(S, fr_cur, fr_next, T, pool_idx, G, agent, inj, act, f, GS, fiso); }
 template <bool GENERAL>
-__global__ FE_KALIGN __launch_bounds__(WG, GENERAL ? 3 : 4) void k_g2p_p2g(SimP S, float* fr_cur, float* fr_next, TableP T, const int* pool_idx, GridW G, AgentP agent, InjectP inj, int act, int f, GridStore GS, int fiso, FuseP FU) { p2g_body<true, GENERAL, true>(S, fr_cur, fr_next, T, pool_idx, G, agent, inj, act, f, GS, fiso, FU); }
+__global__ FE_KALIGN __launch_bounds__(WG, GENERAL ? 3 : 4) void k_g2p_p2g(const UnitRec* h_units, const int* h_meta, int h_cap, SimP S, float* fr_cur, float* fr_next, TableP T, const int* pool_idx, GridW G, AgentP agent, InjectP inj, int act, int f, GridStore GS, int fiso, FuseP FU) { T.units = h_units; T.meta = h_meta; T.units_cap = h_cap; p2g_body<true, GENERAL, true>(S, fr_cur, fr_next, T, pool_idx, G, agent, inj, act, f, GS, fiso, FU); }
 template <typename ARGS>
 __device__ __forceinline__ const ARGS* fg_args_again() {
     const ARGS* p = (const ARGS*)__builtin_amdgcn_kernarg_segment_ptr();
@@ -1270,8 +1281,7 @@
     return acc;
 }
 
-__device__ __forceinline__ int static_entry(int wave) {
-    const int G = gridDim.x;
+__device__ __forceinline__ int static_entry(int wave, int G) {
     if ((G & 127) != 0) return blockIdx.x * 4 + wave;
     const int j = blockIdx.x >> 3;
     return ((j >> 4) * 8 + (blockIdx.x & 7)) * 64 + (j & 15) * 4 + wave;
@@ -1279,16 +1289,22 @@
 template <bool KEEP, bool STATICS, bool DYN>
 __device__ __forceinline__ void grid_body(SimP S, TableP T, const float4* __restrict__ slab, float* g_in, float4* g_out,
                                               const int* __restrict__ blk_list, const int* __restrict__ blk_count, int* blk_flag,
-                                              GridStore GS, int f, int* frame_slow, StaticsP ST, AgentP agent) {
+                                              GridStore GS, int f, int* frame_slow, StaticsP ST, AgentP agent, int nb3, int n_wg) {
     if (KEEP && GS.cap > 0 && GS.flag[f]) return;
     const int lane = threadIdx.x & 63, wave = __builtin_amdgcn_readfirstlane(threadIdx.x >> 6);
+    const int es = static_entry(wave, n_wg);
+    const bool es_ok = es < nb3;
+    const int esc = es_ok ? es : 0;
+    const int blk_l = head_ask(T.active, esc);
+    const unsigned char tch_l = head_ask(GS.touched, esc), drt_l = head_ask(GS.dirty, esc);
+    const int2 nbr_l = T.nbr[esc * 27 + min(lane, 26)];
+    const int n_static_l = head_ask(T.meta, 2), n_dyn_l = head_ask(blk_count, 0);
+    HEAD_END(n_wg);
+    const int n_static = __builtin_amdgcn_readfirstlane(n_static_l), n_dyn = __builtin_amdgcn_readfirstlane(n_dyn_l);
+    const int blk_s = es_ok ? __builtin_amdgcn_readfirstlane(blk_l) : 0;
+    const unsigned char tch_s = es_ok ? tch_l : (unsigned char)0, drt_s = es_ok ? drt_l : (unsigned char)0;
+    const int2 nbr_s = (es_ok && lane < 27) ? nbr_l : make_int2(0, 0);
     TL(S, 0);
-    const int es = static_entry(wave);
-    const bool es_ok = es < S.nb * S.nb * S.nb;
-    const int blk_s = es_ok ? T.active[es] : 0;
-    const unsigned char tch_s = es_ok ? GS.touched[es] : (unsigned char)0, drt_s = es_ok ? GS.dirty[es] : (unsigned char)0;
-    const int2 nbr_s = es_ok ? nbr_record(T, es, lane) : make_int2(0, 0);
-    const int n_static = T.meta[2], n_dyn = *blk_count;
     if (!KEEP && blockIdx.x == 0 && threadIdx.x == 0) {
         if (GS.cap > 0) GS.flag[f] = (n_static <= GS.cap && *frame_slow == 0) ? 1 : 0;
         *frame_slow = 0;
@@ -1322,7 +1338,7 @@
         }
         TL(S, 3);
     };
-    if (n_static <= 4 * (int)gridDim.x) {
+    if (n_static <= 4 * n_wg) {
         if (es < n_static) {
             const bool tm = tch_s == GS.stamp, dm = drt_s == GS.stamp;
             if (lane == 0) {
@@ -1332,7 +1348,7 @@
             if (tm || dm) one_block(es, blk_s, true, tm, dm, nbr_s);
         }
     } else {
-        const int W = 4 * (int)gridDim.x;
+        const int W = 4 * n_wg;
         for (int e0 = es; e0 < n_static; e0 += 8 * W) {
             unsigned tm = 0, dm = 0;
             int blk8[8]; int2 nbr8[8];
@@ -1362,13 +1378,13 @@
             }
         }
     }
-    for (int d = blockIdx.x * 4 + wave; d < n_dyn; d += gridDim.x * 4) one_block(-1, blk_list[d], false, false, true, make_int2(0, 0));
+    for (int d = blockIdx.x * 4 + wave; d < n_dyn; d += n_wg * 4) one_block(-1, blk_list[d], false, false, true, make_int2(0, 0));
 }
 struct GridArgs { SimP S; TableP T; const float4* slab; float* g_in; float4* g_out; const int* blk_list; const int* blk_count; int* blk_flag; GridStore GS; int f; int* frame_slow; StaticsP ST; AgentP agent; };
 template <bool KEEP, bool STATICS, bool DYN>
-__global__ FE_KALIGN __launch_bounds__(256, (STATICS || DYN) ? 2 : 4) void k_grid(SimP S, TableP T, const float4* slab, float* g_in, float4* g_out, const int* blk_list, const int* blk_count, int* blk_flag, GridStore GS, int f, int* frame_slow, StaticsP ST, AgentP agent) { grid_body<KEEP, STATICS, DYN>(S, T, slab, g_in, g_out, blk_list, blk_count, blk_flag, GS, f, frame_slow, ST, agent); }
+__global__ FE_KALIGN __launch_bounds__(256, (STATICS || DYN) ? 2 : 4) void k_grid(const int* h_active, unsigned char* h_touched, unsigned char* h_dirty, const int2* h_nbr, const int* h_meta, const int* blk_count, int nb3, int n_wg, SimP S, TableP T, const float4* slab, float* g_in, float4* g_out, const int* blk_list, int* blk_flag, GridStore GS, int f, int* frame_slow, StaticsP ST, AgentP agent) { T.active = h_active; T.nbr = h_nbr; T.meta = h_meta; GS.touched = h_touched; GS.dirty = h_dirty; grid_body<KEEP, STATICS, DYN>(S, T, slab, g_in, g_out, blk_list, blk_count, blk_flag, GS, f, frame_slow, ST, agent, nb3, n_wg); }
 template <bool KEEP, bool STATICS, bool DYN>
-__global__ FE_KALIGN __launch_bounds__(256, (STATICS || DYN) ? 2 : 4) void k_grid_b(Batch<GridArgs> B) { const GridArgs& A = B.a[blockIdx.y]; grid_body<KEEP, STATICS, DYN>(A.S, A.T, A.slab, A.g_in, A.g_out, A.blk_list, A.blk_count, A.blk_flag, A.GS, A.f, A.frame_slow, A.ST, A.agent); }
+__global__ FE_KALIGN __launch_bounds__(256, (STATICS || DYN) ? 2 : 4) void k_grid_b(Batch<GridArgs> B) { const GridArgs& A = B.a[blockIdx.y]; grid_body<KEEP, STATICS, DYN>(A.S, A.T, A.slab, A.g_in, A.g_out, A.blk_list, A.blk_count, A.blk_flag, A.GS, A.f, A.frame_slow, A.ST, A.agent, A.S.nb * A.S.nb * A.S.nb, (int)gridDim.x); }
 
 __device__ __forceinline__ float4 fg_load16(const void* base, unsigned byte_off) {
     const u32x4 u = __builtin_amdgcn_raw_buffer_load_b128(wt_rsrc((void*)base), (int)byte_off, 0, 16);
@@ -1526,7 +1542,7 @@
     const FgDev* F = A.F;
     int* const ctr = F->ctr;
     const int G_ = gridDim.x, W = 4 * G_;
-    const int es = static_entry(wave);
+    const int es = static_entry(wave, G_);
     const int n_static = T.meta[2];
     const int* __restrict__ expected = (const int*)(T.arrive + S.nb * S.nb * S.nb);
     const int e_l = es + lane * W;
@@ -1722,14 +1738,16 @@
 template <bool COLLIDE, bool SORTKEY = false>
 __device__ __forceinline__ void g2p_body(SimP S, float* fr_cur, float* fr_next, TableP T, const float4* __restrict__ g_out,
                                             int* blk_count, int* slow, AgentP agent, int f, SortKeyP K = SortKeyP{nullptr, nullptr, nullptr, nullptr, nullptr}) {
+    const UnitAsk ask0 = unit_ask<true>(T, blockIdx.x);
+    const int n_slots = T.meta[9];
+    HEAD_END(T.units_cap);
     const int tid = threadIdx.x;
     if (blockIdx.x == 0 && tid == 0) { *blk_count = 0; if (SORTKEY) *K.nact = 0; }
     const int n_wg = gridDim.x;
     FrameV cur = frame_view(fr_cur, S.Np);
     FrameV nxt = frame_view(fr_next, S.Np, S.wt & 2);
     TL(S, 0);
-    Unit un = unit_load<true>(T, blockIdx.x);
-    const int n_slots = T.meta[9];
+    Unit un = unit_take(ask0);
     for (int wg = blockIdx.x; wg < n_slots; wg += n_wg) {
         if (wg != (int)blockIdx.x) un = unit_load<true>(T, wg);
         if (un.a.z == -2) continue;
@@ -1775,9 +1793,9 @@
 }
 struct G2PArgs { SimP S; float* fr_cur; float* fr_next; TableP T; const float4* g_out; int* blk_count; int* slow; AgentP agent; int f; };
 template <bool COLLIDE>
-__global__ FE_KALIGN __launch_bounds__(WG) void k_g2p(SimP S, float* fr_cur, float* fr_next, TableP T, const float4* g_out, int* blk_count, int* slow, AgentP agent, int f) { g2p_body<COLLIDE>(S, fr_cur, fr_next, T, g_out, blk_count, slow, agent, f); }
+__global__ FE_KALIGN __launch_bounds__(WG) void k_g2p(const UnitRec* h_units_p, const int* h_meta, int h_cap, SimP S, float* fr_cur, float* fr_next, TableP T, const float4* g_out, int* blk_count, int* slow, AgentP agent, int f) { T.units_p = h_units_p; T.meta = h_meta; T.units_cap = h_cap; g2p_body<COLLIDE>(S, fr_cur, fr_next, T, g_out, blk_count, slow, agent, f); }
 template <bool COLLIDE>
-__global__ FE_KALIGN __launch_bounds__(WG) void k_g2p_sortkey(SimP S, float* fr_cur, float* fr_next, TableP T, const float4* g_out, int* blk_count, int* slow, AgentP agent, int f, SortKeyP K) { g2p_body<COLLIDE, true>(S, fr_cur, fr_next, T, g_out, blk_count, slow, agent, f, K); }
+__global__ FE_KALIGN __launch_bounds__(WG) void k_g2p_sortkey(const UnitRec* h_units_p, const int* h_meta, int h_cap, SimP S, float* fr_cur, float* fr_next, TableP T, const float4* g_out, int* blk_count, int* slow, AgentP agent, int f, SortKeyP K) { T.units_p = h_units_p; T.meta = h_meta; T.units_cap = h_cap; g2p_body<COLLIDE, true>(S, fr_cur, fr_next, T, g_out, blk_count, slow, agent, f, K); }
 template <bool COLLIDE>
 __global__ FE_KALIGN __launch_bounds__(WG) void k_g2p_b(Batch<G2PArgs> B) { const G2PArgs& A = B.a[blockIdx.y]; g2p_body<COLLIDE>(A.S, A.fr_cur, A.fr_next, A.T, A.g_out, A.blk_count, A.slow, A.agent, A.f); }
 
@@ -2146,14 +2164,16 @@
 __device__ __forceinline__ void g2p_grad2_body(SimP S, float* fr_cur, float* Gn_, float* Gc_, TableP T,
                                                   const float4* __restrict__ g_out, float* gg_out, float4* slab, int* slow,
                                                   GridStore GS, int f, AgentP agent) {
+    const UnitAsk ask0 = unit_ask(T, blockIdx.x);
+    const int n_slots = T.meta[5];
+    HEAD_END(T.units_cap);
     const int tid = threadIdx.x;
     const bool stored = GS.cap > 0 && GS.flag[f];
     VoutSrc V; V.g_out = g_out; V.store = stored ? GS.data + (size_t)f * GS.cap * GS_BLK : nullptr; V.blk_slot = T.blk_slot;
     FrameV cur = frame_view(fr_cur, S.Np);
     FrameV Gn = frame_view(Gn_, S.Np), Gc = frame_view(Gc_, S.Np, S.wt & 4);
     TL(S, 0);
-    Unit un = unit_load(T, blockIdx.x);
-    const int n_slots = T.meta[5];
+    Unit un = unit_take(ask0);
     bool prev_quad = false;
     for (int wg = blockIdx.x; wg < n_slots; wg += gridDim.x) {
         if (wg != (int)blockIdx.x) un = unit_load(T, wg);
@@ -2224,7 +2244,7 @@
     }
 }
 template <int MINW>
-__global__ FE_KALIGN __launch_bounds__(WG, MINW) void k_g2p_grad2(SimP S, float* fr_cur, float* Gn_, float* Gc_, TableP T, const float4* g_out, float* gg_out, float4* slab, int* slow, GridStore GS, int f, AgentP agent) { g2p_grad2_body<MINW>(S, fr_cur, Gn_, Gc_, T, g_out, gg_out, slab, slow, GS, f, agent); }
+__global__ FE_KALIGN __launch_bounds__(WG, MINW) void k_g2p_grad2(const UnitRec* h_units, const int* h_meta, int h_cap, SimP S, float* fr_cur, float* Gn_, float* Gc_, TableP T, const float4* g_out, float* gg_out, float4* slab, int* slow, GridStore GS, int f, AgentP agent) { T.units = h_units; T.meta = h_meta; T.units_cap = h_cap; g2p_grad2_body<MINW>(S, fr_cur, Gn_, Gc_, T, g_out, gg_out, slab, slow, GS, f, agent); }
 template <int MINW>
 __global__ FE_KALIGN __launch_bounds__(WG, MINW) void k_g2p_grad2_b(Batch<G2PGradArgs> B) { const G2PGradArgs& A = B.a[blockIdx.y]; g2p_grad2_body<MINW>(A.S, A.fr_cur, A.Gn_, A.Gc_, A.T, A.g_out, A.gg_out, A.slab, A.slow, A.GS, A.f, A.agent); }
 
@@ -2363,16 +2383,23 @@
 template <bool STATICS, bool DYN>
 __device__ __forceinline__ void grid_grad_body(SimP S, TableP T, const float4* __restrict__ slab, float* g_in, float* gg_out, float4* gg_in,
                                                    const int* __restrict__ blk_list, const int* __restrict__ blk_count, int* blk_flag,
-                                                   GridStore GS, int f, StaticsP ST, AgentP agent, NodeWork* work, int* work_count) {
+                                                   GridStore GS, int f, StaticsP ST, AgentP agent, NodeWork* work, int* work_count,
+                                                   int nb3, int n_wg, const unsigned char* __restrict__ live, bool stored) {
     const int lane = threadIdx.x & 63, wave = __builtin_amdgcn_readfirstlane(threadIdx.x >> 6);
-    const int es = static_entry(wave);
-    const bool es_ok = es < S.nb * S.nb * S.nb;
-    const int blk_s = es_ok ? T.active[es] : 0;
-    const unsigned char lv_st = (es_ok && es < GS.cap) ? GS.live[(size_t)f * GS.cap + es] : (unsigned char)0, lv_cur = es_ok ? GS.cur[es] : (unsigned char)0;
-    const unsigned char drt_s = es_ok ? GS.dirty[es] : (unsigned char)0;
-    const int2 nbr_s = es_ok ? nbr_record(T, es, lane) : make_int2(0, 0);
-    const bool stored = GS.cap > 0 && GS.flag[f];
-    const int n_static = T.meta[2], n_dyn = *blk_count;
+    const int es = static_entry(wave, n_wg);
+    const bool es_ok = es < nb3;
+    const int esc = es_ok ? es : 0;
+    const bool lv_ok = es_ok && (!stored || es < GS.cap);
+    const int blk_l = head_ask(T.active, esc);
+    const unsigned char lv_l = head_ask(live, lv_ok ? es : 0), drt_l = head_ask(GS.dirty, esc);
+    const int2 nbr_l = T.nbr[esc * 27 + min(lane, 26)];
+    const int n_static_l = head_ask(T.meta, 2);
+    HEAD_END(n_wg);
+    const int n_static = __builtin_amdgcn_readfirstlane(n_static_l), n_dyn = *blk_count;
+    const int blk_s = es_ok ? __builtin_amdgcn_readfirstlane(blk_l) : 0;
+    const unsigned char lv_s = lv_ok ? (unsigned char)__builtin_amdgcn_readfirstlane((int)lv_l) : (unsigned char)0;
+    const unsigned char drt_s = es_ok ? drt_l : (unsigned char)0;
+    const int2 nbr_s = (es_ok && lane < 27) ? nbr_l : make_int2(0, 0);
     auto one_block = [&](int e, int b, bool is_static, bool dirty, const int2 nbr) {
         const int c = (b << 6) | lane;
         const int bi = b / (S.nb * S.nb), bj = (b / S.nb) % S.nb, bk = b % S.nb;
@@ -2405,11 +2432,10 @@
         if (dirty) { gg_out[c] = 0.f; gg_out[S.ncell + c] = 0.f; gg_out[2 * S.ncell + c] = 0.f; }
         if (lane == 0 && !is_static) blk_flag[b] = 0;
     };
-    const unsigned char* __restrict__ live = stored ? GS.live + (size_t)f * GS.cap : GS.cur;
-    if (n_static <= 4 * (int)gridDim.x) {
-        if (es < n_static && (stored ? lv_st : lv_cur) != 0) one_block(es, blk_s, true, drt_s == GS.stamp, nbr_s);
+    if (n_static <= 4 * n_wg) {
+        if (es < n_static && lv_s != 0) one_block(es, blk_s, true, drt_s == GS.stamp, nbr_s);
     } else {
-        const int W = 4 * (int)gridDim.x;
+        const int W = 4 * n_wg;
         for (int e0 = es; e0 < n_static; e0 += 8 * W) {
             unsigned lm = 0, dm = 0;
 #pragma unroll
@@ -2434,13 +2460,13 @@
             }
         }
     }
-    for (int d = blockIdx.x * 4 + wave; d < n_dyn; d += gridDim.x * 4) one_block(0, blk_list[d], false, true, make_int2(0, 0));
+    for (int d = blockIdx.x * 4 + wave; d < n_dyn; d += n_wg * 4) one_block(0, blk_list[d], false, true, make_int2(0, 0));
 }
 struct GridGradArgs { SimP S; TableP T; const float4* slab; float* g_in; float* gg_out; float4* gg_in; const int* blk_list; const int* blk_count; int* blk_flag; GridStore GS; int f; StaticsP ST; AgentP agent; NodeWork* work; int* work_count; };
 template <bool STATICS, bool DYN>
-__global__ FE_KALIGN __launch_bounds__(256, (STATICS || DYN) ? 2 : 4) void k_grid_grad(SimP S, TableP T, const float4* slab, float* g_in, float* gg_out, float4* gg_in, const int* blk_list, const int* blk_count, int* blk_flag, GridStore GS, int f, StaticsP ST, AgentP agent, NodeWork* work, int* work_count) { grid_grad_body<STATICS, DYN>(S, T, slab, g_in, gg_out, gg_in, blk_list, blk_count, blk_flag, GS, f, ST, agent, work, work_count); }
+__global__ FE_KALIGN __launch_bounds__(256, (STATICS || DYN) ? 2 : 4) void k_grid_grad(const int* h_active, const unsigned char* h_live, unsigned char* h_dirty, const int2* h_nbr, const int* h_meta, int nb3, int n_wg, int h_cap, int h_stored, SimP S, TableP T, const float4* slab, float* g_in, float* gg_out, float4* gg_in, const int* blk_list, const int* blk_count, int* blk_flag, GridStore GS, int f, StaticsP ST, AgentP agent, NodeWork* work, int* work_count) { T.active = h_active; T.nbr = h_nbr; T.meta = h_meta; GS.dirty = h_dirty; GS.cap = h_cap; grid_grad_body<STATICS, DYN>(S, T, slab, g_in, gg_out, gg_in, blk_list, blk_count, blk_flag, GS, f, ST, agent, work, work_count, nb3, n_wg, h_live, h_stored != 0); }
 template <bool STATICS, bool DYN>
-__global__ FE_KALIGN __launch_bounds__(256, (STATICS || DYN) ? 2 : 4) void k_grid_grad_b(Batch<GridGradArgs> B) { const GridGradArgs& A = B.a[blockIdx.y]; grid_grad_body<STATICS, DYN>(A.S, A.T, A.slab, A.g_in, A.gg_out, A.gg_in, A.blk_list, A.blk_count, A.blk_flag, A.GS, A.f, A.ST, A.agent, A.work, A.work_count); }
+__global__ FE_KALIGN __launch_bounds__(256, (STATICS || DYN) ? 2 : 4) void k_grid_grad_b(Batch<GridGradArgs> B) { const GridGradArgs& A = B.a[blockIdx.y]; grid_grad_body<STATICS, DYN>(A.S, A.T, A.slab, A.g_in, A.gg_out, A.gg_in, A.blk_list, A.blk_count, A.blk_flag, A.GS, A.f, A.ST, A.agent, A.work, A.work_count, A.S.nb * A.S.nb * A.S.nb, (int)gridDim.x, (A.GS.cap > 0 && A.GS.flag[A.f]) ? A.GS.live + (size_t)A.f * A.GS.cap : A.GS.cur, A.GS.cap > 0 && A.GS.flag[A.f]); }
 
 
 template <bool STATICS>
@@ -2693,6 +2719,10 @@
                                                  const int* __restrict__ pool_idx,
                                                  const float4* __restrict__ gg_in, int* blk_count, int* slow, AgentP agent,
                                                  InjectP inj, int act, int f, float* Gd_, const int* __restrict__ to_slot, int fiso) {
+    constexpr bool QLIST = !GENERAL;
+    const UnitAsk ask0 = unit_ask<!QLIST>(T, blockIdx.x), ask0_p = unit_ask<true>(T, blockIdx.x);
+    const int m16 = T.meta[16], m5 = T.meta[5], m9 = T.meta[9];
+    HEAD_END(T.units_cap);
     const int tid = threadIdx.x;
     if (blockIdx.x == 0 && tid == 0) {
         *blk_count = 0;
@@ -2702,15 +2732,14 @@
     FrameV Gn = frame_view(Gn_, S.Np, 0, (!GENERAL && (fiso & 2)) ? 2 : 0), Gc = frame_view(Gc_, S.Np, S.wt & 8);
     const GradDst D = {frame_view(Gd_, S.Np, S.wt & 8, (!GENERAL && (fiso & 4)) ? 2 : 0), to_slot, T.pid_of_slot};
     TL(S, 0);
-    constexpr bool QLIST = !GENERAL;
-    Unit un = unit_load<!QLIST>(T, blockIdx.x);
+    Unit un = unit_take(ask0);
     bool useq = QLIST;
     if (QLIST) {
-        const Unit un_p = unit_load<true>(T, blockIdx.x);
-        useq = T.meta[16] != 0;
+        const Unit un_p = unit_take(ask0_p);
+        useq = m16 != 0;
         if (!useq) un = un_p;
     }
-    const int n_slots = T.meta[useq ? 5 : 9];
+    const int n_slots = useq ? m5 : m9;
     bool prev_quad = false;
     for (int wg = blockIdx.x; wg < n_slots; wg += gridDim.x) {
         if (wg != (int)blockIdx.x) { if (useq) un = unit_load<false>(T, wg); else un = unit_load<true>(T, wg); }
@@ -2771,7 +2800,7 @@
 }
 struct P2GGradArgs { SimP S; float* fr_cur; float* Gn_; float* Gc_; TableP T; const int* pool_idx; const float4* gg_in; int* blk_count; int* slow; AgentP agent; InjectP inj; int act; int f; float* Gd_; const int* to_slot; int fiso; };
 template <bool GENERAL, int MINW>
-__global__ FE_KALIGN __launch_bounds__(WG, MINW) void k_p2g_grad(SimP S, float* fr_cur, float* Gn_, float* Gc_, TableP T, const int* pool_idx, const float4* gg_in, int* blk_count, int* slow, AgentP agent, InjectP inj, int act, int f, float* Gd_, const int* to_slot, int fiso) { p2g_grad_body<GENERAL, MINW>(S, fr_cur, Gn_, Gc_, T, pool_idx, gg_in, blk_count, slow, agent, inj, act, f, Gd_, to_slot, fiso); }
+__global__ FE_KALIGN __launch_bounds__(WG, MINW) void k_p2g_grad(const UnitRec* h_units, const UnitRec* h_units_p, const int* h_meta, int h_cap, SimP S, float* fr_cur, float* Gn_, float* Gc_, TableP T, const int* pool_idx, const float4* gg_in, int* blk_count, int* slow, AgentP agent, InjectP inj, int act, int f, float* Gd_, const int* to_slot, int fiso) { T.units = h_units; T.units_p = h_units_p; T.meta = h_meta; T.units_cap = h_cap; p2g_grad_body<GENERAL, MINW>(S, fr_cur, Gn_, Gc_, T, pool_idx, gg_in, blk_count, slow, agent, inj, act, f, Gd_, to_slot, fiso); }
 template <bool GENERAL, int MINW>
 __global__ FE_KALIGN __launch_bounds__(WG, MINW) void k_p2g_grad_b(Batch<P2GGradArgs> B) { const P2GGradArgs& A = B.a[blockIdx.y]; p2g_grad_body<GENERAL, MINW>(A.S, A.fr_cur, A.Gn_, A.Gc_, A.T, A.pool_idx, A.gg_in, A.blk_count, A.slow, A.agent, A.inj, A.act, A.f, A.Gd_, A.to_slot, A.fiso); }
 
@@ -2780,6 +2809,10 @@
 __device__ __forceinline__ void p2g_grad_g2p_grad_body(SimP S, float* fr_cur, float* Gn_, float* Gc_, TableP T, const int* __restrict__ pool_idx,
                                                          const float4* __restrict__ gg_in, int* blk_count, int* slow, AgentP agent, InjectP inj, int act, int f,
                                                          int fiso, BwdFuseP B, GridStore GS) {
+    const UnitAsk ask0 = unit_ask<GENERAL>(T, blockIdx.x);
+    const int n_slots = T.meta[GENERAL ? 9 : 5];
+    HEAD_END(T.units_cap);
+    const Unit un0 = unit_take(ask0);
     const int tid = threadIdx.x;
     if (blockIdx.x == 0 && tid == 0) {
         *blk_count = 0;
@@ -2794,10 +2827,10 @@
     const GradDst D = {Gc, nullptr, T.pid_of_slot};
     float* const t4 = lds_tile4<AR>();
     double* const acc3 = lds_acc3<AR>();
-    const int n_slots = T.meta[GENERAL ? 9 : 5];
     bool prev_quad = false, any_tail = false;
     for (int wg = blockIdx.x; ; wg += gridDim.x) {
-        const Unit un = unit_load<GENERAL>(T, wg);
+        Unit un = un0;
+        if (wg != (int)blockIdx.x) un = unit_load<GENERAL>(T, wg);
         if (wg >= n_slots) break;
         if (un.a.z == -2) continue;
         if (un.a.z >= 0) {
@@ -2896,7 +2929,7 @@
 #define FE_FB_WAVES_LESS 0
 #endif
 template <int MINW, bool GENERAL = false>
-__global__ FE_KALIGN __launch_bounds__(WG, MINW - FE_FB_WAVES_LESS) void k_pgg_g2pg(SimP S, float* fr_cur, float* Gn_, float* Gc_, TableP T, const int* pool_idx, const float4* gg_in, int* blk_count, int* slow, AgentP agent, InjectP inj, int act, int f, int fiso, BwdFuseP B, GridStore GS) { p2g_grad_g2p_grad_body<MINW, GENERAL>(S, fr_cur, Gn_, Gc_, T, pool_idx, gg_in, blk_count, slow, agent, inj, act, f, fiso, B, GS); }
+__global__ FE_KALIGN __launch_bounds__(WG, MINW - FE_FB_WAVES_LESS) void k_pgg_g2pg(const UnitRec* h_list, const int* h_meta, int h_cap, SimP S, float* fr_cur, float* Gn_, float* Gc_, TableP T, const int* pool_idx, const float4* gg_in, int* blk_count, int* slow, AgentP agent, InjectP inj, int act, int f, int fiso, BwdFuseP B, GridStore GS) { if (GENERAL) T.units_p = h_list; else T.units = h_list; T.meta = h_meta; T.units_cap = h_cap; p2g_grad_g2p_grad_body<MINW, GENERAL>(S, fr_cur, Gn_, Gc_, T, pool_idx, gg_in, blk_count, slow, agent, inj, act, f, fiso, B, GS); }
 template <int MINW>
 __global__ FE_KALIGN __launch_bounds__(WG, MINW - FE_FB_WAVES_LESS) void k_pgg_g2pg_b(Batch<PggArgs> Bt) { const PggArgs& A = Bt.a[blockIdx.y]; p2g_grad_g2p_grad_body<MINW>(A.S, A.fr_cur, A.Gn_, A.Gc_, A.T, A.pool_idx, A.gg_in, A.blk_count, A.slow, A.agent, A.inj, A.act, A.f, A.fiso, A.B, A.GS); }
 
@@ -3898,6 +3931,9 @@
     return a;
 }
 
+#define HEAD_UNITS(T_)   (T_).units, (T_).meta, (T_).units_cap
+#define HEAD_UNITS_P(T_) (T_).units_p, (T_).meta, (T_).units_cap
+#define HEAD_UNITS_2(T_) (T_).units, (T_).units_p, (T_).meta, (T_).units_cap
 inline dim3 pgrid(FeEngine* h) { return dim3((h->N + 255) / 256); }
 inline dim3 wgrid(FeEngine* h) { int g = (h->N + 63) / 64 + 8; if (g < 512) g = 512; return dim3(g < h->wgrid_cap ? g : h->wgrid_cap); }
 inline dim3 wgrid_g2p(FeEngine* h) { int g = (h->N + 63) / 64 + 8; if (g < 512) g = 512; return dim3(g < h->wgrid_cap_g2p ? g : h->wgrid_cap_g2p); }
@@ -4108,8 +4144,10 @@
 template <bool KEEP>
 void launch_grid(FeEngine* h, const TableP& T, int f, const AgentP& ag) {
     const dim3 gg = ggrid_list(h, h->tbl_of_frame[f], f, !KEEP);
-#define LAUNCH_GRID(ST_, DY_) hipLaunchKernelGGL(HIP_KERNEL_NAME(k_grid<KEEP, ST_, DY_>), gg, dim3(256), 0, h->stream, h->S, T, h->slab, h->g_in, gout(h, f), \
-                           h->blk_list, bcount(h, f), h->blk_flag, grid_store(h), f, h->frame_slow_dev, statics_p(h), ag)
+    const GridStore GS = grid_store(h);
+#define LAUNCH_GRID(ST_, DY_) hipLaunchKernelGGL(HIP_KERNEL_NAME(k_grid<KEEP, ST_, DY_>), gg, dim3(256), 0, h->stream, T.active, GS.touched, GS.dirty, T.nbr, T.meta, \
+                           (const int*)bcount(h, f), h->nb * h->nb * h->nb, (int)gg.x, h->S, T, h->slab, h->g_in, gout(h, f), \
+                           h->blk_list, h->blk_flag, GS, f, h->frame_slow_dev, statics_p(h), ag)
     if (grid_collide(h)) { if (h->statics_host.empty()) LAUNCH_GRID(false, true); else LAUNCH_GRID(true, true); }
     else { if (h->statics_host.empty()) LAUNCH_GRID(false, false); else LAUNCH_GRID(true, false); }
 #undef LAUNCH_GRID
@@ -4149,10 +4187,10 @@
             if (h->all_simple_liquid) hipLaunchKernelGGL((k_g2p_p2g_fg<false>), wgrid(h), dim3(WG), 0, h->stream, A);
             else hipLaunchKernelGGL((k_g2p_p2g_fg<true>), wgrid(h), dim3(WG), 0, h->stream, A);
         } else if (h->all_simple_liquid)
-            hipLaunchKernelGGL((k_g2p_p2g<false>), wgrid(h), dim3(WG), 0, h->stream, h->S, h->frame(f), h->frame(f + 1), T,
+            hipLaunchKernelGGL((k_g2p_p2g<false>), wgrid(h), dim3(WG), 0, h->stream, HEAD_UNITS(T), h->S, h->frame(f), h->frame(f + 1), T,
                                h->pool_idx, grid_w(h, f), ag, inj, act, f, grid_store(h), fiso, FU);
         else
-            hipLaunchKernelGGL((k_g2p_p2g<true>), wgrid(h), dim3(WG), 0, h->stream, h->S, h->frame(f), h->frame(f + 1), T,
+            hipLaunchKernelGGL((k_g2p_p2g<true>), wgrid(h), dim3(WG), 0, h->stream, HEAD_UNITS(T), h->S, h->frame(f), h->frame(f + 1), T,
                                h->pool_idx, grid_w(h, f), ag, inj, act, f, grid_store(h), 0, FU);
         prof_end(h);
     } else {
@@ -4162,10 +4200,10 @@
         if (h->all_simple_liquid) hipLaunchKernelGGL((k_p2g_fg<false>), wgrid(h), dim3(WG), 0, h->stream, A);
         else hipLaunchKernelGGL((k_p2g_fg<true>), wgrid(h), dim3(WG), 0, h->stream, A);
     } else if (h->all_simple_liquid)
-        hipLaunchKernelGGL((k_p2g<true, false>), wgrid(h), dim3(WG), 0, h->stream, h->S, h->frame(f), h->frame(f + 1), T,
+        hipLaunchKernelGGL((k_p2g<true, false>), wgrid(h), dim3(WG), 0, h->stream, HEAD_UNITS(T), h->S, h->frame(f), h->frame(f + 1), T,
                            h->pool_idx, grid_w(h, f), ag, inj, act, f, grid_store(h), fiso);
     else
-        hipLaunchKernelGGL((k_p2g<true, true>), wgrid(h), dim3(WG), 0, h->stream, h->S, h->frame(f), h->frame(f + 1), T,
+        hipLaunchKernelGGL((k_p2g<true, true>), wgrid(h), dim3(WG), 0, h->stream, HEAD_UNITS(T), h->S, h->frame(f), h->frame(f + 1), T,
                            h->pool_idx, grid_w(h, f), ag, inj, act, f, grid_store(h), 0);
     prof_end(h);
     }
@@ -4186,14 +4224,14 @@
         }
         const SortKeyP K = {h->sort_key, h->sort_rank, h->sort_cnt, h->sort_bcnt, h->sort_nact};
         if (particle_collide(h))
-            hipLaunchKernelGGL(k_g2p_sortkey<true>, wgrid_g2p(h), dim3(WG), 0, h->stream, h->S, h->frame(f), h->frame(f + 1), T, gout(h, f), bcount(h, f), h->slow_dev, ag, f, K);
+            hipLaunchKernelGGL(k_g2p_sortkey<true>, wgrid_g2p(h), dim3(WG), 0, h->stream, HEAD_UNITS_P(T), h->S, h->frame(f), h->frame(f + 1), T, gout(h, f), bcount(h, f), h->slow_dev, ag, f, K);
         else
-            hipLaunchKernelGGL(k_g2p_sortkey<false>, wgrid_g2p(h), dim3(WG), 0, h->stream, h->S, h->frame(f), h->frame(f + 1), T, gout(h, f), bcount(h, f), h->slow_dev, ag, f, K);
+            hipLaunchKernelGGL(k_g2p_sortkey<false>, wgrid_g2p(h), dim3(WG), 0, h->stream, HEAD_UNITS_P(T), h->S, h->frame(f), h->frame(f + 1), T, gout(h, f), bcount(h, f), h->slow_dev, ag, f, K);
         h->keys_frame = f + 1; h->sort_scratch_dirty = true;
     } else if (particle_collide(h))
-        hipLaunchKernelGGL(k_g2p<true>, wgrid_g2p(h), dim3(WG), 0, h->stream, h->S, h->frame(f), h->frame(f + 1), T, gout(h, f), bcount(h, f), h->slow_dev, ag, f);
+        hipLaunchKernelGGL(k_g2p<true>, wgrid_g2p(h), dim3(WG), 0, h->stream, HEAD_UNITS_P(T), h->S, h->frame(f), h->frame(f + 1), T, gout(h, f), bcount(h, f), h->slow_dev, ag, f);
     else
-        hipLaunchKernelGGL(k_g2p<false>, wgrid_g2p(h), dim3(WG), 0, h->stream, h->S, h->frame(f), h->frame(f + 1), T, gout(h, f), bcount(h, f), h->slow_dev, ag, f);
+        hipLaunchKernelGGL(k_g2p<false>, wgrid_g2p(h), dim3(WG), 0, h->stream, HEAD_UNITS_P(T), h->S, h->frame(f), h->frame(f + 1), T, gout(h, f), bcount(h, f), h->slow_dev, ag, f);
     prof_end(h);
     if (h->has_rigid) {
         hipLaunchKernelGGL(k_rigid_body<false>, dim3(h->n_bodies), dim3(256), 0, h->stream, h->S, h->frame(f), h->frame(f + 1), (float*)nullptr,
@@ -4233,10 +4271,10 @@
     h->stamp++;
     prof_begin(h, KID_P2G_RE);
     if (h->all_simple_liquid)
-        hipLaunchKernelGGL((k_p2g<false, false>), wgrid(h), dim3(WG), 0, h->stream, h->S, h->frame(f), h->frame(f + 1), T,
+        hipLaunchKernelGGL((k_p2g<false, false>), wgrid(h), dim3(WG), 0, h->stream, HEAD_UNITS(T), h->S, h->frame(f), h->frame(f + 1), T,
                            h->pool_idx, grid_w(h, f), ag, noinj, 0, f, grid_store(h), h->fiso[f] ? 1 : 0);
     else
-        hipLaunchKernelGGL((k_p2g<false, true>), wgrid(h), dim3(WG), 0, h->stream, h->S, h->frame(f), h->frame(f + 1), T,
+        hipLaunchKernelGGL((k_p2g<false, true>), wgrid(h), dim3(WG), 0, h->stream, HEAD_UNITS(T), h->S, h->frame(f), h->frame(f + 1), T,
                            h->pool_idx, grid_w(h, f), ag, noinj, 0, f, grid_store(h), 0);
     prof_end(h);
     prof_begin(h, KID_GRID_KEEP);
@@ -4255,14 +4293,16 @@
         hipLaunchKernelGGL(k_collide_grad, dim3(std::min((h->N + 15) / 16, 2048)), dim3(256), 0, h->stream, h->S, h->frame(f), h->grad(f + 1), gout(h, f), T, grid_store(h), f, ag,
                            h->hit_list, h->hit_count);
     }
-    if (h->g2p_grad_v == 2) hipLaunchKernelGGL(k_g2p_grad2<3>, wgrid(h), dim3(WG), 0, h->stream, h->S, h->frame(f), h->grad(f + 1), h->grad(f), T, gout(h, f), h->gg_out, h->slab, h->slow_dev, grid_store(h), f, ag);
-    else hipLaunchKernelGGL(k_g2p_grad2<4>, wgrid(h), dim3(WG), 0, h->stream, h->S, h->frame(f), h->grad(f + 1), h->grad(f), T, gout(h, f), h->gg_out, h->slab, h->slow_dev, grid_store(h), f, ag);
+    if (h->g2p_grad_v == 2) hipLaunchKernelGGL(k_g2p_grad2<3>, wgrid(h), dim3(WG), 0, h->stream, HEAD_UNITS(T), h->S, h->frame(f), h->grad(f + 1), h->grad(f), T, gout(h, f), h->gg_out, h->slab, h->slow_dev, grid_store(h), f, ag);
+    else hipLaunchKernelGGL(k_g2p_grad2<4>, wgrid(h), dim3(WG), 0, h->stream, HEAD_UNITS(T), h->S, h->frame(f), h->grad(f + 1), h->grad(f), T, gout(h, f), h->gg_out, h->slab, h->slow_dev, grid_store(h), f, ag);
     prof_end(h);
     }
     prof_begin(h, KID_GRID_GRAD);
     const dim3 ggg = ggrid_list(h, t, f, false);
-#define LAUNCH_GRID_GRAD(ST_, DY_) hipLaunchKernelGGL(HIP_KERNEL_NAME(k_grid_grad<ST_, DY_>), ggg, dim3(256), 0, h->stream, h->S, T, h->slab, h->g_in, h->gg_out, \
-                           ggin(h, f), h->blk_list, bcount(h, f), h->blk_flag, grid_store(h), f, statics_p(h), ag, h->node_work, h->node_work_count)
+    const GridStore GSg = grid_store(h);
+#define LAUNCH_GRID_GRAD(ST_, DY_) hipLaunchKernelGGL(HIP_KERNEL_NAME(k_grid_grad<ST_, DY_>), ggg, dim3(256), 0, h->stream, T.active, (const unsigned char*)(stored ? GSg.live + (size_t)f * GSg.cap : GSg.cur), \
+                           GSg.dirty, T.nbr, T.meta, h->nb * h->nb * h->nb, (int)ggg.x, GSg.cap, stored ? 1 : 0, h->S, T, h->slab, h->g_in, h->gg_out, \
+                           ggin(h, f), h->blk_list, bcount(h, f), h->blk_flag, GSg, f, statics_p(h), ag, h->node_work, h->node_work_count)
     if (grid_collide(h)) {
         if (!h->node_work && (dev_alloc(h, &h->node_work, (size_t)h->S.ncell, false) || dev_alloc(h, &h->node_work_count, 1))) return 1;
         HIPCK(h, hipMemsetAsync(h->node_work_count, 0, sizeof(int), h->stream));
@@ -4284,7 +4324,7 @@
     const int* to_slot = fold ? h->tables[t_next].slot_of_pid : nullptr;
     const bool gc_out = compact_out && h->compact_F && h->all_simple_liquid && !h->has_collector;
     const int giso = (h->fiso[f] ? 1 : 0) | (h->gcompact[(f + 1) & 1] ? 2 : 0) | (gc_out ? 4 : 0);
-#define LAUNCH_P2G_GRAD(G, W) hipLaunchKernelGGL((k_p2g_grad<G, W>), wgrid_pgg(h), dim3(WG), 0, h->stream, h->S, h->frame(f), h->grad(f + 1), \
+#define LAUNCH_P2G_GRAD(G, W) hipLaunchKernelGGL((k_p2g_grad<G, W>), wgrid_pgg(h), dim3(WG), 0, h->stream, HEAD_UNITS_2(T), h->S, h->frame(f), h->grad(f + 1), \
                            h->grad(f), T, h->pool_idx, ggin(h, f), bcount(h, f), h->slow_dev, ag, inj, act, f, g_dst, to_slot, giso)
     if (!fuse_next) prof_begin(h, KID_P2G_GRAD);
     if (fuse_next) {
@@ -4292,10 +4332,10 @@
         const BwdFuseP B = {h->frame(f - 1), h->grad(f - 1), gout(h, f - 1), h->gg_out, h->slab};
         prof_begin(h, KID_PGG_G2PG);
         if (h->all_simple_liquid)
-            hipLaunchKernelGGL(k_pgg_g2pg<4>, wgrid(h), dim3(WG), 0, h->stream, h->S, h->frame(f), h->grad(f + 1), h->grad(f), T, h->pool_idx, ggin(h, f), bcount(h, f), h->slow_dev,
+            hipLaunchKernelGGL(k_pgg_g2pg<4>, wgrid(h), dim3(WG), 0, h->stream, HEAD_UNITS(T), h->S, h->frame(f), h->grad(f + 1), h->grad(f), T, h->pool_idx, ggin(h, f), bcount(h, f), h->slow_dev,
                                ag, inj, act, f, giso, B, grid_store(h));
         else
-            hipLaunchKernelGGL((k_pgg_g2pg<3, true>), wgrid(h), dim3(WG), 0, h->stream, h->S, h->frame(f), h->grad(f + 1), h->grad(f), T, h->pool_idx, ggin(h, f), bcount(h, f), h->slow_dev,
+            hipLaunchKernelGGL((k_pgg_g2pg<3, true>), wgrid(h), dim3(WG), 0, h->stream, HEAD_UNITS_P(T), h->S, h->frame(f), h->grad(f + 1), h->grad(f), T, h->pool_idx, ggin(h, f), bcount(h, f), h->slow_dev,
                                ag, inj, act, f, 0, B, grid_store(h));
     } else if (h->all_simple_liquid) {
         if (h->p2g_grad_waves >= 4) LAUNCH_P2G_GRAD(false, 4);
```
